# 07350100647/nvbio-gpl

Hardware: AMD Instinct MI355X
Metric: aligned reads/sec (150 bp single-end, 3 Gbp ref); GCUPS of the banded extend pass in `extend` (higher is better)
Workload: dtype u32 (FM-index coordinates) / i16x2 (band-31 DP, two alignments per 32-bit lane: 16-bit integer scores, held in binary16 lanes where every score is an integer of magnitude <= 2040 -- exact -- and in int16 lanes otherwise; bound-checked on the host)

## Files before the change

### include/nvbio_amd.h

```cpp
#ifndef NVBIO_AMD_H
#define NVBIO_AMD_H

#include <stdint.h>

#ifdef __cplusplus
extern "C" {
#endif

#define NVBIO_AMD_VERSION 100

typedef enum
{
    NVBIO_OK              = 0,
    NVBIO_ERR_INVALID     = 1,
    NVBIO_ERR_HIP         = 2,
    NVBIO_ERR_NOMEM       = 3,
    NVBIO_ERR_UNSUPPORTED = 4,
    NVBIO_ERR_NO_DEVICE   = 5
} nvbio_status;

int         nvbio_amd_version(void);
const char* nvbio_amd_last_error(void);
nvbio_status nvbio_amd_device_count(int* count);
nvbio_status nvbio_amd_device_arch(int device, char* name, uint32_t name_len);
nvbio_status nvbio_amd_stream_synchronize(int device, void* stream);
nvbio_status nvbio_amd_release_scratch(void);
nvbio_status nvbio_amd_set_scratch_check(int enable, uint32_t fill_byte);
nvbio_status nvbio_amd_scratch_check_report(char* buf, uint64_t buf_len);

typedef struct { uint32_t x, y; } nvbio_uint2;


typedef struct
{
    uint32_t        length;
    uint32_t        primary;
    uint32_t        L2[5];
    const uint32_t* bwt_occ_dev;
    uint64_t        bwt_occ_words;
    const uint32_t* ssa_dev;
    uint64_t        ssa_words;
    uint32_t        sa_int;
} nvbio_fm_index_view;

typedef struct nvbio_fm_index_s* nvbio_fm_index_t;

nvbio_status nvbio_fm_index_create(const nvbio_fm_index_view* view, int device, uint32_t kmer_len,
                                   void* stream, nvbio_fm_index_t* out);

typedef struct
{
    uint32_t kmer_len;
    uint32_t sa_int;
    uint32_t max_lcp;
    uint32_t verify;
    uint32_t table_flags;
    uint32_t bucket_symbols;
} nvbio_fm_build_options;

enum
{
    NVBIO_FM_TABLE_NO_DIRECT  = 1,
    NVBIO_FM_TABLE_NO_CONTEXT = 2,
    NVBIO_FM_TABLE_NO_GROUPS  = 4,
    NVBIO_FM_TABLE_CANONICAL_WIDE = 16,
    NVBIO_FM_TABLE_NO_TEXT_PLANES = 32,
    NVBIO_FM_TABLE_CANONICAL  = 8
};

nvbio_status nvbio_fm_index_build(const uint32_t* text2_dev, uint32_t length, int device,
                                  const nvbio_fm_build_options* options ,
                                  void* stream, nvbio_fm_index_t* out);

nvbio_status nvbio_fm_index_load(const char* bwt_path, const char* sa_path, int device, uint32_t kmer_len,
                                 void* stream, nvbio_fm_index_t* out);
nvbio_status nvbio_fm_index_save(nvbio_fm_index_t index, const char* bwt_path, const char* sa_path, void* stream);

nvbio_status nvbio_fm_index_destroy(nvbio_fm_index_t index);
nvbio_status nvbio_fm_index_get_view(nvbio_fm_index_t index, nvbio_fm_index_view* view);
nvbio_status nvbio_fm_index_export(nvbio_fm_index_t index, uint32_t* bwt_occ_out_dev, uint32_t* ssa_out_dev, void* stream);
nvbio_status nvbio_fm_index_device_bytes(nvbio_fm_index_t index, uint64_t* bytes);

nvbio_status nvbio_text_planes_bytes(uint32_t length, uint64_t* bytes);
nvbio_status nvbio_text_planes_build(int device, const uint32_t* text2_dev, uint32_t length, void* planes_dev, void* stream);
nvbio_status nvbio_fm_index_text_planes(nvbio_fm_index_t index, const void** planes_dev, uint32_t* length);

typedef struct
{
    const void*     symbols_dev;
    uint32_t        symbol_bits;
    const uint32_t* offsets_dev;
    uint32_t        offsets_are_ranges;
    uint32_t        fixed_len;
    uint32_t        stride;
    uint32_t        n;
    uint32_t        seeds_per_string;
    uint32_t        seed_interval;
    const uint32_t* seed_intervals_dev;
} nvbio_string_set;

enum
{
    NVBIO_FM_SCAN_FORWARD = 1,
    NVBIO_FM_COMPLEMENT   = 2,
    NVBIO_FM_NO_KMER_TABLE = 4,
    NVBIO_FM_NO_VERIFY     = 8,
    NVBIO_FM_COUNT_SECTORS = 16,
    NVBIO_FM_NO_PIPELINE   = 32
};

nvbio_status nvbio_fm_match(nvbio_fm_index_t index, const nvbio_string_set* queries, uint32_t flags,
                            nvbio_uint2* ranges_dev, uint32_t* blocks_dev, void* stream);

nvbio_status nvbio_fm_rank(nvbio_fm_index_t index, const uint32_t* rows_dev, const uint8_t* syms_dev, uint32_t n,
                           uint32_t* out_dev, void* stream);
nvbio_status nvbio_fm_rank4(nvbio_fm_index_t index, const uint32_t* rows_dev, uint32_t n,
                            uint32_t* out_dev, void* stream);

typedef struct
{
    const void* text_dev;
    uint32_t    word_bits;
    const void* occ_dev;
    uint32_t    index_bits;
    uint32_t    K;
    uint64_t    length;
} nvbio_rank_dictionary;
nvbio_status nvbio_rank_dictionary_occ_entries(const nvbio_rank_dictionary* dict, uint64_t* entries);
nvbio_status nvbio_rank_dictionary_build(int device, const nvbio_rank_dictionary* dict, void* occ_out_dev, uint64_t counts[4], void* stream);
nvbio_status nvbio_rank_dictionary_rank(int device, const nvbio_rank_dictionary* dict, const void* idx_dev, const uint8_t* syms_dev, uint32_t n,
                                        void* out_dev, void* stream);
nvbio_status nvbio_rank_dictionary_rank4(int device, const nvbio_rank_dictionary* dict, const void* idx_dev, uint32_t n, void* out_dev, void* stream);

nvbio_status nvbio_fm_basic_inv_psi(nvbio_fm_index_t index, const uint32_t* rows_dev, uint32_t n,
                                    uint32_t* out_dev, void* stream);

nvbio_status nvbio_fm_locate(nvbio_fm_index_t index, const uint32_t* rows_dev, uint32_t n,
                             uint32_t* pos_dev, void* stream);
nvbio_status nvbio_fm_match_direct(nvbio_fm_index_t index, const nvbio_string_set* queries, uint32_t flags,
                                   nvbio_uint2* ranges_dev, uint8_t* direct_dev, void* stream);
nvbio_status nvbio_fm_index_supports_direct(nvbio_fm_index_t index, int* yes);
nvbio_status nvbio_fm_filter_locate_direct(nvbio_fm_index_t index, const nvbio_uint2* ranges_dev, const uint64_t* slots_dev,
                                           const uint8_t* direct_dev, uint32_t n_queries, uint64_t begin, uint64_t end,
                                           nvbio_uint2* hits_dev, void* stream);

nvbio_status nvbio_fm_filter_locate_diagonals(nvbio_fm_index_t index, const nvbio_uint2* ranges_dev, const uint64_t* slots_dev,
                                              const uint8_t* direct_dev, uint32_t n_queries, uint64_t begin, uint64_t end,
                                              uint32_t seeds_per_read, uint32_t seed_interval, uint32_t seed_len, uint32_t read_len,
                                              uint32_t strand, const uint32_t* query_ids_dev, uint64_t* keys_dev, void* stream);

enum { NVBIO_BACKTRACK_REFERENCE_QUIRKS = 1 };
nvbio_status nvbio_fm_hamming_backtrack(nvbio_fm_index_t index, const nvbio_string_set* queries, uint32_t seed_len, uint32_t mismatches, uint32_t flags,
                                        uint32_t* counts_dev, uint32_t* n_ranges_dev, nvbio_uint2* ranges_dev, uint32_t max_ranges, void* stream);

nvbio_status nvbio_fm_match_seed_diagonals_temp_bytes(const nvbio_string_set* seeds, uint64_t* bytes);
nvbio_status nvbio_fm_match_seed_diagonals(nvbio_fm_index_t index, const nvbio_string_set* seeds, uint32_t flags, uint32_t read_len,
                                           uint32_t strand, uint64_t* keys_dev, nvbio_uint2* residual_ranges_dev, uint32_t* residual_ids_dev,
                                           uint32_t* counts_dev, void* temp_dev, uint64_t temp_bytes, void* stream);

#define NVBIO_FM_INLINE_HITS(h) (((uint32_t)(h) & 15u) << 8)
#define NVBIO_FM_DEFER_HEAVY 64u
nvbio_status nvbio_fm_match_seed_diagonals_both_temp_bytes(const nvbio_string_set* seeds, uint64_t* bytes);
nvbio_status nvbio_fm_match_seed_diagonals_both_keys_capacity(const nvbio_string_set* seeds, uint64_t* n_keys);
nvbio_status nvbio_fm_match_seed_diagonals_both(nvbio_fm_index_t index, const nvbio_string_set* seeds, uint32_t flags, uint32_t read_len,
                                                uint64_t* keys_dev, nvbio_uint2* residual_ranges_dev, uint32_t* residual_ids_dev,
                                                uint32_t residual_capacity, uint32_t* counts_dev, void* temp_dev, uint64_t temp_bytes,
                                                void* stream);
nvbio_status nvbio_fm_seed_tiles(const nvbio_string_set* seeds, uint32_t* reads_per_tile, uint32_t* n_tiles);
nvbio_status nvbio_fm_match_seed_diagonals_both_tiled(nvbio_fm_index_t index, const nvbio_string_set* seeds, uint32_t flags, uint32_t read_len,
                                                      uint64_t* keys_dev, nvbio_uint2* residual_ranges_dev, uint32_t* residual_ids_dev,
                                                      uint32_t residual_capacity, uint32_t* counts_dev, uint32_t* tile_offsets_dev,
                                                      void* temp_dev, uint64_t temp_bytes, void* stream);
int nvbio_fm_index_is_canonical(nvbio_fm_index_t index);

nvbio_status nvbio_fm_locate_init(nvbio_fm_index_t index, const uint32_t* rows_dev, uint32_t n,
                                  nvbio_uint2* jt_dev, void* stream);
nvbio_status nvbio_fm_locate_lookup(nvbio_fm_index_t index, const nvbio_uint2* jt_dev, uint32_t n,
                                    uint32_t* pos_dev, void* stream);

nvbio_status nvbio_fm_filter_rank(nvbio_fm_index_t index, const nvbio_string_set* queries, uint32_t flags,
                                  nvbio_uint2* ranges_dev, uint64_t* slots_dev, uint64_t* n_hits, void* stream);
nvbio_status nvbio_fm_filter_scan(nvbio_fm_index_t index, const nvbio_uint2* ranges_dev, uint32_t n_queries,
                                  uint64_t* slots_dev, uint64_t* n_hits, void* stream);
nvbio_status nvbio_fm_filter_locate(nvbio_fm_index_t index, const nvbio_uint2* ranges_dev, const uint64_t* slots_dev,
                                    uint32_t n_queries, uint64_t begin, uint64_t end,
                                    nvbio_uint2* hits_dev, void* stream);


typedef struct { uint32_t x, y, string_id, span; } nvbio_mem_range;
typedef struct { uint32_t pos, string_id, span_begin, span_end; } nvbio_mem_hit;
typedef struct { uint32_t min_intv, max_intv, min_span, split_len, split_width; } nvbio_mem_params;

nvbio_status nvbio_mem_filter_temp_bytes(const nvbio_string_set* reads, const nvbio_mem_params* params, uint64_t* bytes, void* stream);
nvbio_status nvbio_mem_filter_rank(nvbio_fm_index_t f_index, nvbio_fm_index_t r_index, const nvbio_string_set* reads,
                                   const nvbio_mem_params* params, nvbio_mem_range* ranges_dev, uint32_t max_ranges,
                                   uint32_t* first_range_dev, uint64_t* slots_dev, void* temp_dev, uint64_t temp_bytes,
                                   uint32_t* n_ranges, uint64_t* n_mems, uint64_t* records, void* stream);
nvbio_status nvbio_mem_filter_locate(nvbio_fm_index_t f_index, const nvbio_mem_range* ranges_dev, const uint64_t* slots_dev,
                                     uint32_t n_ranges, uint64_t begin, uint64_t end, nvbio_mem_hit* hits_dev, void* stream);

typedef struct nvbio_qgram_index_s* nvbio_qgram_index_t;

typedef struct
{
    uint32_t        q, symbol_size, qlut;
    uint32_t        is_set;
    uint32_t        n_qgrams, n_unique;
    uint64_t        lut_size;
    int             device;
    const uint64_t* qgrams_dev;
    const uint32_t* slots_dev;
    const void*     index_dev;
    const uint32_t* lut_dev;
} nvbio_qgram_index_view;

nvbio_status nvbio_qgram_index_build(int device, const void* text_dev, uint32_t text_bits, uint32_t length, uint32_t q, uint32_t symbol_size,
                                     uint32_t qlut, nvbio_qgram_index_t* out, void* stream);
nvbio_status nvbio_qgram_set_index_build(int device, const nvbio_string_set* set, uint32_t q, uint32_t symbol_size, uint32_t seed_interval,
                                         uint32_t qlut, nvbio_qgram_index_t* out, void* stream);
nvbio_status nvbio_qgram_index_destroy(nvbio_qgram_index_t index);
nvbio_status nvbio_qgram_index_get_view(nvbio_qgram_index_t index, nvbio_qgram_index_view* view);
nvbio_status nvbio_qgram_index_device_bytes(nvbio_qgram_index_t index, uint64_t* bytes);
nvbio_status nvbio_qgram_index_export(nvbio_qgram_index_t index, uint64_t* qgrams_out_dev, uint32_t* slots_out_dev, void* index_out_dev,
                                      uint32_t* lut_out_dev, void* stream);

nvbio_status nvbio_generate_qgrams_temp_bytes(uint32_t n, int sort, uint64_t* bytes);
nvbio_status nvbio_generate_qgrams(int device, uint32_t q, uint32_t symbol_size, const void* text_dev, uint32_t text_bits, uint32_t text_len,
                                   uint32_t first_pos, uint32_t n, uint64_t* qgrams_dev, uint32_t* indices_dev, int sort,
                                   void* temp_dev, uint64_t temp_bytes, void* stream);
nvbio_status nvbio_qgram_ranges(nvbio_qgram_index_t index, const uint64_t* qgrams_dev, uint32_t n, nvbio_uint2* ranges_dev, void* stream);

nvbio_status nvbio_qgram_filter_temp_bytes(uint32_t n_queries, uint64_t* bytes);
nvbio_status nvbio_qgram_filter_rank(nvbio_qgram_index_t index, const uint64_t* qgrams_dev, uint32_t n, nvbio_uint2* ranges_dev, uint64_t* slots_dev,
                                     void* temp_dev, uint64_t temp_bytes, uint64_t* n_hits, void* stream);
nvbio_status nvbio_qgram_filter_locate(nvbio_qgram_index_t index, const nvbio_uint2* ranges_dev, const uint64_t* slots_dev, const uint32_t* indices_dev,
                                       uint32_t n, uint64_t begin, uint64_t end, void* hits_dev, void* stream);
nvbio_status nvbio_qgram_filter_merge_temp_bytes(int is_set, uint32_t n_hits, uint64_t* bytes);
nvbio_status nvbio_qgram_filter_merge(int device, int is_set, uint32_t interval, const void* hits_dev, uint32_t n_hits, void* merged_dev,
                                      uint32_t* counts_dev, uint32_t* n_merged, void* temp_dev, uint64_t temp_bytes, void* stream);

typedef struct
{
    uint32_t           q, symbol_size;
    uint32_t           is_set;
    uint32_t           n_qgrams, n_unique;
    uint64_t           n_words;
    int                device;
    const nvbio_uint2* table_dev;
    const uint32_t*    ss_dev;
    const void*        p_dev;
} nvbio_qgroup_index_view;

nvbio_status nvbio_qgroup_index_build(int device, const void* text_dev, uint32_t text_bits, uint32_t length, uint32_t q, uint32_t symbol_size,
                                      nvbio_qgram_index_t* out, void* stream);
nvbio_status nvbio_qgroup_set_index_build(int device, const nvbio_string_set* set, uint32_t q, uint32_t symbol_size, uint32_t seed_interval,
                                          nvbio_qgram_index_t* out, void* stream);
nvbio_status nvbio_qgroup_index_get_view(nvbio_qgram_index_t index, nvbio_qgroup_index_view* view);
nvbio_status nvbio_qgroup_index_export(nvbio_qgram_index_t index, uint32_t* I_out_dev, uint32_t* S_out_dev, uint32_t* SS_out_dev, void* P_out_dev,
                                       void* stream);

enum { NVBIO_SUFSORT_NO_EMPTY_SUFFIXES = 1 };

typedef struct
{
    uint32_t n_suffixes;
    uint32_t rounds;
    uint32_t sorted_per_round[16];
    uint32_t symbols_per_word;
    uint64_t peak_bytes;
} nvbio_sufsort_stats;

nvbio_status nvbio_set_suffix_count(int device, const nvbio_string_set* set, uint32_t flags, uint32_t* n_suffixes, void* stream);
nvbio_status nvbio_set_suffix_sort(int device, const nvbio_string_set* set, uint32_t flags, nvbio_uint2* suffixes_dev, uint32_t* global_dev,
                                   uint64_t capacity, uint32_t* n_suffixes, nvbio_sufsort_stats* stats, void* stream);
nvbio_status nvbio_set_suffix_sort_flat(int device, const nvbio_string_set* set, uint32_t flags, uint32_t* suffix_array_dev, uint32_t* string_ids_dev,
                                        uint32_t* cum_lengths_dev, uint64_t capacity, uint32_t* n_suffixes, nvbio_sufsort_stats* stats, void* stream);
nvbio_status nvbio_set_bwt(int device, const nvbio_string_set* set, uint32_t flags, uint8_t* bwt_dev, nvbio_uint2* suffixes_dev,
                           uint64_t capacity, uint32_t* n_suffixes, nvbio_sufsort_stats* stats, void* stream);

nvbio_status nvbio_suffix_sort(const uint32_t* text2_dev, uint32_t length, int device, uint32_t* sa_dev, void* stream);
nvbio_status nvbio_bwt(const uint32_t* text2_dev, uint32_t length, int device, uint32_t* bwt_words_dev, uint32_t* primary, void* stream);


nvbio_status nvbio_hits_to_diagonals(int device, const nvbio_uint2* hits_dev, uint64_t n_hits, uint32_t seeds_per_read,
                                     uint32_t seed_interval, uint32_t seed_len, uint32_t read_len, uint32_t strand,
                                     uint64_t* keys_dev, void* stream);

nvbio_status nvbio_sort_unique_keys_temp_bytes(uint64_t n, uint64_t* bytes);
nvbio_status nvbio_sort_unique_keys(int device, uint64_t* keys_dev, uint64_t n, uint32_t* n_out_dev, void* temp_dev, uint64_t temp_bytes, void* stream);

nvbio_status nvbio_diagonals_to_windows(int device, const uint64_t* keys_dev, uint64_t n, uint32_t band, uint32_t read_len,
                                        uint32_t genome_len, uint32_t* read_id_dev, uint8_t* flags_dev,
                                        uint32_t* win_begin_dev, uint32_t* win_end_dev, void* stream);

nvbio_status nvbio_diagonals_to_windows_ragged(int device, const uint64_t* keys_dev, uint64_t n, uint32_t band, const uint32_t* read_offsets_dev,
                                               uint32_t genome_len, uint32_t* read_id_dev, uint8_t* flags_dev,
                                               uint32_t* win_begin_dev, uint32_t* win_end_dev, void* stream);
nvbio_status nvbio_fm_filter_locate_diagonals_ragged(nvbio_fm_index_t index, const nvbio_uint2* ranges_dev, const uint64_t* slots_dev,
                                                     const uint8_t* direct_dev, uint32_t n_queries, uint64_t begin, uint64_t end,
                                                     uint32_t seeds_per_read, uint32_t seed_len, const uint32_t* read_offsets_dev,
                                                     const uint32_t* seed_intervals_dev, uint32_t strand, const uint32_t* query_ids_dev,
                                                     uint64_t* keys_dev, void* stream);
nvbio_status nvbio_traceback_best_batch_ragged(int device, const uint64_t* best_dev, const int64_t* best_wb_dev, uint32_t n_reads,
                                               const uint32_t* read_offsets_dev, uint32_t band, uint32_t genome_len, const int32_t* min_scores_dev,
                                               uint8_t* flags_dev, uint32_t* win_begin_dev, uint32_t* win_end_dev, int32_t* scores_dev,
                                               nvbio_uint2* sinks_dev, void* stream);
nvbio_status nvbio_second_candidate_reduce_ragged(int device, const uint64_t* keys_dev, const int32_t* scores_dev, const nvbio_uint2* sinks_dev,
                                                  const uint32_t* win_begin_dev, uint64_t n, const uint64_t* best_dev,
                                                  const uint32_t* read_offsets_dev, const int32_t* min_scores_dev, uint64_t* second_dev, void* stream);
nvbio_status nvbio_mapq_ragged(int device, const uint64_t* best_dev, const uint64_t* second_dev, uint32_t n_reads, int32_t version, int32_t match,
                               const uint32_t* read_offsets_dev, const int32_t* min_scores_dev, int32_t* second_scores_dev, uint8_t* mapq_dev,
                               void* stream);

nvbio_status nvbio_fm_residual_diagonals(nvbio_fm_index_t index, const nvbio_uint2* ranges_dev, const uint32_t* ids_dev, uint32_t n, uint32_t cap,
// ... 380 lines not shown
```

### nvbio-gpl_amd/__init__.py

```python
import ctypes
import os

import numpy as np

_HERE = os.path.dirname(os.path.abspath(__file__))
LIB_PATH = os.path.join(_HERE, "lib", "libnvbio_amd.so")
HEADER_PATH = os.path.join(os.path.dirname(_HERE), "include", "nvbio_amd.h")

GLOBAL, LOCAL, SEMI_GLOBAL = 0, 1, 2
SCORE_MIN = -(1 << 30)
FM_SCAN_FORWARD, FM_COMPLEMENT, FM_NO_KMER_TABLE, FM_NO_VERIFY, FM_COUNT_SECTORS, FM_NO_PIPELINE, FM_DEFER_HEAVY = 1, 2, 4, 8, 16, 32, 64
FM_TABLE_NO_DIRECT, FM_TABLE_NO_CONTEXT, FM_TABLE_NO_GROUPS, FM_TABLE_CANONICAL, FM_TABLE_CANONICAL_WIDE = 1, 2, 4, 8, 16
FM_TABLE_NO_TEXT_PLANES = 32
READ_REVERSE, READ_COMPLEMENT = 1, 2
TRACEBACK_SINKS_GIVEN = 1
ALN_NO_UNGAPPED_SCORE, ALN_NO_THIRD_CHANCE, ALN_NO_PACKED_DP, ALN_FORCE_PACKED_DP, ALN_NO_UNGAPPED_TRACEBACK, ALN_PK_THREE_WAVES = 1, 2, 4, 8, 16, 32
ALN_NO_NARROW_TRACEBACK, ALN_NO_SECOND_CHANCE, ALN_PK_STRIPE8, ALN_NO_NARROW_SCORE, ALN_NO_BAND_ROUTE = 64, 128, 256, 512, 1024
ALN_NO_QUALITY_SHORTCUT, ALN_RAGGED_READS, ALN_NO_LENGTH_SORT, ALN_NO_F16_DP, ALN_NO_COOPERATIVE_DP, ALN_NO_GAP_CHANCE = 2048, 4096, 8192, 16384, 32768, 65536
ALN_SPLIT_CHANCES, ALN_NO_PAIRED_GAP_CHANCE = 131072, 262144
ALN_NO_NARROW_DP = 524288
ALN_NO_TEXT_PLANES = 1048576
ROUTE_SETTLED, ROUTE_FULL_BAND, ROUTE_CLASS_A, ROUTE_CLASS_B, ROUTE_REDONE = 0, 1, 2, 3, 8
DEFAULT_ALGO_FLAGS = 0
BACKTRACK_REFERENCE_QUIRKS = 1

_STATUS = {0: "OK", 1: "INVALID", 2: "HIP", 3: "NOMEM", 4: "UNSUPPORTED", 5: "NO_DEVICE"}


class NvbioError(RuntimeError):
    def __init__(self, status, msg):
        super().__init__("nvbio_amd: %s: %s" % (_STATUS.get(status, status), msg))
        self.status = status


class _View(ctypes.Structure):
    _fields_ = [("length", ctypes.c_uint32), ("primary", ctypes.c_uint32), ("L2", ctypes.c_uint32 * 5),
                ("bwt_occ_dev", ctypes.c_void_p), ("bwt_occ_words", ctypes.c_uint64),
                ("ssa_dev", ctypes.c_void_p), ("ssa_words", ctypes.c_uint64), ("sa_int", ctypes.c_uint32)]


class _BuildOptions(ctypes.Structure):
    _fields_ = [("kmer_len", ctypes.c_uint32), ("sa_int", ctypes.c_uint32), ("max_lcp", ctypes.c_uint32),
                ("verify", ctypes.c_uint32), ("table_flags", ctypes.c_uint32), ("bucket_symbols", ctypes.c_uint32)]


class _StringSet(ctypes.Structure):
    _fields_ = [("symbols_dev", ctypes.c_void_p), ("symbol_bits", ctypes.c_uint32),
                ("offsets_dev", ctypes.c_void_p), ("offsets_are_ranges", ctypes.c_uint32),
                ("fixed_len", ctypes.c_uint32), ("stride", ctypes.c_uint32), ("n", ctypes.c_uint32),
                ("seeds_per_string", ctypes.c_uint32), ("seed_interval", ctypes.c_uint32),
                ("seed_intervals_dev", ctypes.c_void_p)]


class _Scheme(ctypes.Structure):
    _fields_ = [("match", ctypes.c_int32), ("mm_min", ctypes.c_int32), ("mm_max", ctypes.c_int32),
                ("pat_gap_open", ctypes.c_int32), ("pat_gap_ext", ctypes.c_int32),
                ("txt_gap_open", ctypes.c_int32), ("txt_gap_ext", ctypes.c_int32)]


class _SWScheme(ctypes.Structure):
    _fields_ = [("match", ctypes.c_int32), ("mismatch", ctypes.c_int32), ("deletion", ctypes.c_int32),
                ("insertion", ctypes.c_int32)]


class _Batch(ctypes.Structure):
    _fields_ = [("reads_dev", ctypes.c_void_p), ("read_bits", ctypes.c_uint32),
                ("read_offsets_dev", ctypes.c_void_p), ("quals_dev", ctypes.c_void_p),
                ("read_id_dev", ctypes.c_void_p), ("flags_dev", ctypes.c_void_p),
                ("text_dev", ctypes.c_void_p), ("text_bits", ctypes.c_uint32),
                ("win_begin_dev", ctypes.c_void_p), ("win_end_dev", ctypes.c_void_p), ("n", ctypes.c_uint32),
                ("max_read_len", ctypes.c_uint32), ("algo_flags", ctypes.c_uint32),
                ("text_planes_dev", ctypes.c_void_p)]


class _HitQueues(ctypes.Structure):
    _fields_ = [("idx_queue_dev", ctypes.c_void_p), ("hit_read_id_dev", ctypes.c_void_p), ("hit_seed_dev", ctypes.c_void_p),
                ("hit_loc_dev", ctypes.c_void_p), ("hit_score_dev", ctypes.c_void_p), ("hit_sink_dev", ctypes.c_void_p),
                ("n", ctypes.c_uint32)]


class _SeedHitsParams(ctypes.Structure):
    _fields_ = [(n, ctypes.c_uint32) for n in ("seeds_per_read", "first_offset", "seed_interval", "seed_len", "read_len", "max_hits",
                                                "rep_seeds", "max_effort", "min_ext", "max_ext")]


class _RaggedSeedLayout(ctypes.Structure):
    _fields_ = [("read_offsets_dev", ctypes.c_void_p), ("seed_intervals_dev", ctypes.c_void_p)] + \
               [(n, ctypes.c_uint32) for n in ("seeds_per_read", "seeding_pass", "max_reseed", "seed_len", "min_read_len")]


class _RankDict(ctypes.Structure):
    _fields_ = [("text_dev", ctypes.c_void_p), ("word_bits", ctypes.c_uint32), ("occ_dev", ctypes.c_void_p), ("index_bits", ctypes.c_uint32),
                ("K", ctypes.c_uint32), ("length", ctypes.c_uint64)]


_lib = None


def lib():
    global _lib
    if _lib is None:
        if not os.path.exists(LIB_PATH):
            raise NvbioError(5, "%s is missing: build it with __graft_entry__.build() "
                                "(there is no CPU fallback)" % LIB_PATH)
        import torch
        L = ctypes.CDLL(LIB_PATH)
        L.nvbio_amd_last_error.restype = ctypes.c_char_p
        L.nvbio_amd_version.restype = ctypes.c_int
        _lib = L
    return _lib


def release_scratch():
    _check(lib().nvbio_amd_release_scratch())


def set_scratch_check(enable, fill_byte=0):
    _check(lib().nvbio_amd_set_scratch_check(ctypes.c_int(1 if enable else 0), ctypes.c_uint32(fill_byte)))


def scratch_check_report():
    buf = ctypes.create_string_buffer(1 << 16)
    _check(lib().nvbio_amd_scratch_check_report(buf, ctypes.c_uint64(len(buf))))
    out = {}
    for line in buf.value.decode().splitlines():
        tag, checked, damaged, sub, off = line.split()
        out[tag] = (int(checked), int(damaged), None if sub == "-" else int(sub), None if off == "-" else int(off))
    return out


def _check(status):
    if status != 0:
        raise NvbioError(status, lib().nvbio_amd_last_error().decode())


def _torch():
    import torch
    return torch


_SCRATCH = {}


def _scratch(device, nbytes, cap=8 << 30):
    torch = _torch()
    nbytes = int(min(max(nbytes, 1 << 20), cap))
    key = str(device)
    t = _SCRATCH.get(key)
    if t is None or t.numel() < nbytes:
        _SCRATCH[key] = None
        t = _SCRATCH[key] = torch.empty(nbytes, dtype=torch.uint8, device=device)
    return t


def _ptr(t):
    return None if t is None else ctypes.c_void_p(t.data_ptr())


def _stream_ptr(device):
    torch = _torch()
    return ctypes.c_void_p(torch.cuda.current_stream(device).cuda_stream)


def device_count():
    n = ctypes.c_int(0)
    lib().nvbio_amd_device_count(ctypes.byref(n))
    return n.value


def _dev_tensor(a, dtype, device):
    torch = _torch()
    if a is None:
        return None
    if isinstance(a, torch.Tensor):
        t = a
        if t.dtype != dtype:
            t = t.view(dtype) if t.element_size() == torch.empty(0, dtype=dtype).element_size() else t.to(dtype)
        return t.to(device).contiguous()
    a = np.ascontiguousarray(a)
    np_of = {torch.int32: np.int32, torch.uint8: np.uint8, torch.int64: np.int64}[dtype]
    if a.dtype.itemsize == np.dtype(np_of).itemsize:
        a = a.view(np_of)
    else:
        a = a.astype(np_of)
    return torch.from_numpy(a).to(device)


class PackedStringSet:

    def __init__(self, symbols, bits, n, offsets=None, ranges=False, fixed_len=0, stride=None, device="cuda:0",
                 seeds_per_string=0, seed_interval=0, seed_intervals=None):
        torch = _torch()
        self.bits, self.n = int(bits), int(n)
        self.symbols = _dev_tensor(symbols, torch.uint8 if bits == 8 else torch.int32, device)
        self.offsets = _dev_tensor(offsets, torch.int32, device)
        self.ranges, self.fixed_len = bool(ranges), int(fixed_len)
        self.stride = int(fixed_len if stride is None else stride)
        self.device = device
        self.seeds_per_string, self.seed_interval = int(seeds_per_string), int(seed_interval)
        self.seed_intervals = _dev_tensor(seed_intervals, torch.int32, device)

    def c_struct(self):
        return _StringSet(_ptr(self.symbols), self.bits, _ptr(self.offsets), 1 if self.ranges else 0,
                          self.fixed_len, self.stride, self.n, self.seeds_per_string, self.seed_interval, _ptr(self.seed_intervals))


class FMIndex:

    def __init__(self, handle, device, keep=()):
        self._h, self.device, self._keep = handle, device, keep
        self._text_src = None
        self._text_planes = None

    @staticmethod
    def _dev_index(device):
        torch = _torch()
        d = torch.device(device)
        return d.index if d.index is not None else 0

    @classmethod
    def from_arrays(cls, length, primary, L2, bwt_occ, ssa, kmer_len=0, sa_int=16, device="cuda:0"):
        torch = _torch()
        b = _dev_tensor(bwt_occ, torch.int32, device)
        s = _dev_tensor(ssa, torch.int32, device) if ssa is not None else None
        v = _View()
        v.length, v.primary = int(length), int(primary)
        for i in range(5):
            v.L2[i] = int(L2[i])
        v.bwt_occ_dev, v.bwt_occ_words = b.data_ptr(), b.numel()
        v.ssa_dev, v.ssa_words = (s.data_ptr(), s.numel()) if s is not None else (None, 0)
        v.sa_int = sa_int
        h = ctypes.c_void_p()
        _check(lib().nvbio_fm_index_create(ctypes.byref(v), cls._dev_index(device), ctypes.c_uint32(kmer_len),
                                           _stream_ptr(device), ctypes.byref(h)))
        return cls(h, device, keep=(b, s))

    @classmethod
    def build(cls, text2, length, kmer_len=0, max_lcp=0, sa_int=16, verify=False, device="cuda:0", table_flags=0,
              bucket_symbols=None):
        torch = _torch()
        t = _dev_tensor(text2, torch.int32, device)
        h = ctypes.c_void_p()
        opts = _BuildOptions(kmer_len, sa_int, max_lcp, 1 if verify else 0, int(table_flags),
                             0 if bucket_symbols is None else 1 + int(bucket_symbols))
        _check(lib().nvbio_fm_index_build(_ptr(t), ctypes.c_uint32(length), cls._dev_index(device),
                                          ctypes.byref(opts), _stream_ptr(device), ctypes.byref(h)))
        fmi = cls(h, device, keep=(t,))
        fmi._text_src = (t.data_ptr(), int(length))
        fmi._text_planes = fmi.text_planes()
        return fmi

    @classmethod
    def load(cls, bwt_path, sa_path=None, kmer_len=0, device="cuda:0"):
        h = ctypes.c_void_p()
        _check(lib().nvbio_fm_index_load(bwt_path.encode(), sa_path.encode() if sa_path else None,
                                         cls._dev_index(device), ctypes.c_uint32(kmer_len), _stream_ptr(device),
                                         ctypes.byref(h)))
        return cls(h, device)

    def save(self, bwt_path, sa_path=None):
        _check(lib().nvbio_fm_index_save(self._h, bwt_path.encode(), sa_path.encode() if sa_path else None,
                                         _stream_ptr(self.device)))

    def close(self):
        if self._h is not None:
            _torch().cuda.synchronize(self.device)
            _check(lib().nvbio_fm_index_destroy(self._h))
            self._h = None
            self._seed_bufs = None

    def __del__(self):
        try:
            self.close()
        except Exception:
            pass

    def view(self):
        v = _View()
        _check(lib().nvbio_fm_index_get_view(self._h, ctypes.byref(v)))
        return v

    @property
    def length(self):
        return self.view().length

    @property
    def primary(self):
        return self.view().primary

    def arrays(self):
        torch = _torch()
        v = self.view()
        b = torch.empty(int(v.bwt_occ_words), dtype=torch.int32, device=self.device)
        s = torch.empty(int(v.ssa_words), dtype=torch.int32, device=self.device)
        _check(lib().nvbio_fm_index_export(self._h, _ptr(b), _ptr(s), _stream_ptr(self.device)))
        return b, s

    def device_bytes(self):
        b = ctypes.c_uint64()
        _check(lib().nvbio_fm_index_device_bytes(self._h, ctypes.byref(b)))
        return b.value

    def text_planes(self):
        p, n = ctypes.c_void_p(), ctypes.c_uint32()
        _check(lib().nvbio_fm_index_text_planes(self._h, ctypes.byref(p), ctypes.byref(n)))
        return (p.value, n.value) if p.value else None

    def text_planes_of(self, text2, length):
        tp = self._text_planes if self._h is not None else None
        same = tp is not None and self._text_src == (text2.data_ptr(), int(length)) and tp[1] == int(length)
        return tp[0] if same else None

    def match(self, queries, flags=0, want_blocks=False):
        torch = _torch()
        ranges = torch.empty((queries.n, 2), dtype=torch.int32, device=self.device)
        blocks = torch.empty(queries.n, dtype=torch.int32, device=self.device) if want_blocks else None
        qs = queries.c_struct()
        _check(lib().nvbio_fm_match(self._h, ctypes.byref(qs), ctypes.c_uint32(flags), _ptr(ranges), _ptr(blocks),
                                    _stream_ptr(self.device)))
        return (ranges, blocks) if want_blocks else ranges

    def supports_direct(self):
        yes = ctypes.c_int(0)
        _check(lib().nvbio_fm_index_supports_direct(self._h, ctypes.byref(yes)))
        return bool(yes.value)

    def match_direct(self, queries, flags=0):
        torch = _torch()
        ranges = torch.empty((queries.n, 2), dtype=torch.int32, device=self.device)
        direct = torch.empty(queries.n, dtype=torch.uint8, device=self.device)
        qs = queries.c_struct()
        _check(lib().nvbio_fm_match_direct(self._h, ctypes.byref(qs), ctypes.c_uint32(flags), _ptr(ranges), _ptr(direct),
                                           _stream_ptr(self.device)))
        return ranges, direct

    def hamming_backtrack(self, queries, seed_len, mismatches, quirks=False, max_ranges=0):
        torch = _torch()
        counts = torch.empty(queries.n, dtype=torch.int32, device=self.device)
        nr = torch.empty(queries.n, dtype=torch.int32, device=self.device)
        rg = torch.zeros((queries.n, max_ranges, 2), dtype=torch.int32, device=self.device) if max_ranges else None
        qs = queries.c_struct()
        _check(lib().nvbio_fm_hamming_backtrack(self._h, ctypes.byref(qs), ctypes.c_uint32(seed_len), ctypes.c_uint32(mismatches),
                                                ctypes.c_uint32(BACKTRACK_REFERENCE_QUIRKS if quirks else 0), _ptr(counts), _ptr(nr), _ptr(rg),
                                                ctypes.c_uint32(max_ranges), _stream_ptr(self.device)))
        return counts, nr, rg

    def match_seed_diagonals(self, seeds, flags, read_len, strand, buffers=None, grid_blocks=0):
        torch = _torch()
        n = seeds.n
        if buffers is None:
            buffers = {}
        qs = seeds.c_struct()
        if buffers.get("n") != n or buffers.get("spr") != seeds.seeds_per_string:
            buffers["n"], buffers["spr"] = n, seeds.seeds_per_string
            buffers["keys"] = torch.empty(n, dtype=torch.int64, device=self.device)
            buffers["ranges"] = torch.empty((n, 2), dtype=torch.int32, device=self.device)
            buffers["ids"] = torch.empty(n, dtype=torch.int32, device=self.device)
            buffers["counts"] = torch.empty(4, dtype=torch.int32, device=self.device)
            nb = ctypes.c_uint64(0)
            _check(lib().nvbio_fm_match_seed_diagonals_temp_bytes(ctypes.byref(qs), ctypes.byref(nb)))
            buffers["temp"] = torch.empty(nb.value, dtype=torch.uint8, device=self.device)
        assert grid_blocks % 64 == 0 and grid_blocks < (1 << 22)
        _check(lib().nvbio_fm_match_seed_diagonals(self._h, ctypes.byref(qs), ctypes.c_uint32(flags | ((grid_blocks // 64) << 16)),
                                                   ctypes.c_uint32(read_len), ctypes.c_uint32(strand), _ptr(buffers["keys"]),
                                                   _ptr(buffers["ranges"]), _ptr(buffers["ids"]), _ptr(buffers["counts"]),
                                                   _ptr(buffers["temp"]), ctypes.c_uint64(buffers["temp"].numel()),
                                                   _stream_ptr(self.device)))
        return buffers

    @property
    def canonical_kmer(self):
        fn = lib().nvbio_fm_index_is_canonical
        fn.restype = ctypes.c_int
        return int(fn(self._h))

    @property
    def canonical(self):
        return self.canonical_kmer != 0

    def match_seed_diagonals_both(self, seeds, read_len, buffers=None, flags=0, grid_blocks=0, inline_hits=0, defer_heavy=False):
        torch = _torch()
        n = seeds.n
        if buffers is None:
            buffers = {}
        qs = seeds.c_struct()
        if buffers.get("n") != n or buffers.get("spr") != seeds.seeds_per_string:
            buffers["n"], buffers["spr"] = n, seeds.seeds_per_string
            cap = ctypes.c_uint64(0)
            _check(lib().nvbio_fm_match_seed_diagonals_both_keys_capacity(ctypes.byref(qs), ctypes.byref(cap)))
            buffers["keys"] = torch.empty(max(int(cap.value), 1), dtype=torch.int64, device=self.device)
            buffers["ranges"] = torch.empty((2 * n, 2), dtype=torch.int32, device=self.device)
            buffers["ids"] = torch.empty(2 * n, dtype=torch.int32, device=self.device)
            buffers["counts"] = torch.empty(6, dtype=torch.int32, device=self.device)
            nb = ctypes.c_uint64(0)
            _check(lib().nvbio_fm_match_seed_diagonals_both_temp_bytes(ctypes.byref(qs), ctypes.byref(nb)))
            buffers["temp"] = torch.empty(nb.value, dtype=torch.uint8, device=self.device)
            rpt, nt = ctypes.c_uint32(0), ctypes.c_uint32(0)
            _check(lib().nvbio_fm_seed_tiles(ctypes.byref(qs), ctypes.byref(rpt), ctypes.byref(nt)))
            buffers["reads_per_tile"], buffers["n_tiles"] = int(rpt.value), int(nt.value)
            buffers["tile_offsets"] = torch.zeros(int(nt.value) + 1, dtype=torch.int32, device=self.device)
        assert grid_blocks % 64 == 0 and grid_blocks < (1 << 22)
        _check(lib().nvbio_fm_match_seed_diagonals_both_tiled(
            self._h, ctypes.byref(qs), ctypes.c_uint32(flags | (FM_DEFER_HEAVY if defer_heavy else 0) | ((int(inline_hits) & 15) << 8) | ((grid_blocks // 64) << 16)),
            ctypes.c_uint32(read_len),
            _ptr(buffers["keys"]), _ptr(buffers["ranges"]), _ptr(buffers["ids"]), ctypes.c_uint32(n), _ptr(buffers["counts"]),
            _ptr(buffers["tile_offsets"]), _ptr(buffers["temp"]), ctypes.c_uint64(buffers["temp"].numel()), _stream_ptr(self.device)))
        return buffers

    def residual_diagonals(self, ranges, ids, cap, seeds_per_read, seed_interval, seed_len, read_len, read_offsets=None, seed_intervals=None):
        torch = _torch()
        n = int(ids.numel())
        keys = torch.empty(max(n * int(cap), 1), dtype=torch.int64, device=self.device)
        n_keys = torch.zeros(1, dtype=torch.int32, device=self.device)
        _check(lib().nvbio_fm_residual_diagonals(
            self._h, _ptr(ranges), _ptr(ids), ctypes.c_uint32(n), ctypes.c_uint32(int(cap)), ctypes.c_uint32(seeds_per_read),
            ctypes.c_uint32(seed_interval), ctypes.c_uint32(seed_len), ctypes.c_uint32(read_len), _ptr(read_offsets), _ptr(seed_intervals),
            _ptr(keys), _ptr(n_keys), _stream_ptr(self.device)))
        return keys, n_keys

    def rank(self, rows, syms):
        torch = _torch()
        rows = _dev_tensor(rows, torch.int32, self.device)
        syms = _dev_tensor(syms, torch.uint8, self.device)
        out = torch.empty(rows.numel(), dtype=torch.int32, device=self.device)
        _check(lib().nvbio_fm_rank(self._h, _ptr(rows), _ptr(syms), ctypes.c_uint32(rows.numel()), _ptr(out),
                                   _stream_ptr(self.device)))
        return out

    def rank4(self, rows):
        torch = _torch()
        rows = _dev_tensor(rows, torch.int32, self.device)
        out = torch.empty((rows.numel(), 4), dtype=torch.int32, device=self.device)
        _check(lib().nvbio_fm_rank4(self._h, _ptr(rows), ctypes.c_uint32(rows.numel()), _ptr(out),
                                    _stream_ptr(self.device)))
        return out

    def basic_inv_psi(self, rows):
        torch = _torch()
        rows = _dev_tensor(rows, torch.int32, self.device)
        out = torch.empty(rows.numel(), dtype=torch.int32, device=self.device)
        _check(lib().nvbio_fm_basic_inv_psi(self._h, _ptr(rows), ctypes.c_uint32(rows.numel()), _ptr(out),
                                            _stream_ptr(self.device)))
        return out

    def locate(self, rows):
        torch = _torch()
        rows = _dev_tensor(rows, torch.int32, self.device)
        pos = torch.empty(rows.numel(), dtype=torch.int32, device=self.device)
        _check(lib().nvbio_fm_locate(self._h, _ptr(rows), ctypes.c_uint32(rows.numel()), _ptr(pos),
                                     _stream_ptr(self.device)))
        return pos

    def locate_ssa_iterator(self, rows):
        torch = _torch()
        rows = _dev_tensor(rows, torch.int32, self.device)
        jt = torch.empty((rows.numel(), 2), dtype=torch.int32, device=self.device)
        _check(lib().nvbio_fm_locate_init(self._h, _ptr(rows), ctypes.c_uint32(rows.numel()), _ptr(jt),
                                          _stream_ptr(self.device)))
        return jt

    def lookup_ssa_iterator(self, jt):
        torch = _torch()
        pos = torch.empty(jt.shape[0], dtype=torch.int32, device=self.device)
        _check(lib().nvbio_fm_locate_lookup(self._h, _ptr(jt), ctypes.c_uint32(jt.shape[0]), _ptr(pos),
                                            _stream_ptr(self.device)))
        return pos


class FMIndexFilter:

    def __init__(self):
        self._index = None
        self._ranges = self._slots = self._direct = None
        self._n_hits = 0
        self._n_queries = 0

    def rank(self, index, string_set, flags=0):
        torch = _torch()
        self._index, self._n_queries, self._direct = index, string_set.n, None
        self._ranges = torch.empty((string_set.n, 2), dtype=torch.int32, device=index.device)
        self._slots = torch.empty(string_set.n, dtype=torch.int64, device=index.device)
        total = ctypes.c_uint64(0)
        qs = string_set.c_struct()
        _check(lib().nvbio_fm_filter_rank(index._h, ctypes.byref(qs), ctypes.c_uint32(flags), _ptr(self._ranges),
                                          _ptr(self._slots), ctypes.byref(total), _stream_ptr(index.device)))
        self._n_hits = total.value
        return self._n_hits

    def rank_ranges(self, index, ranges, direct=None):
        torch = _torch()
        self._index, self._n_queries, self._ranges, self._direct = index, ranges.shape[0], ranges, direct
        self._slots = torch.empty(ranges.shape[0], dtype=torch.int64, device=index.device)
        total = ctypes.c_uint64(0)
        _check(lib().nvbio_fm_filter_scan(index._h, _ptr(ranges), ctypes.c_uint32(ranges.shape[0]), _ptr(self._slots),
                                          ctypes.byref(total), _stream_ptr(index.device)))
        self._n_hits = total.value
        return self._n_hits

    def locate(self, begin, end, hits=None):
        torch = _torch()
        if hits is None:
            hits = torch.empty((end - begin, 2), dtype=torch.int32, device=self._index.device)
        if self._direct is not None:
            _check(lib().nvbio_fm_filter_locate_direct(self._index._h, _ptr(self._ranges), _ptr(self._slots), _ptr(self._direct),
                                                       ctypes.c_uint32(self._n_queries), ctypes.c_uint64(begin),
                                                       ctypes.c_uint64(end), _ptr(hits), _stream_ptr(self._index.device)))
            return hits
        _check(lib().nvbio_fm_filter_locate(self._index._h, _ptr(self._ranges), _ptr(self._slots),
                                            ctypes.c_uint32(self._n_queries), ctypes.c_uint64(begin),
                                            ctypes.c_uint64(end), _ptr(hits), _stream_ptr(self._index.device)))
        return hits

    def locate_diagonals(self, begin, end, seeds_per_read, seed_interval, seed_len, read_len, strand, query_ids=None, read_offsets=None,
                         seed_intervals=None):
        torch = _torch()
        keys = torch.empty(end - begin, dtype=torch.int64, device=self._index.device)
        if read_offsets is not None:
            _check(lib().nvbio_fm_filter_locate_diagonals_ragged(
                self._index._h, _ptr(self._ranges), _ptr(self._slots), _ptr(self._direct), ctypes.c_uint32(self._n_queries),
                ctypes.c_uint64(begin), ctypes.c_uint64(end), ctypes.c_uint32(seeds_per_read), ctypes.c_uint32(seed_len), _ptr(read_offsets),
                _ptr(seed_intervals), ctypes.c_uint32(strand), _ptr(query_ids), _ptr(keys), _stream_ptr(self._index.device)))
            return keys
        _check(lib().nvbio_fm_filter_locate_diagonals(
            self._index._h, _ptr(self._ranges), _ptr(self._slots), _ptr(self._direct), ctypes.c_uint32(self._n_queries),
            ctypes.c_uint64(begin), ctypes.c_uint64(end), ctypes.c_uint32(seeds_per_read), ctypes.c_uint32(seed_interval),
            ctypes.c_uint32(seed_len), ctypes.c_uint32(read_len), ctypes.c_uint32(strand), _ptr(query_ids), _ptr(keys),
            _stream_ptr(self._index.device)))
        return keys

    def n_hits(self):
        return self._n_hits

    def ranges(self):
        return self._ranges

    def slots(self):
        return self._slots


class _MemParams(ctypes.Structure):
    _fields_ = [("min_intv", ctypes.c_uint32), ("max_intv", ctypes.c_uint32), ("min_span", ctypes.c_uint32),
                ("split_len", ctypes.c_uint32), ("split_width", ctypes.c_uint32)]


MEM_GROUP_FLAG = 1 << 31
MEM_UNLIMITED = 0xFFFFFFFF
# ... 333 lines not shown

class QGramFilter:

    def __init__(self):
        self._index = None
        self._ranges = self._slots = self._indices = self._temp = None
        self._merged = self._counts = None
        self._n_queries = self._n_hits = 0

    def _grow_temp(self, nbytes, dev):
        torch = _torch()
        if self._temp is None or self._temp.numel() < nbytes or self._temp.device != torch.device(dev):
            self._temp = None
            self._temp = torch.empty(max(int(nbytes), 1), dtype=torch.uint8, device=dev)

    def rank(self, index, qgrams, indices):
        torch = _torch()
        dev = index.device
        g = _dev_tensor(qgrams, torch.int64, dev)
        ix = _dev_tensor(indices, torch.int32, dev)
        n = g.numel()
        self._index, self._n_queries, self._indices = index, n, ix
        if self._ranges is None or self._ranges.shape[0] < n or self._ranges.device != torch.device(dev):
            self._ranges = torch.empty((max(n, 1), 2), dtype=torch.int32, device=dev)
            self._slots = torch.empty(max(n, 1), dtype=torch.int64, device=dev)
        tb = ctypes.c_uint64(0)
        _check(lib().nvbio_qgram_filter_temp_bytes(ctypes.c_uint32(n), ctypes.byref(tb)))
        self._grow_temp(tb.value, dev)
        nh = ctypes.c_uint64(0)
        _check(lib().nvbio_qgram_filter_rank(index._h, _ptr(g), ctypes.c_uint32(n), _ptr(self._ranges), _ptr(self._slots), _ptr(self._temp),
                                             ctypes.c_uint64(self._temp.numel()), ctypes.byref(nh), _stream_ptr(dev)))
        self._n_hits = nh.value
        return self._n_hits

    def n_hits(self):
        return self._n_hits

    def ranges(self):
        return self._ranges[:self._n_queries]

    def slots(self):
        return self._slots[:self._n_queries]

    def locate(self, begin, end, hits=None):
        torch = _torch()
        cols = 4 if self._index.IS_SET else 2
        if hits is None:
            hits = torch.empty((max(end - begin, 0), cols), dtype=torch.int32, device=self._index.device)
        if end > begin:
            _check(lib().nvbio_qgram_filter_locate(self._index._h, _ptr(self._ranges), _ptr(self._slots), _ptr(self._indices),
                                                   ctypes.c_uint32(self._n_queries), ctypes.c_uint64(begin), ctypes.c_uint64(end), _ptr(hits),
                                                   _stream_ptr(self._index.device)))
        return hits

    def merge(self, interval, hits, is_set=None):
        torch = _torch()
        if is_set is None:
            is_set = hits.dim() == 2 and hits.shape[1] == 4
        dev = hits.device
        n = hits.shape[0]
        tb = ctypes.c_uint64(0)
        _check(lib().nvbio_qgram_filter_merge_temp_bytes(ctypes.c_int(1 if is_set else 0), ctypes.c_uint32(n), ctypes.byref(tb)))
        self._grow_temp(tb.value, dev)
        if self._merged is None or self._merged.shape[0] < max(n, 1) or self._merged.device != dev:
            self._merged = torch.empty((max(n, 1), 2), dtype=torch.int32, device=dev)
            self._counts = torch.empty(max(n, 1), dtype=torch.int32, device=dev)
        nm = ctypes.c_uint32(0)
        hits = hits.contiguous()
        _check(lib().nvbio_qgram_filter_merge(FMIndex._dev_index(dev), ctypes.c_int(1 if is_set else 0), ctypes.c_uint32(interval), _ptr(hits),
                                              ctypes.c_uint32(n), _ptr(self._merged), _ptr(self._counts), ctypes.byref(nm), _ptr(self._temp),
                                              ctypes.c_uint64(self._temp.numel()), _stream_ptr(dev)))
        m = nm.value
        merged = self._merged.view(-1)[:2 * m].view(m, 2) if is_set else self._merged.view(-1)[:m]
        return merged.clone(), self._counts[:m].clone()


class GotohScheme:

    def __init__(self, match, mm_min, mm_max, pat_gap_open, pat_gap_ext, txt_gap_open, txt_gap_ext):
        self.c = _Scheme(match, mm_min, mm_max, pat_gap_open, pat_gap_ext, txt_gap_open, txt_gap_ext)


def SimpleGotohScheme(match, mismatch, gap_open, gap_ext):
    return GotohScheme(match, -mismatch, -mismatch, gap_open, gap_ext, gap_open, gap_ext)


def EditDistanceScheme():
    return GotohScheme(0, 1, 1, -1, -1, -1, -1)


class SimpleSmithWatermanScheme:

    def __init__(self, match, mismatch, deletion, insertion):
        self.c = _SWScheme(match, mismatch, deletion, insertion)


class SmithWatermanAligner:

    def __init__(self, type, scheme):
        self.type, self.sw = type, scheme
        c = scheme.c
        self.scheme = (GotohScheme(c.match, -c.mismatch, -c.mismatch, c.deletion, c.deletion, c.deletion, c.deletion)
                       if c.deletion == c.insertion else None)


def make_smith_waterman_aligner(type, scheme):
    return SmithWatermanAligner(type, scheme)


def make_edit_distance_aligner(type):
    return SmithWatermanAligner(type, SimpleSmithWatermanScheme(0, -1, -1, -1))


class GotohAligner:

    def __init__(self, type, scheme):
        self.type, self.scheme = type, scheme


def make_gotoh_aligner(type, scheme):
    return GotohAligner(type, scheme)


class AlignmentBatch:

    def __init__(self, reads, read_bits, read_offsets, text, text_bits, win_begin, win_end, quals=None, read_id=None,
                 flags=None, device="cuda:0", max_read_len=0, algo_flags=None, text_planes=None):
        torch = _torch()
        self.device = device
        self.text_planes = text_planes
        self.algo_flags = DEFAULT_ALGO_FLAGS if algo_flags is None else int(algo_flags)
        self.read_bits, self.text_bits = int(read_bits), int(text_bits)
        self.reads = _dev_tensor(reads, torch.uint8 if read_bits == 8 else torch.int32, device)
        self.read_offsets = _dev_tensor(read_offsets, torch.int32, device)
        self.text = _dev_tensor(text, torch.uint8 if text_bits == 8 else torch.int32, device)
        self.win_begin = _dev_tensor(win_begin, torch.int32, device)
        self.win_end = _dev_tensor(win_end, torch.int32, device)
        self.quals = _dev_tensor(quals, torch.uint8, device)
        self.read_id = _dev_tensor(read_id, torch.int32, device)
        self.flags = _dev_tensor(flags, torch.uint8, device)
        self.n = int(self.win_begin.numel())
        self.max_read_len = int(max_read_len)

    def size(self):
        return self.n

    def c_struct(self):
        return _Batch(_ptr(self.reads), self.read_bits, _ptr(self.read_offsets), _ptr(self.quals), _ptr(self.read_id),
                      _ptr(self.flags), _ptr(self.text), self.text_bits, _ptr(self.win_begin), _ptr(self.win_end),
                      self.n, self.max_read_len, self.algo_flags,
                      ctypes.c_void_p(self.text_planes.data_ptr() if hasattr(self.text_planes, "data_ptr") else self.text_planes))


def text_planes_bytes(length):
    b = ctypes.c_uint64()
    _check(lib().nvbio_text_planes_bytes(ctypes.c_uint32(length), ctypes.byref(b)))
    return b.value


def build_text_planes(text2, length, device="cuda:0", out=None):
    torch = _torch()
    t = _dev_tensor(text2, torch.int32, device)
    if out is None:
        out = torch.empty(text_planes_bytes(length), dtype=torch.uint8, device=device)
    _check(lib().nvbio_text_planes_build(FMIndex._dev_index(device), _ptr(t), ctypes.c_uint32(length), _ptr(out), _stream_ptr(device)))
    return out


DEVICE_THREAD_SCHEDULER = "DeviceThreadScheduler"
DEVICE_STAGED_THREAD_SCHEDULER = "DeviceStagedThreadScheduler"


class BatchedBandedAlignmentScore:

    def __init__(self, band_len, aligner, scheduler=DEVICE_THREAD_SCHEDULER):
        self.band_len, self.aligner, self.scheduler = int(band_len), aligner, scheduler
        if scheduler not in (DEVICE_THREAD_SCHEDULER, DEVICE_STAGED_THREAD_SCHEDULER):
            raise NvbioError(1, "unknown scheduler %r" % (scheduler,))

    def min_temp_storage(self, max_pattern_len, max_text_len, stream_size):
        return 0

    max_temp_storage = min_temp_storage

    def enact(self, batch, scores=None, sinks=None, min_scores=None):
        torch = _torch()
        if scores is None:
            scores = torch.empty(batch.n, dtype=torch.int32, device=batch.device)
        if sinks is None:
            sinks = torch.empty((batch.n, 2), dtype=torch.int32, device=batch.device)
        bs = batch.c_struct()
        sw = getattr(self.aligner, "sw", None)
        if self.scheduler == DEVICE_STAGED_THREAD_SCHEDULER:
            if sw is not None:
                raise NvbioError(4, "the staged scheduler is instantiated for Gotoh aligners")
            per_job = min_scores is not None and not isinstance(min_scores, int)
            if per_job and (min_scores.dtype != torch.int32 or min_scores.numel() != batch.n):
                raise NvbioError(1, "min_scores: int32 per job")
            _check(lib().nvbio_banded_gotoh_score_staged(
                FMIndex._dev_index(batch.device), ctypes.c_uint32(self.band_len), ctypes.c_int(self.aligner.type),
                ctypes.byref(self.aligner.scheme.c), ctypes.byref(bs), _ptr(min_scores) if per_job else None,
                ctypes.c_int32(SCORE_MIN if min_scores is None else (0 if per_job else int(min_scores))),
                _ptr(scores), _ptr(sinks), _stream_ptr(batch.device)))
            return scores, sinks
        fn = lib().nvbio_banded_sw_score if sw is not None else lib().nvbio_banded_gotoh_score
        _check(fn(FMIndex._dev_index(batch.device), ctypes.c_uint32(self.band_len), ctypes.c_int(self.aligner.type),
                  ctypes.byref(sw.c if sw is not None else self.aligner.scheme.c),
                  ctypes.byref(bs), _ptr(scores), _ptr(sinks), _stream_ptr(batch.device)))
        return scores, sinks


def batch_banded_alignment_score(band_len, aligner, batch):
    return BatchedBandedAlignmentScore(band_len, aligner).enact(batch)


def banded_gotoh_score_routes(band_len, aligner, batch):
    torch = _torch()
    scores = torch.empty(batch.n, dtype=torch.int32, device=batch.device)
    sinks = torch.empty((batch.n, 2), dtype=torch.int32, device=batch.device)
    routes = torch.empty(batch.n, dtype=torch.uint8, device=batch.device)
    bs = batch.c_struct()
    _check(lib().nvbio_banded_gotoh_score_routes(FMIndex._dev_index(batch.device), ctypes.c_uint32(int(band_len)), ctypes.c_int(aligner.type),
                                                 ctypes.byref(aligner.scheme.c), ctypes.byref(bs), _ptr(scores), _ptr(sinks), _ptr(routes),
                                                 _stream_ptr(batch.device)))
    return scores, sinks, routes


TB_ROUTE_SETTLED, TB_ROUTE_FULL_BAND, TB_ROUTE_BAND15, TB_ROUTE_BAND7 = 0, 1, 2, 3


def banded_gotoh_traceback_routes(band_len, aligner, batch, cigar_stride=64, temp=None, scores=None, sinks=None):
    torch = _torch()
    n, dev = batch.n, batch.device
    given = scores is not None and sinks is not None
    if not given:
        scores = torch.empty(n, dtype=torch.int32, device=dev)
        sinks = torch.empty((n, 2), dtype=torch.int32, device=dev)
    sources = torch.empty((n, 2), dtype=torch.int32, device=dev)
    cigars = torch.zeros((n, cigar_stride), dtype=torch.int16, device=dev)
    lens = torch.empty(n, dtype=torch.int32, device=dev)
    routes = torch.empty(n, dtype=torch.uint8, device=dev)
    band_off = torch.empty(n, dtype=torch.uint8, device=dev)
    bs = batch.c_struct()
    _check(lib().nvbio_banded_gotoh_traceback_routes(
        FMIndex._dev_index(dev), ctypes.c_uint32(int(band_len)), ctypes.c_int(aligner.type), ctypes.byref(aligner.scheme.c), ctypes.byref(bs),
        _ptr(scores), _ptr(sources), _ptr(sinks), _ptr(cigars), ctypes.c_uint32(cigar_stride), _ptr(lens),
        ctypes.c_uint32(TRACEBACK_SINKS_GIVEN if given else 0), _ptr(temp),
        ctypes.c_uint64(0 if temp is None else temp.numel() * temp.element_size()), _ptr(routes), _ptr(band_off), _stream_ptr(dev)))
    return scores, sources, sinks, cigars, lens, routes, band_off


GAP_PAIR_MAX_SHIFT = 5
NO_PARTNER = 0xFFFFFFFF


def banded_gap_pairs(batch):
    torch = _torch()
    partner = torch.empty(batch.n, dtype=torch.int32, device=batch.device)
    bs = batch.c_struct()
    _check(lib().nvbio_banded_gap_pairs(FMIndex._dev_index(batch.device), ctypes.byref(bs), _ptr(partner), _stream_ptr(batch.device)))
    return partner


class BatchedBandedAlignmentTraceback:

    def __init__(self, band_len, aligner):
        self.band_len, self.aligner = int(band_len), aligner

    def min_temp_storage(self, batch):
        out = ctypes.c_uint64(0)
        bs = batch.c_struct()
        _check(lib().nvbio_banded_gotoh_traceback_temp_bytes(ctypes.byref(bs), ctypes.c_uint32(self.band_len), ctypes.byref(out)))
        return int(out.value)

    def enact(self, batch, cigar_stride=64, temp=None, scores=None, sinks=None):
        torch = _torch()
        n, dev = batch.n, batch.device
        given = scores is not None and sinks is not None
        if not given:
            scores = torch.empty(n, dtype=torch.int32, device=dev)
            sinks = torch.empty((n, 2), dtype=torch.int32, device=dev)
        sources = torch.empty((n, 2), dtype=torch.int32, device=dev)
        cigars = torch.zeros((n, cigar_stride), dtype=torch.int16, device=dev)
        lens = torch.empty(n, dtype=torch.int32, device=dev)
        bs = batch.c_struct()
        sw = getattr(self.aligner, "sw", None)
        fn = lib().nvbio_banded_sw_traceback if sw is not None else lib().nvbio_banded_gotoh_traceback
        _check(fn(
            FMIndex._dev_index(dev), ctypes.c_uint32(self.band_len), ctypes.c_int(self.aligner.type),
            ctypes.byref(sw.c if sw is not None else self.aligner.scheme.c), ctypes.byref(bs), _ptr(scores), _ptr(sources), _ptr(sinks), _ptr(cigars),
            ctypes.c_uint32(cigar_stride), _ptr(lens), ctypes.c_uint32(TRACEBACK_SINKS_GIVEN if given else 0), _ptr(temp),
            ctypes.c_uint64(0 if temp is None else temp.numel() * temp.element_size()), _stream_ptr(dev)))
        return scores, sources, sinks, cigars, lens


class BatchedAlignmentTraceback:

    def __init__(self, aligner):
        self.aligner = aligner

    def min_temp_storage(self, batch, max_pattern_len, max_text_len):
        out = ctypes.c_uint64(0)
        bs = batch.c_struct()
        _check(lib().nvbio_full_gotoh_traceback_temp_bytes(ctypes.byref(bs), ctypes.c_uint32(max_pattern_len),
                                                           ctypes.c_uint32(max_text_len), ctypes.byref(out)))
        return int(out.value)
# ... 655 lines not shown
```

### nvbio-gpl_amd/csrc/bitplanes.h

```cpp
#pragma once
#include "common.h"

namespace nvbio_amd {

constexpr uint32_t PLANE_MAX_READ = 161u;

template <int RBITS> struct ReadWords { static constexpr int N = (161 + 15) * RBITS / 32 + 2; uint32_t w[N]; };

template <int RBITS>
__device__ __forceinline__ void load_read_words(const void* reads, const uint32_t first, const uint32_t M, ReadWords<RBITS>& out)
{
    constexpr uint32_t RPW = 32u / RBITS;
    const uint32_t* __restrict__ rwords = (const uint32_t*)reads;
    const uint32_t rw0 = (first & ~(RPW - 1u)) / RPW, rw_last = (first + M - 1u) / RPW;
    #pragma unroll
    for (int j = 0; j < ReadWords<RBITS>::N; ++j) { const uint32_t widx = rw0 + (uint32_t)j; out.w[j] = rwords[widx < rw_last ? widx : rw_last]; }
}

template <typename W>
__device__ __forceinline__ void load_text_words13(const void* text, const uint32_t tb, const uint32_t T, W& out)
{
    const uint32_t* __restrict__ twords = (const uint32_t*)text;
    const uint32_t tw0 = (tb & ~15u) >> 4, tw_last = (tb + T - 1u) >> 4;
    #pragma unroll
    for (int j = 0; j < 13; ++j) { const uint32_t widx = tw0 + (uint32_t)j; out.w[j] = twords[widx < tw_last ? widx : tw_last]; }
}

template <typename W>
__device__ __forceinline__ void load_text_words14(const void* text, const uint32_t tb, const uint32_t T, W& out)
{
    const uint32_t* __restrict__ twords = (const uint32_t*)text;
    const uint32_t tw0 = (tb & ~15u) >> 4, tw_last = (tb + T - 1u) >> 4;
    #pragma unroll
    for (int j = 0; j < 14; ++j) { const uint32_t widx = tw0 + (uint32_t)j; out.w[j] = twords[widx < tw_last ? widx : tw_last]; }
}

__device__ __forceinline__ void shr192(uint64_t (&v)[3], const uint32_t sh)
{
    const uint32_t ws = sh >> 6, bs = sh & 63u;
    uint64_t x[5] = { v[0], v[1], v[2], 0ull, 0ull };
    uint64_t y[4];
    #pragma unroll
    for (int k = 0; k < 4; ++k) y[k] = ws == 0u ? x[k] : (ws == 1u ? x[k + 1 < 5 ? k + 1 : 4] : (ws == 2u ? (k + 2 < 5 ? x[k + 2] : 0ull) : 0ull));
    #pragma unroll
    for (int k = 0; k < 3; ++k) v[k] = bs ? ((y[k] >> bs) | (y[k + 1] << (64u - bs))) : y[k];
}
__device__ __forceinline__ void mirror192(uint64_t (&v)[3])
{
    const uint64_t a = __brevll( v[2] ), c = __brevll( v[0] );
    v[1] = __brevll( v[1] ); v[0] = a; v[2] = c;
}

__device__ __forceinline__ uint32_t squeeze2(uint32_t x)
{
    x &= 0x55555555u;
    x = (x | (x >> 1)) & 0x33333333u; x = (x | (x >> 2)) & 0x0F0F0F0Fu; x = (x | (x >> 4)) & 0x00FF00FFu; x = (x | (x >> 8)) & 0xFFFFu;
    return x;
}
__device__ __forceinline__ uint32_t squeeze4(uint32_t x)
{
    x &= 0x11111111u;
    x = (x | (x >> 3)) & 0x03030303u; x = (x | (x >> 6)) & 0x000F000Fu; x = (x | (x >> 12)) & 0xFFu;
    return x;
}

template <int RBITS>
__device__ __forceinline__ void read_planes192(const ReadWords<RBITS>& rw, const uint32_t first, const uint32_t M, const bool rev, const bool comp,
                                               uint64_t (&rlo)[3], uint64_t (&rhi)[3], uint64_t (&rn)[3])
{
    constexpr uint32_t RPW = 32u / RBITS;
    const uint32_t roff = first & (RPW - 1u);
    #pragma unroll
    for (int k = 0; k < 3; ++k) { rlo[k] = 0; rhi[k] = 0; rn[k] = 0; }
    #pragma unroll
    for (int j = 0; j < ReadWords<RBITS>::N; ++j)
    {
        if (!__any( (uint32_t)j * RPW < roff + M )) continue;
        const uint32_t w = __brev( rw.w[j] );
        uint32_t lo, hi, nn;
        if (RBITS == 4)
        {
            lo = squeeze4( w >> 3 ); hi = squeeze4( w >> 2 ); nn = squeeze4( (w >> 1) | w );
        }
        else { lo = squeeze2( w >> 1 ); hi = squeeze2( w ); nn = 0; }
        const int bitpos = j * (int)RPW;
        if (bitpos < 192)
        {
            rlo[bitpos >> 6] |= (uint64_t)lo << (bitpos & 63);
            rhi[bitpos >> 6] |= (uint64_t)hi << (bitpos & 63);
            rn [bitpos >> 6] |= (uint64_t)nn << (bitpos & 63);
        }
    }
    if (rev)
    {
        mirror192( rlo ); mirror192( rhi ); mirror192( rn );
        const uint32_t sh = 192u - roff - M;
        shr192( rlo, sh ); shr192( rhi, sh ); shr192( rn, sh );
    }
    else { shr192( rlo, roff ); shr192( rhi, roff ); shr192( rn, roff ); }
    if (comp)
    {
        #pragma unroll
        for (int k = 0; k < 3; ++k) { rlo[k] ^= ~rn[k]; rhi[k] ^= ~rn[k]; }
    }
}

template <typename W>
__device__ __forceinline__ void text_planes208(const W& tw, const uint32_t tb, uint64_t (&tlo)[4], uint64_t (&thi)[4])
{
    #pragma unroll
    for (int k = 0; k < 4; ++k) { tlo[k] = 0; thi[k] = 0; }
    #pragma unroll
    for (int j = 0; j < 13; ++j)
    {
        const uint32_t w = __brev( tw.w[j] );
        const uint32_t lo = squeeze2( w >> 1 ), hi = squeeze2( w );
        const int bitpos = j * 16;
        tlo[bitpos >> 6] |= (uint64_t)lo << (bitpos & 63);
        thi[bitpos >> 6] |= (uint64_t)hi << (bitpos & 63);
    }
    const uint32_t toff = tb & 15u;
    if (toff)
    {
        #pragma unroll
        for (int k = 0; k < 3; ++k)
        {
            tlo[k] = (tlo[k] >> toff) | (tlo[k + 1] << (64u - toff));
            thi[k] = (thi[k] >> toff) | (thi[k + 1] << (64u - toff));
        }
        tlo[3] >>= toff; thi[3] >>= toff;
    }
}

constexpr uint32_t TEXT_PLANE_LINE_BYTES = 128u;
inline __host__ __device__ uint64_t text_plane_lines(const uint32_t n) { return (((uint64_t)n + 255u) >> 8) + 1u; }

template <int UNITS> struct TextUnits { uint32_t w[4 * UNITS]; };

template <int UNITS, int FROM = 0, int TO = UNITS>
__device__ __forceinline__ void load_text_units(const void* planes, const uint32_t tb, TextUnits<UNITS>& out)
{
    static_assert( UNITS == 4 || UNITS == 5, "4 units hold 192 symbols at any shift, 5 units hold 197" );
    static_assert( 3 + UNITS - 1 <= 7, "the last unit of a window lies in the line its first unit lies in" );
    typedef uint32_t unit_t __attribute__((ext_vector_type(4)));
    const unit_t* __restrict__ p = (const unit_t*)planes + ((size_t)(tb >> 8) * 8u + ((tb & 255u) >> 6));
    #pragma unroll
    for (int j = FROM; j < TO; ++j) { const unit_t v = p[j]; out.w[4*j] = v.x; out.w[4*j+1] = v.y; out.w[4*j+2] = v.z; out.w[4*j+3] = v.w; }
}

template <int UNITS>
__device__ __forceinline__ void text_planes_units(const TextUnits<UNITS>& tu, const uint32_t tb, uint64_t (&tlo)[4], uint64_t (&thi)[4])
{
    const uint32_t s = tb & 63u;
    const uint32_t up = s >= 32u ? 0xFFFFFFFFu : 0u;
    auto lo = [&](const int i) { return i < 2 * UNITS ? tu.w[4 * (i >> 1) + (i & 1)] : 0u; };
    auto hi = [&](const int i) { return i < 2 * UNITS ? tu.w[4 * (i >> 1) + 2 + (i & 1)] : 0u; };
    uint32_t a[9], c[9];
    #pragma unroll
    for (int i = 0; i < 9; ++i) { a[i] = (lo( i + 1 ) & up) | (lo( i ) & ~up); c[i] = (hi( i + 1 ) & up) | (hi( i ) & ~up); }
    #pragma unroll
    for (int k = 0; k < 4; ++k)
    {
        tlo[k] = (uint64_t)__builtin_amdgcn_alignbit( a[2*k+1], a[2*k], s ) | ((uint64_t)__builtin_amdgcn_alignbit( a[2*k+2], a[2*k+1], s ) << 32);
        thi[k] = (uint64_t)__builtin_amdgcn_alignbit( c[2*k+1], c[2*k], s ) | ((uint64_t)__builtin_amdgcn_alignbit( c[2*k+2], c[2*k+1], s ) << 32);
    }
}

template <typename W>
__device__ __forceinline__ void text_planes224(const W& tw, const uint32_t tb, uint64_t (&tlo)[4], uint64_t (&thi)[4])
{
    #pragma unroll
    for (int k = 0; k < 4; ++k) { tlo[k] = 0; thi[k] = 0; }
    #pragma unroll
    for (int j = 0; j < 14; ++j)
    {
        const uint32_t w = __brev( tw.w[j] );
        const uint32_t lo = squeeze2( w >> 1 ), hi = squeeze2( w );
        const int bitpos = j * 16;
        tlo[bitpos >> 6] |= (uint64_t)lo << (bitpos & 63);
        thi[bitpos >> 6] |= (uint64_t)hi << (bitpos & 63);
    }
    const uint32_t toff = tb & 15u;
    if (toff)
    {
        #pragma unroll
        for (int k = 0; k < 3; ++k)
        {
            tlo[k] = (tlo[k] >> toff) | (tlo[k + 1] << (64u - toff));
            thi[k] = (thi[k] >> toff) | (thi[k + 1] << (64u - toff));
        }
        tlo[3] >>= toff; thi[3] >>= toff;
    }
}

}
```

### nvbio-gpl_amd/csrc/fm_canon_inl.h

```cpp
constexpr uint32_t CTAB_FLANK    = 7u;
constexpr uint32_t CTAB_ROWS_MAX = 8u;
constexpr uint32_t CTAB_INLINE   = 4u;

__device__ __forceinline__ uint64_t canon_revcomp(const uint64_t key, const uint32_t k)
{
    return reverse_symbols( key, k ) ^ ((1ull << (2u * k)) - 1ull);
}
__device__ __forceinline__ uint64_t canon_index(const uint64_t ckey, const uint32_t k)
{
    return ((ckey >> (k + 1u)) << k) | (ckey & ((1ull << k) - 1ull));
}
__device__ __forceinline__ uint64_t canon_key(const uint64_t idx, const uint32_t k)
{
    return ((idx >> k) << (k + 1u)) | (idx & ((1ull << k) - 1ull));
}
__device__ __forceinline__ uint32_t text_symbol(const uint32_t* __restrict__ text, const uint32_t i)
{
    return (text[i >> 4] >> (30u - 2u * (i & 15u))) & 3u;
}

__device__ __forceinline__ uint2 canon_range(const DevIndex& f, const uint64_t key)
{
    const uint2 r = f.ktab[key >> 2];
    uint32_t x = r.x, y = r.y, nb = 0;
// ... 6 lines not shown
{
    if (m == 1u || (wide && m == 2u)) return 1u;
    return m >= 2u && m <= 4u ? 2u : (m >= 5u && m <= CTAB_ROWS_MAX ? 3u : 0u);
}

__device__ __forceinline__ uint2 canon_row(const uint32_t* __restrict__ text, const uint32_t length, const uint32_t k, const uint32_t p, const uint32_t o)
{
    uint32_t before = 0, after = 0;
    #pragma unroll
    for (uint32_t t = 0; t < CTAB_FLANK; ++t)
    {
        const bool has_l = p >= t + 1u, has_r = (uint64_t)p + k + t < length;
        const uint32_t l = has_l ? text_symbol( text, p - 1u - t ) : 0u;
        const uint32_t g = has_r ? text_symbol( text, p + k + t ) : 0u;
        const uint32_t b = o ? (has_r ? 3u - g : 0u) : l;
        const uint32_t a = o ? (has_l ? 3u - l : 0u) : g;
        before |= b << (2u * (CTAB_FLANK - 1u - t));
        after  |= a << (2u * (CTAB_FLANK - 1u - t));
    }
    return make_uint2( p, DTAB_MARK | (o << 28) | (before << 14) | after );
}

__global__ void __launch_bounds__(256)
fm_ctab_count_kernel(const DevIndex f, const uint32_t k, const uint32_t wide, uint2* __restrict__ tab, const uint64_t n, const uint32_t n_tiles,
                     uint32_t* __restrict__ cnt_small, uint32_t* __restrict__ cnt_large)
{
    const uint32_t stride = wide ? 2u : 1u;
    __shared__ uint32_t s_a[4], s_b[4];
    for (uint32_t tile = blockIdx.x; tile < n_tiles; tile += gridDim.x)
    {
        const uint64_t e0 = (uint64_t)tile * DT_TILE + threadIdx.x * 4u;
        uint32_t a = 0, b = 0;
        #pragma unroll
        for (uint32_t j = 0; j < 4u; ++j)
            if (e0 + j < n)
            {
                const uint64_t key = canon_key( e0 + j, k );
                const uint2 r1 = canon_range( f, key ), r2 = canon_range( f, canon_revcomp( key, k ) );
                tab[(e0 + j) * stride] = r2;
                const uint32_t c = canon_class( range_rows( r1 ) + range_rows( r2 ), wide != 0u );
                a += (c == 2u); b += (c == 3u);
            }
        a = wave_inclusive_sum( a ); b = wave_inclusive_sum( b );
        if ((threadIdx.x & 63u) == 63u) { s_a[threadIdx.x >> 6] = a; s_b[threadIdx.x >> 6] = b; }
        __syncthreads();
        if (threadIdx.x == 0) { cnt_small[tile] = s_a[0] + s_a[1] + s_a[2] + s_a[3]; cnt_large[tile] = s_b[0] + s_b[1] + s_b[2] + s_b[3]; }
        __syncthreads();
    }
}

__global__ void __launch_bounds__(256)
fm_ctab_fill_kernel(const DevIndex f, const uint32_t k, const uint32_t wide, uint2* __restrict__ tab, const uint64_t n, const uint32_t n_tiles,
                    const uint32_t* __restrict__ off_small, const uint32_t* __restrict__ off_large, const uint32_t tot_large, uint2* __restrict__ side)
{
    __shared__ uint32_t s_a[4], s_b[4];
    const uint32_t stride = wide ? 2u : 1u;
    auto position = [&](const uint32_t row) -> uint32_t { const uint32_t sv = f.ssa[row]; return sv == 0xFFFFFFFFu ? f.length : sv; };
    for (uint32_t tile = blockIdx.x; tile < n_tiles; tile += gridDim.x)
    {
        const uint64_t e0 = (uint64_t)tile * DT_TILE + threadIdx.x * 4u;
        uint2 r1[4], r2[4]; uint32_t c[4];
        uint32_t a = 0, b = 0;
        #pragma unroll
        for (uint32_t j = 0; j < 4u; ++j)
        {
            c[j] = 0u; r1[j] = r2[j] = make_uint2( 1u, 0u );
            if (e0 + j < n)
            {
                r1[j] = canon_range( f, canon_key( e0 + j, k ) ); r2[j] = tab[(e0 + j) * stride];
                c[j] = canon_class( range_rows( r1[j] ) + range_rows( r2[j] ), wide != 0u );
                a += (c[j] == 2u); b += (c[j] == 3u);
            }
        }
        const uint32_t ia = wave_inclusive_sum( a ), ib = wave_inclusive_sum( b );
        if ((threadIdx.x & 63u) == 63u) { s_a[threadIdx.x >> 6] = ia; s_b[threadIdx.x >> 6] = ib; }
        __syncthreads();
        uint32_t ga = ia - a, gb = ib - b;
        for (uint32_t w = 0; w < (threadIdx.x >> 6); ++w) { ga += s_a[w]; gb += s_b[w]; }
        ga += off_small[tile]; gb += off_large[tile];
        __syncthreads();
        #pragma unroll
        for (uint32_t j = 0; j < 4u; ++j)
        {
            if (e0 + j >= n) continue;
            const uint32_t n1 = range_rows( r1[j] ), n2 = range_rows( r2[j] ), m = n1 + n2;
            uint2* ent = tab + (e0 + j) * stride;
            if (wide) ent[1] = make_uint2( 0u, 0u );
            auto occurrence = [&](const uint32_t s) -> uint2 {
                return s < n1 ? canon_row( f.text, f.length, k, position( r1[j].x + s ), 0u )
                              : canon_row( f.text, f.length, k, position( r2[j].x + (s - n1) ), 1u );
            };
            if (c[j] == 1u)
            {
                ent[0] = occurrence( 0u );
                if (m == 2u) ent[1] = occurrence( 1u );
            }
            else if (c[j] >= 2u)
            {
                const uint32_t slots = c[j] == 2u ? 4u : 8u;
                const uint32_t idx4  = c[j] == 2u ? 2u * tot_large + ga++ : 2u * gb++;
                uint2* g = side + 4ull * idx4;
                for (uint32_t s = 0; s < slots; ++s) g[s] = s < m ? occurrence( s ) : make_uint2( 0u, DTAB_MARK );
                ent[0] = make_uint2( DTAB_MARK | idx4, DTAB_MARK | m );
            }
            else ent[0] = m ? make_uint2( 0u, 1u ) : make_uint2( 1u, 0u );
        }
    }
}

static nvbio_status build_canonical_table(FMIndexImpl* idx, const uint32_t k, const bool wide, hipStream_t stream)
{
    const uint32_t length = idx->view.length;
    if ((uint64_t)length + 2u > DTAB_MARK) { set_error( "canonical table: the text is too long for the position marker" ); return NVBIO_ERR_UNSUPPORTED; }
    const uint64_t entries = 1ull << (2u * k - 1u);
    const uint32_t n_tiles = (uint32_t)((entries + DT_TILE - 1u) / DT_TILE);
    const dim3 grid( n_tiles < 256u * 64u ? n_tiles : 256u * 64u ), block( 256 );
    uint2* tab = nullptr; uint32_t* cnt = nullptr; void* temp = nullptr; uint2* side = nullptr;
    size_t temp_bytes = 0;
    const uint64_t tab_bytes = entries * sizeof(uint2) * (wide ? 2u : 1u);
    if (hipMalloc( (void**)&tab, tab_bytes ) != hipSuccess) { (void)hipGetLastError(); set_error( "canonical table: out of device memory" ); return NVBIO_ERR_NOMEM; }
    if (hipMalloc( (void**)&cnt, 4ull * n_tiles * sizeof(uint32_t) ) != hipSuccess) { (void)hipGetLastError(); (void)hipFree( tab ); set_error( "canonical table: out of device memory" ); return NVBIO_ERR_NOMEM; }
    uint32_t *cs = cnt, *cl = cnt + n_tiles, *os = cnt + 2ull * n_tiles, *ol = cnt + 3ull * n_tiles;
    const DevIndex f = idx->dev();
    nvbio_status st = NVB_LAUNCH( fm_ctab_count_kernel, grid, block, stream, f, k, wide ? 1u : 0u, tab, entries, n_tiles, cs, cl );
    if (st != NVBIO_OK) { (void)hipFree( cnt ); (void)hipFree( tab ); return st; }
    hipError_t e = hipcub::DeviceScan::ExclusiveSum( nullptr, temp_bytes, cs, os, (int)n_tiles, stream );
    if (e == hipSuccess) e = hipMalloc( &temp, temp_bytes ? temp_bytes : 16 );
    if (e == hipSuccess) e = hipcub::DeviceScan::ExclusiveSum( temp, temp_bytes, cs, os, (int)n_tiles, stream );
    if (e == hipSuccess) e = hipcub::DeviceScan::ExclusiveSum( temp, temp_bytes, cl, ol, (int)n_tiles, stream );
    uint32_t last[4] = { 0, 0, 0, 0 };
    if (e == hipSuccess) e = hipMemcpyAsync( &last[0], cs + n_tiles - 1u, 4, hipMemcpyDeviceToHost, stream );
    if (e == hipSuccess) e = hipMemcpyAsync( &last[1], os + n_tiles - 1u, 4, hipMemcpyDeviceToHost, stream );
    if (e == hipSuccess) e = hipMemcpyAsync( &last[2], cl + n_tiles - 1u, 4, hipMemcpyDeviceToHost, stream );
    if (e == hipSuccess) e = hipMemcpyAsync( &last[3], ol + n_tiles - 1u, 4, hipMemcpyDeviceToHost, stream );
    if (e == hipSuccess) e = hipStreamSynchronize( stream );
    if (e != hipSuccess) { (void)hipGetLastError(); set_error( "canonical table: counting pass failed: %s", hipGetErrorString( e ) ); st = NVBIO_ERR_HIP; }
    const uint32_t tot_small = last[0] + last[1], tot_large = last[2] + last[3];
    const uint64_t units = 2ull * tot_large + tot_small;
    if (st == NVBIO_OK && units >= (1ull << 30)) { set_error( "canonical table: too many groups" ); st = NVBIO_ERR_UNSUPPORTED; }
    if (st == NVBIO_OK && hipMalloc( (void**)&side, (units ? units : 1u) * 32ull ) != hipSuccess) { (void)hipGetLastError(); set_error( "canonical table: out of device memory" ); st = NVBIO_ERR_NOMEM; }
    if (st == NVBIO_OK)
    {
        st = NVB_LAUNCH( fm_ctab_fill_kernel, grid, block, stream, f, k, wide ? 1u : 0u, tab, entries, n_tiles, (const uint32_t*)os, (const uint32_t*)ol, tot_large, side );
        if (st == NVBIO_OK && hipStreamSynchronize( stream ) != hipSuccess) { set_error( "canonical table: fill pass failed" ); st = NVBIO_ERR_HIP; }
    }
    (void)hipFree( cnt );
    if (temp) (void)hipFree( temp );
    if (st != NVBIO_OK) { (void)hipFree( tab ); if (side) (void)hipFree( side ); return st; }
    idx->ctab = tab; idx->cside = side; idx->ckmer = k; idx->cwide = wide ? 1u : 0u;
    idx->owned_bytes += tab_bytes + (units ? units : 1u) * 32ull;
    return NVBIO_OK;
}

template <int BITS, bool COUNT, bool WIDE, bool DEFER>
__global__ void __launch_bounds__(256)
fm_seed_both_kernel(const DevIndex f, const StringSetDev q, const SeedTiles tl, const uint32_t read_len, const uint32_t inline_max,
                    uint64_t* __restrict__ tile_keys, uint32_t* __restrict__ tile_counts, uint2* __restrict__ res_ranges,
                    uint32_t* __restrict__ res_ids, const uint32_t res_cap, unsigned int* __restrict__ counts, unsigned long long* __restrict__ sectors_out,
                    uint32_t* __restrict__ tile_defer, uint32_t* __restrict__ defer_counts)
{
    const uint32_t lane = threadIdx.x & 63u;
    const uint32_t n_waves = gridDim.x * 4u;
    const uint32_t k = f.ckmer, len = q.fixed_len, r = len - k;
    const uint32_t lr = lane / q.spr, j = lane - lr * q.spr;
    const bool lane_ok = lr < tl.rpt;
    const bool ragged = q.intervals != nullptr;
    const uint32_t rmask = (1u << (2u * r)) - 1u;
    const uint32_t fshift = 2u * (CTAB_FLANK - r);
    DevIndex fplain = f; fplain.dtab = nullptr; fplain.dkmer = 0;

    auto seed_geom = [&](const uint32_t rid, uint32_t& begin, uint32_t& p_fw, uint32_t& rlen) -> bool {
        const uint32_t base = q.offsets ? q.offsets[rid] : rid * q.stride;
        p_fw  = j * (ragged ? q.intervals[rid] : q.interval);
        rlen  = ragged ? q.offsets[rid + 1] - base : read_len;
        begin = base + p_fw;
        return !ragged || p_fw + len <= rlen;
    };
    auto entry_of = [&](const uint64_t V, uint32_t& qo) -> uint4 {
        const uint64_t key = V >> (2u * r);
        qo = (uint32_t)(key >> k) & 1u;
        const uint64_t idx = canon_index( qo ? canon_revcomp( key, k ) : key, k );
        if (WIDE)
        {
            typedef unsigned int u4v __attribute__((ext_vector_type(4)));
            const u4v v = __builtin_nontemporal_load( (const u4v*)f.ctab + idx );
            return make_uint4( v.x, v.y, v.z, v.w );
        }
        const uint2 e = load_table_entry( f.ctab, idx, true );
        return make_uint4( e.x, e.y, 0u, 0u );
    };

    uint32_t tile = blockIdx.x * 4u + (threadIdx.x >> 6);
    if (tile >= tl.n_tiles) return;
    SeedWords W = { 0, 0, 0, 0, 0 }; uint32_t w_begin = 0, w_pfw = 0, w_rlen = 0; bool w_valid = false;
    uint64_t V = 0; uint4 e = make_uint4( 1u, 0u, 0u, 0u ); bool e_valid = false; uint32_t qo = 0, c_pfw = 0, c_rlen = 0; bool c_seed = false;
    {
        const uint32_t rid = tile * tl.rpt + lr;
        if (lane_ok && rid < tl.reads)
        {
            uint32_t b0;
            c_seed = seed_geom( rid, b0, c_pfw, c_rlen );
            if (c_seed)
            {
                const SeedWords W0 = load_seed_words<BITS>( q.symbols, b0, len );
                e_valid = seed_bits_from_words<BITS>( W0, b0, len, false, false, V );
                if (e_valid) e = entry_of( V, qo );
            }
        }
        const uint32_t t1 = tile + n_waves, rid1 = t1 * tl.rpt + lr;
        if (t1 < tl.n_tiles && lane_ok && rid1 < tl.reads)
        {
            w_valid = seed_geom( rid1, w_begin, w_pfw, w_rlen );
            if (w_valid) W = load_seed_words<BITS>( q.symbols, w_begin, len );
        }
    }
    for (; tile < tl.n_tiles; tile += n_waves)
    {
        const uint32_t rid = tile * tl.rpt + lr;
        const bool valid = lane_ok && rid < tl.reads && c_seed;
        const bool is_one   = e_valid && e.y >= DTAB_MARK && e.x < DTAB_MARK;
        const bool is_group = e_valid && e.y >= DTAB_MARK && e.x >= DTAB_MARK;
        const bool is_heavy = e_valid && e.y < DTAB_MARK && e.x <= e.y;
        uint4 q0 = make_uint4( 0, 0, 0, 0 ), q1 = q0, q2 = q0, q3 = q0;
        const uint32_t m = e.y - DTAB_MARK;
        if (is_group)
        {
            const uint4* g4 = (const uint4*)(f.cside + 4ull * (e.x - DTAB_MARK));
            q0 = g4[0]; q1 = g4[1];
            if (m > 4u) { q2 = g4[2]; q3 = g4[3]; }
        }
        uint64_t Vn = 0; uint4 en = make_uint4( 1u, 0u, 0u, 0u ); bool en_valid = false; uint32_t qon = 0;
        const uint32_t n_pfw = w_pfw, n_rlen = w_rlen; const bool n_seed = w_valid;
        if (w_valid)
        {
            en_valid = seed_bits_from_words<BITS>( W, w_begin, len, false, false, Vn );
            if (en_valid) en = entry_of( Vn, qon );
        }
        {
            const uint32_t t2 = tile + 2u * n_waves, rid2 = t2 * tl.rpt + lr;
            w_valid = t2 < tl.n_tiles && lane_ok && rid2 < tl.reads;
            if (w_valid) w_valid = seed_geom( rid2, w_begin, w_pfw, w_rlen );
            if (w_valid) W = load_seed_words<BITS>( q.symbols, w_begin, len );
        }
        const uint32_t rest = (uint32_t)V & rmask;
        const uint32_t want = qo ? (~rest & rmask) : rest;
        uint32_t hits[2] = { 0, 0 }, pos[2][CTAB_INLINE] = { { 0, 0, 0, 0 }, { 0, 0, 0, 0 } };
        auto row = [&](const uint32_t P, const uint32_t C) {
            const uint32_t pay = C - DTAB_MARK;
            const uint32_t o = (pay >> 28) & 1u;
            const uint32_t flank = qo ? (pay & 0x3FFFu) : ((pay >> 14) & 0x3FFFu);
            if ((flank >> fshift) != want) return;
            const bool rev = (o ^ qo) != 0u;
            if (rev ? ((uint64_t)P + len > f.length) : (P < r)) return;
            const uint32_t v = rev ? P : P - r;
            #pragma unroll
            for (int s = 0; s < 2; ++s)
                if ((s == 1) == rev)
                {
                    #pragma unroll
                    for (uint32_t t = 0; t < CTAB_INLINE; ++t) pos[s][t] = (hits[s] == t) ? v : pos[s][t];
                    ++hits[s];
                }
        };
        if (is_one) { row( e.x, e.y ); if (WIDE && e.w >= DTAB_MARK) row( e.z, e.w ); }
        else if (is_group)
        {
#define NVB_CROW(jj, P, C) if ((jj) < m) row( (P), (C) );
            NVB_CROW( 0u, q0.x, q0.y ) NVB_CROW( 1u, q0.z, q0.w ) NVB_CROW( 2u, q1.x, q1.y ) NVB_CROW( 3u, q1.z, q1.w )
            NVB_CROW( 4u, q2.x, q2.y ) NVB_CROW( 5u, q2.z, q2.w ) NVB_CROW( 6u, q3.x, q3.y ) NVB_CROW( 7u, q3.z, q3.w )
#undef NVB_CROW
        }
        uint32_t sectors = e_valid ? (is_group ? 2u : 1u) : 0u;
        const uint32_t i = rid * q.spr + j;
        uint32_t tile_fill = 0;
        uint32_t defer_fill = 0;
        #pragma unroll
        for (int s = 0; s < 2; ++s)
        {
            uint32_t cnt = (valid && e_valid && !is_heavy && hits[s] <= inline_max) ? hits[s] : 0u;
            uint32_t rx = 1u, ry = 0u;
            bool searched = false, deferred = false;
            const uint32_t sflags = s ? (NVBIO_FM_SCAN_FORWARD | NVBIO_FM_COMPLEMENT) : 0u;
            auto plain_search = [&]() -> bool {
                uint32_t nblk, sec = 0; bool single = false;
                match_one<BITS,false,true,true>( fplain, q, sflags, f.ktab != nullptr, false, i, rx, ry, nblk, single, &sec );
                sectors += sec; searched = true;
                return single;
            };
            if (valid && e_valid && (is_heavy || hits[s] > inline_max))
            {
                cnt = 0u;
                if (DEFER) deferred = true;
                else if (plain_search()) { pos[s][0] = rx; cnt = 1u; }
                else if (rx <= ry && ry - rx < inline_max)
                {
                    cnt = ry - rx + 1u;
                    #pragma unroll
                    for (uint32_t t = 0; t < CTAB_INLINE; ++t)
                        if (t < cnt) { const uint32_t sv = f.ssa[rx + t]; pos[s][t] = (sv == 0xFFFFFFFFu) ? f.length : sv; }
                    sectors += cnt;
                }
            }
            uint32_t total = (uint32_t)__popcll( __ballot( cnt == 1u ) );
            #pragma unroll
            for (uint32_t t = 0; t < CTAB_INLINE; ++t) total += (uint32_t)__popcll( __ballot( cnt >= 2u && t < cnt ) );
            if (total > 64u && cnt >= 2u)
            {
                if (DEFER) { deferred = true; rx = 1u; ry = 0u; }
                else if (!searched) (void)plain_search();
                cnt = 0u;
            }
            uint64_t* slots = tile_keys + (uint64_t)tile * 128u + tile_fill;
            uint32_t n_out = 0; uint64_t last = ~0ull;
            const uint32_t x1 = cnt == 1u ? pos[s][0] : (cnt == 0u ? rx : 1u), y1 = cnt == 1u ? pos[s][0] : (cnt == 0u ? ry : 0u);
            emit_seed_results( c_pfw, len, c_rlen, (uint32_t)s, lane, valid, cnt == 1u, x1, y1, rid, i, slots, n_out, last,
                               res_ranges + (s ? res_cap : 0u), res_ids + (s ? res_cap : 0u), counts + s );
            if (__ballot( cnt >= 2u ))
            {
                uint32_t pq = c_pfw;
                if (s) pq = c_rlen - pq - len;
                #pragma unroll
                for (uint32_t t = 0; t < CTAB_INLINE; ++t)
                {
                    const bool on = cnt >= 2u && t < cnt;
                    const uint64_t mk = __ballot( on );
                    if (on) slots[n_out + (uint32_t)__popcll( mk & ((1ull << lane) - 1ull) )] =
                                ((uint64_t)rid << 34) | ((uint64_t)s << 33) | ((uint64_t)pos[s][t] + 1024u - pq);
                    n_out += (uint32_t)__popcll( mk );
                }
            }
            tile_fill += n_out;
            if (DEFER)
            {
                const uint64_t md = __ballot( deferred );
                if (md)
                {
                    if (deferred) tile_defer[(uint64_t)tile * 128u + defer_fill + (uint32_t)__popcll( md & ((1ull << lane) - 1ull) )] = i | ((uint32_t)s << 31);
                    defer_fill += (uint32_t)__popcll( md );
                }
            }
        }
        if (lane == 0) { tile_counts[tile] = tile_fill; if (DEFER) defer_counts[tile] = defer_fill; }
        if (COUNT)
        {
            uint32_t tot = valid ? sectors : 0u;
            #pragma unroll
            for (int d = 32; d > 0; d >>= 1) tot += (uint32_t)__shfl_xor( (int)tot, d );
            if (lane == 0 && tot) atomicAdd( sectors_out, (unsigned long long)tot );
        }
        V = Vn; e = en; e_valid = en_valid; qo = qon; c_pfw = n_pfw; c_rlen = n_rlen; c_seed = n_seed;
    }
}

constexpr uint32_t HEAVY_PER_LANE = 4u;
template <int BITS>
__global__ void __launch_bounds__(256)
fm_seed_heavy_kernel(const DevIndex f, const StringSetDev q, const uint32_t read_len, const uint32_t* __restrict__ list, const uint32_t* __restrict__ n_list,
                     uint64_t* __restrict__ keys_out, uint2* __restrict__ res_ranges, uint32_t* __restrict__ res_ids, const uint32_t res_cap,
                     unsigned int* __restrict__ counts)
{
    __shared__ uint32_t s_cnt[4][3], s_base[3];
    const uint32_t n = *n_list;
    const uint32_t lane = threadIdx.x & 63u, wave = threadIdx.x >> 6;
    const uint32_t len = q.fixed_len;
    const bool ragged = q.intervals != nullptr;
    DevIndex fplain = f; fplain.dtab = nullptr; fplain.dkmer = 0;
    const uint32_t chunk = 256u * HEAVY_PER_LANE;
    for (uint32_t c0 = blockIdx.x * chunk; c0 < n; c0 += gridDim.x * chunk)
    {
        uint32_t kind[HEAVY_PER_LANE], vx[HEAVY_PER_LANE], vy[HEAVY_PER_LANE], ent[HEAVY_PER_LANE];
        uint32_t nk = 0, nr0 = 0, nr1 = 0;
        #pragma unroll
        for (uint32_t u = 0; u < HEAVY_PER_LANE; ++u)
        {
            const uint32_t t = c0 + u * 256u + threadIdx.x;
            kind[u] = 0u; vx[u] = 1u; vy[u] = 0u; ent[u] = 0u;
            if (t < n)
            {
                ent[u] = list[t];
                const uint32_t i = ent[u] & 0x7FFFFFFFu, s = ent[u] >> 31;
                uint32_t rx, ry, nblk; bool single;
                match_one<BITS,false,true,true>( fplain, q, s ? (NVBIO_FM_SCAN_FORWARD | NVBIO_FM_COMPLEMENT) : 0u, f.ktab != nullptr, false, i, rx, ry, nblk, single );
                if (!single && rx == ry) { const uint32_t sv = f.ssa[rx]; rx = ry = (sv == 0xFFFFFFFFu) ? f.length : sv; single = true; }
                if (single)        { kind[u] = 1u; vx[u] = rx; ++nk; }
                else if (rx < ry)  { kind[u] = 2u + s; vx[u] = rx; vy[u] = ry; if (s) ++nr1; else ++nr0; }
            }
        }
        uint32_t pk = nk, p0 = nr0, p1 = nr1;
        #pragma unroll
        for (int d = 1; d < 64; d <<= 1)
        {
            const uint32_t a = (uint32_t)__shfl_up( (int)pk, d ), b = (uint32_t)__shfl_up( (int)p0, d ), c = (uint32_t)__shfl_up( (int)p1, d );
            if (lane >= (uint32_t)d) { pk += a; p0 += b; p1 += c; }
        }
        if (lane == 63u) { s_cnt[wave][0] = pk; s_cnt[wave][1] = p0; s_cnt[wave][2] = p1; }
        __syncthreads();
        if (threadIdx.x < 3u)
        {
            const uint32_t tot = s_cnt[0][threadIdx.x] + s_cnt[1][threadIdx.x] + s_cnt[2][threadIdx.x] + s_cnt[3][threadIdx.x];
            s_base[threadIdx.x] = tot ? atomicAdd( &counts[threadIdx.x], tot ) : 0u;
        }
        __syncthreads();
        uint32_t ok = s_base[0] + (pk - nk), o0 = s_base[1] + (p0 - nr0), o1 = s_base[2] + (p1 - nr1);
        for (uint32_t w = 0; w < wave; ++w) { ok += s_cnt[w][0]; o0 += s_cnt[w][1]; o1 += s_cnt[w][2]; }
        #pragma unroll
        for (uint32_t u = 0; u < HEAVY_PER_LANE; ++u)
        {
            const uint32_t i = ent[u] & 0x7FFFFFFFu, s = ent[u] >> 31;
            if (kind[u] == 1u)
            {
                const uint32_t rid = i / q.spr, j = i - rid * q.spr;
                uint32_t pq = j * (ragged ? q.intervals[rid] : q.interval);
                const uint32_t rlen = ragged ? q.offsets[rid + 1] - q.offsets[rid] : read_len;
                if (s) pq = rlen - pq - len;
                keys_out[ok++] = ((uint64_t)rid << 34) | ((uint64_t)s << 33) | ((uint64_t)vx[u] + 1024u - pq);
            }
            else if (kind[u] == 2u) { res_ranges[o0] = make_uint2( vx[u], vy[u] ); res_ids[o0] = i; ++o0; }
            else if (kind[u] == 3u) { res_ranges[res_cap + o1] = make_uint2( vx[u], vy[u] ); res_ids[res_cap + o1] = i; ++o1; }
        }
        __syncthreads();
    }
}

__global__ void __launch_bounds__(256)
fm_seed_defer_compact_kernel(const uint32_t* __restrict__ tile_defer, const uint32_t* __restrict__ defer_counts, const uint32_t* __restrict__ defer_offsets,
                             const uint32_t n_tiles, uint32_t* __restrict__ list, uint32_t* __restrict__ n_out)
{
    for (uint32_t tile = blockIdx.x * blockDim.x + threadIdx.x; tile < n_tiles; tile += gridDim.x * blockDim.x)
    {
        const uint32_t n = defer_counts[tile], off = defer_offsets[tile];
        const uint32_t* src = tile_defer + (uint64_t)tile * 128u;
        for (uint32_t k = 0; k < n; ++k) list[off + k] = src[k];
        if (tile == n_tiles - 1u) n_out[0] = off + n;
    }
}
```

### nvbio-gpl_amd/csrc/fm_index.hip

```cpp
#include "fm_device.h"
#include "fm_seed_device.h"
#include "seed_hits_device.h"
#include <hipcub/hipcub.hpp>
#include <new>
#include <stdlib.h>

namespace nvbio_amd {

struct FMIndexImpl
{
    int                  device;
    nvbio_fm_index_view  view;
    uint2*               ktab;
    uint32_t             kmer;
    uint2*               dtab;
    uint32_t             dkmer;
    uint2*               side;
    uint32_t             dmark, dctx;
    uint2*               ctab;
    uint2*               cside;
    uint32_t             ckmer;
    uint32_t             cwide;
    uint32_t             table_flags;
    bool                 owns_arrays;
    uint64_t             owned_bytes;
    uint32_t*            isa;
    uint32_t*            text;
    void*                planes;

    DevIndex dev() const
    {
        DevIndex d;
        d.length = view.length; d.primary = view.primary;
        d.L2_0 = view.L2[0]; d.L2_1 = view.L2[1]; d.L2_2 = view.L2[2]; d.L2_3 = view.L2[3]; d.L2_4 = view.L2[4];
        d.rec  = (const uint4*)view.bwt_occ_dev;
        d.ssa  = view.ssa_dev;
        d.sa_log = 0; while ((1u << d.sa_log) < (view.sa_int ? view.sa_int : 16u)) ++d.sa_log;
        d.ktab = ktab; d.kmer = kmer; d.dtab = dtab; d.dkmer = dkmer;
        d.side = side; d.dmark = dmark; d.dctx = dctx;
        d.isa = isa; d.text = text;
        d.ctab = ctab; d.cside = cside; d.ckmer = ckmer;
        return d;
    }
};

struct StringSetDev
{
    const void*     symbols;
    const uint32_t* offsets;
    uint32_t        ranges;
    uint32_t        fixed_len;
    uint32_t        stride;
    uint32_t        n;
    uint32_t        spr;
    uint32_t        interval;
    const uint32_t* intervals;
};

__device__ __forceinline__ bool string_bounds(const StringSetDev& q, const uint32_t i, uint32_t& begin, uint32_t& len)
{
    if (q.spr)
    {
        const uint32_t r = i / q.spr, j = i - r * q.spr;
        const uint32_t base = q.offsets ? q.offsets[r] : r * q.stride;
        begin = base + j * (q.intervals ? q.intervals[r] : q.interval);
        len   = q.fixed_len;
        if (q.intervals && begin + len > q.offsets[r + 1]) return false;
    }
    else if (q.offsets)
    {
        begin = q.offsets[i];
        len   = q.ranges ? q.offsets[i + 1] - begin : q.fixed_len;
    }
    else { begin = i * q.stride; len = q.fixed_len; }
    return true;
}

#ifndef NVB_NT_TABLE
#define NVB_NT_TABLE 1
#endif
constexpr bool NT_TABLE = NVB_NT_TABLE != 0;

struct SearchState
{
    uint32_t x, y, s;
    bool     have_pos;
    uint32_t tpos;
    bool     have_ctx;
    uint32_t ctx;
    bool     is_pos;
    uint32_t sectors;
};

__device__ __forceinline__ uint2 load_table_entry(const uint2* __restrict__ tab, const uint64_t key, const bool nt)
{
    if (nt && NT_TABLE)
    {
        const unsigned long long v = __builtin_nontemporal_load( (const unsigned long long*)tab + key );
        return make_uint2( (uint32_t)v, (uint32_t)(v >> 32) );
    }
    return tab[key];
}

template <class Sym>
__device__ __forceinline__ void direct_entry(const DevIndex& f, const uint2 e, Sym& sym, const uint32_t len, SearchState& st)
{
    if (e.y < f.dmark) { st.x = e.x; st.y = e.y; return; }
    if (e.x < f.dmark)
    {
        st.have_pos = true; st.tpos = e.x; st.x = st.y = 0u;
        st.have_ctx = f.dctx != 0u; st.ctx = e.y - f.dmark;
        return;
    }
    const uint32_t m  = e.y - f.dmark;
    const uint4*   g4 = (const uint4*)(f.side + 4ull * (e.x - f.dmark));
    st.sectors += 1u;
    const uint4 q0 = g4[0], q1 = g4[1];
    uint4 q2 = make_uint4( 0, 0, 0, 0 ), q3 = q2;
    if (m > 3u) { q2 = g4[2]; q3 = g4[3]; }
    const uint32_t r = len - st.s;
    st.x = q0.x; st.y = q0.y;
    if (r > f.dctx) return;
    uint32_t rest = 0; bool clean = true;
    for (uint32_t t = 0; t < r; ++t) { const uint32_t c = sym( st.s + t ); clean = clean && c < 4u; rest = (rest << 2) | (c & 3u); }
    if (!clean) { st.x = 1u; st.y = 0u; return; }
    uint32_t hits = 0, pos = 0;
#define NVB_SIDE_ROW(j, P, C) if ((j) <= m && context_matches( (P), (C) - f.dmark, rest, r )) { ++hits; pos = (P); }
    NVB_SIDE_ROW( 1u, q0.z, q0.w ) NVB_SIDE_ROW( 2u, q1.x, q1.y ) NVB_SIDE_ROW( 3u, q1.z, q1.w )
    NVB_SIDE_ROW( 4u, q2.x, q2.y ) NVB_SIDE_ROW( 5u, q2.z, q2.w ) NVB_SIDE_ROW( 6u, q3.x, q3.y ) NVB_SIDE_ROW( 7u, q3.z, q3.w )
#undef NVB_SIDE_ROW
    if (hits == 0u)      { st.x = 1u; st.y = 0u; }
    else if (hits == 1u) { st.x = st.y = pos - r; st.is_pos = true; st.s = len; }
}

template <bool COUNT, bool DIRECT, class Sym>
__device__ __forceinline__ void search_tail(const DevIndex& f, Sym& sym, const uint32_t len, const bool verify, SearchState& st, uint32_t& nblk)
{
    uint32_t x = st.x, y = st.y, s = st.s;
    if (st.is_pos) return;
    for (; s < len && x <= y && !st.have_pos; ++s)
    {
        if (DIRECT && x == y) break;
        if (verify && x == y && len - s >= 2u)
        {
            const uint32_t sv = f.ssa[x];
            const uint32_t p  = (sv == 0xFFFFFFFFu) ? f.length : sv;
            const uint32_t r  = len - s;
            const uint32_t full = (p >= r) ? f.isa[p - r] : 0u;
            SymbolReader<2> tr( f.text );
            uint32_t t = 0;
            while (t < r && t < p)
            {
                const uint32_t c = sym( s + t );
                if (c > 3u || c != tr.get( p - 1u - t )) break;
                ++t;
            }
            if (t == r)  { x = y = full; s = len; }
            else if (t)  { x = y = f.isa[p - t]; s += t; }
            if (s >= len) break;
        }
        const uint32_t c = sym( s );
        if (c > 3u) { x = 1u; y = 0u; break; }
        search_step<COUNT>( f, x, y, c, nblk, &st.sectors );
    }
    if (DIRECT && ((s < len && x == y) || st.have_pos))
    {
        uint32_t p = st.tpos;
        if (!st.have_pos)
        {
            const uint32_t sv = NT_TABLE ? __builtin_nontemporal_load( f.ssa + x ) : f.ssa[x];
            p = (sv == 0xFFFFFFFFu) ? f.length : sv;
            st.sectors += 1u;
        }
        const uint32_t r  = len - s;
        bool ok = (p >= r);
        if (ok && r > 0u)
        {
            const uint32_t w0 = (p - r) >> 4;
            if (st.have_pos && st.have_ctx && r <= f.dctx)
            {
                uint32_t rest = 0;
// ... 762 lines not shown
            {
                const uint32_t p = position( r[k].x );
                tab[e0 + k] = make_uint2( p, DTAB_MARK | left_context( text, p ) );
            }
            else if (c[k] >= 2u)
            {
                const uint32_t rows  = r[k].y - r[k].x + 1u;
                const uint32_t slots = c[k] == 2u ? 4u : 8u;
                const uint32_t idx4  = c[k] == 2u ? 2u * tot_large + ga++ : 2u * gb++;
                uint2* g = side + 4ull * idx4;
                g[0] = r[k];
                for (uint32_t j = 1; j < slots; ++j)
                {
                    uint2 v = make_uint2( 0u, DTAB_MARK );
                    if (j <= rows) { const uint32_t p = position( r[k].x + j - 1u ); v = make_uint2( p, DTAB_MARK | left_context( text, p ) ); }
                    g[j] = v;
                }
                tab[e0 + k] = make_uint2( DTAB_MARK | idx4, DTAB_MARK | rows );
            }
        }
    }
}

static nvbio_status build_direct_table(FMIndexImpl* idx, uint2* tab, const uint64_t entries, hipStream_t stream)
{
    const uint32_t length = idx->view.length;
    idx->side = nullptr; idx->dmark = 0xFFFFFFFFu; idx->dctx = 0;
    if ((uint64_t)length + 2u > DTAB_MARK || (idx->table_flags & NVBIO_FM_TABLE_NO_CONTEXT))
    {
        return NVB_LAUNCH( fm_dtab_kernel, dim3( grid_for( entries ) ), dim3(256), stream, tab, idx->view.ssa_dev, length, entries );
    }
    const uint32_t n_tiles = (uint32_t)((entries + DT_TILE - 1u) / DT_TILE);
    const dim3 grid( n_tiles < 256u * 64u ? n_tiles : 256u * 64u ), block( 256 );
    BuildBuffers bufs;
    uint32_t* cnt = nullptr; uint2* side = nullptr;
    size_t temp_bytes = 0;
    uint32_t tot_small = 0, tot_large = 0;
    const bool want_groups = !(idx->table_flags & NVBIO_FM_TABLE_NO_GROUPS);
    nvbio_status st = NVBIO_OK;
    if (want_groups)
    {
        cnt = bufs.alloc<uint32_t>( 4ull * n_tiles );
        if (!cnt) { set_error( "direct table: out of device memory" ); return NVBIO_ERR_NOMEM; }
        uint32_t *cs = cnt, *cl = cnt + n_tiles, *os = cnt + 2ull * n_tiles, *ol = cnt + 3ull * n_tiles;
        NVB_CHECK( NVB_LAUNCH( fm_dtab_count_kernel, grid, block, stream, (const uint2*)tab, entries, n_tiles, cs, cl ) );
        hipError_t e = hipcub::DeviceScan::ExclusiveSum( nullptr, temp_bytes, cs, os, (int)n_tiles, stream );
        void* temp = nullptr;
        if (e == hipSuccess && !(temp = bufs.alloc<uint8_t>( temp_bytes ))) e = hipErrorOutOfMemory;
        if (e == hipSuccess) e = hipcub::DeviceScan::ExclusiveSum( temp, temp_bytes, cs, os, (int)n_tiles, stream );
        if (e == hipSuccess) e = hipcub::DeviceScan::ExclusiveSum( temp, temp_bytes, cl, ol, (int)n_tiles, stream );
        uint32_t last[4] = { 0, 0, 0, 0 };
        if (e == hipSuccess) e = hipMemcpyAsync( &last[0], cs + n_tiles - 1u, 4, hipMemcpyDeviceToHost, stream );
        if (e == hipSuccess) e = hipMemcpyAsync( &last[1], os + n_tiles - 1u, 4, hipMemcpyDeviceToHost, stream );
        if (e == hipSuccess) e = hipMemcpyAsync( &last[2], cl + n_tiles - 1u, 4, hipMemcpyDeviceToHost, stream );
        if (e == hipSuccess) e = hipMemcpyAsync( &last[3], ol + n_tiles - 1u, 4, hipMemcpyDeviceToHost, stream );
        if (e == hipSuccess) e = hipStreamSynchronize( stream );
        if (e != hipSuccess) { (void)hipGetLastError(); set_error( "direct table: counting pass failed: %s", hipGetErrorString( e ) ); st = NVBIO_ERR_HIP; }
        tot_small = last[0] + last[1]; tot_large = last[2] + last[3];
        const uint64_t units = 2ull * tot_large + tot_small;
        if (st == NVBIO_OK && units > 0 && units < (1ull << 30))
            side = bufs.alloc<uint2>( units * 4u );
    }
    if (st == NVBIO_OK)
    {
        NVB_CHECK( NVB_LAUNCH( fm_dtab_fill_kernel, grid, block, stream, tab, entries, n_tiles, cnt ? cnt + 2ull * n_tiles : nullptr,
                               cnt ? cnt + 3ull * n_tiles : nullptr, tot_large, idx->view.ssa_dev, (const uint32_t*)idx->text, length, side ) );
        if (hipStreamSynchronize( stream ) != hipSuccess) { set_error( "direct table: fill pass failed" ); st = NVBIO_ERR_HIP; }
    }
    if (st != NVBIO_OK) return st;
    bufs.forget( side );
    idx->side = side; idx->dmark = DTAB_MARK; idx->dctx = DTAB_CTX;
    if (side) idx->owned_bytes += (2ull * tot_large + tot_small) * 32ull;
    return NVBIO_OK;
}

#include "fm_canon_inl.h"

static nvbio_status build_canonical_tables(FMIndexImpl* idx, uint32_t k, hipStream_t stream)
{
    const uint32_t kk = k - 1u;
    const uint64_t entries = 1ull << (2 * kk);
    BuildBuffers bufs;
    uint2* a = bufs.alloc<uint2>( entries );
    uint2* b = a ? bufs.alloc<uint2>( entries / 4 ) : nullptr;
    if (!b) { set_error( "k-mer table: out of device memory" ); return NVBIO_ERR_NOMEM; }
    uint2* cur = (kk % 2 == 0) ? a : b;
    uint2* oth = (kk % 2 == 0) ? b : a;
    DevIndex f = idx->dev(); f.ktab = nullptr; f.kmer = 0; f.dtab = nullptr; f.dkmer = 0;
    NVB_CHECK( NVB_LAUNCH( fm_ktab_root_kernel, dim3(1), dim3(1), stream, cur, idx->view.length ) );
    for (uint32_t j = 1; j <= kk; ++j)
    {
        const uint64_t n_next = 1ull << (2 * j);
        NVB_CHECK( NVB_LAUNCH( fm_ktab_level_kernel, dim3( grid_for( n_next ) ), dim3(256), stream, f, (const uint2*)cur, oth, n_next ) );
        uint2* t = cur; cur = oth; oth = t;
    }
    const bool ok = hipStreamSynchronize( stream ) == hipSuccess;
    bufs.release( b );
    if (!ok) { set_error( "k-mer table build failed" ); return NVBIO_ERR_HIP; }
    idx->ktab = a; idx->kmer = kk;
    idx->owned_bytes += entries * sizeof(uint2);
    const nvbio_status st = build_canonical_table( idx, k, (idx->table_flags & NVBIO_FM_TABLE_CANONICAL_WIDE) != 0, stream );
    if (st != NVBIO_OK) { idx->ktab = nullptr; idx->kmer = 0; return st; }
    bufs.forget( a );
    return NVBIO_OK;
}

static nvbio_status build_kmer_table(FMIndexImpl* idx, uint32_t k, hipStream_t stream)
{
    idx->ktab = nullptr; idx->kmer = 0; idx->dtab = nullptr; idx->dkmer = 0; idx->side = nullptr; idx->dmark = 0xFFFFFFFFu; idx->dctx = 0;
    idx->ctab = nullptr; idx->cside = nullptr; idx->ckmer = 0; idx->cwide = 0;
    if (k == 0) return NVBIO_OK;
    const bool direct = idx->text && idx->view.ssa_dev && idx->view.sa_int == 1 && k >= 2 && !(idx->table_flags & NVBIO_FM_TABLE_NO_DIRECT);
    if (idx->table_flags & (NVBIO_FM_TABLE_CANONICAL | NVBIO_FM_TABLE_CANONICAL_WIDE))
    {
        if (!direct || (k & 1u) == 0u || k < 3u)
        {
            set_error( "NVBIO_FM_TABLE_CANONICAL needs the full suffix array, the text (sa_int = 1) and an odd kmer_len >= 3" );
            return NVBIO_ERR_UNSUPPORTED;
        }
        return build_canonical_tables( idx, k, stream );
    }
    const uint64_t entries = 1ull << (2 * k);
    BuildBuffers bufs;
    uint2* a = bufs.alloc<uint2>( entries );
    uint2* b = a ? bufs.alloc<uint2>( entries / 4 ) : nullptr;
    if (!b) { set_error( "k-mer table: out of device memory" ); return NVBIO_ERR_NOMEM; }
    uint2* cur = (k % 2 == 0) ? a : b;
    uint2* oth = (k % 2 == 0) ? b : a;
    DevIndex f = idx->dev(); f.ktab = nullptr; f.kmer = 0; f.dtab = nullptr; f.dkmer = 0;
    NVB_CHECK( NVB_LAUNCH( fm_ktab_root_kernel, dim3(1), dim3(1), stream, cur, idx->view.length ) );
    for (uint32_t j = 1; j <= k; ++j)
    {
        const uint64_t n_next = 1ull << (2 * j);
        NVB_CHECK( NVB_LAUNCH( fm_ktab_level_kernel, dim3( grid_for( n_next ) ), dim3(256), stream, f, (const uint2*)cur, oth, n_next ) );
        uint2* t = cur; cur = oth; oth = t;
    }
    if (direct) NVB_CHECK( build_direct_table( idx, a, entries, stream ) );
    if (hipStreamSynchronize( stream ) != hipSuccess) { set_error( "k-mer table build failed" ); return NVBIO_ERR_HIP; }
    bufs.forget( a );
    if (direct)
    {
        bufs.forget( b );
        idx->ktab = b; idx->kmer = k - 1u; idx->dtab = a; idx->dkmer = k;
        idx->owned_bytes += (entries + entries / 4) * sizeof(uint2);
    }
    else
    {
        idx->ktab = a; idx->kmer = k;
        idx->owned_bytes += entries * sizeof(uint2);
    }
    return NVBIO_OK;
}

nvbio_status fm_index_adopt(const nvbio_fm_index_view* view, int device, uint32_t kmer_len, bool owns, hipStream_t stream, nvbio_fm_index_t* out,
                            uint32_t* isa, uint32_t* text, uint32_t table_flags)
{
    FMIndexImpl* idx = new (std::nothrow) FMIndexImpl;
    if (!idx) { set_error( "out of host memory" ); return NVBIO_ERR_NOMEM; }
    idx->device = device; idx->view = *view; idx->ktab = nullptr; idx->kmer = 0; idx->dtab = nullptr; idx->dkmer = 0; idx->isa = nullptr; idx->text = nullptr;
    idx->side = nullptr; idx->dmark = 0xFFFFFFFFu; idx->dctx = 0; idx->table_flags = table_flags;
    idx->ctab = nullptr; idx->cside = nullptr; idx->ckmer = 0; idx->cwide = 0;
    if (idx->view.sa_int == 0) idx->view.sa_int = 16;
    idx->owns_arrays = owns; idx->owned_bytes = owns ? (view->bwt_occ_words + view->ssa_words) * 4ull : 0ull;
    idx->isa = isa; idx->text = text;
    if (isa)  idx->owned_bytes += ((uint64_t)view->length + 1u) * 4ull;
    if (text) idx->owned_bytes += (((uint64_t)view->length + 15u) / 16u) * 4ull;
    idx->planes = nullptr;
    nvbio_status st = build_kmer_table( idx, kmer_len, stream );
    const bool tables = st == NVBIO_OK;
    if (st == NVBIO_OK && text && !(table_flags & NVBIO_FM_TABLE_NO_TEXT_PLANES))
    {
        uint64_t bytes = 0;
        (void)nvbio_text_planes_bytes( view->length, &bytes );
        if (hipMalloc( &idx->planes, bytes ) != hipSuccess) { idx->planes = nullptr; set_error( "out of device memory (text planes, %llu bytes)", (unsigned long long)bytes ); st = NVBIO_ERR_NOMEM; }
        else st = nvbio_text_planes_build( device, text, view->length, idx->planes, stream );
        if (st == NVBIO_OK && hipStreamSynchronize( stream ) != hipSuccess) { set_error( "text planes build failed" ); st = NVBIO_ERR_HIP; }
        if (st == NVBIO_OK) idx->owned_bytes += bytes;
    }
    if (st != NVBIO_OK)
    {
        if (idx->planes) (void)hipFree( idx->planes );
        if (tables)
        {
            if (idx->ktab)  (void)hipFree( idx->ktab );
            if (idx->dtab)  (void)hipFree( idx->dtab );
            if (idx->side)  (void)hipFree( idx->side );
            if (idx->ctab)  (void)hipFree( idx->ctab );
            if (idx->cside) (void)hipFree( idx->cside );
        }
        if (owns) { (void)hipFree( (void*)view->bwt_occ_dev ); (void)hipFree( (void*)view->ssa_dev ); }
        if (isa)  (void)hipFree( isa );
        if (text) (void)hipFree( text );
        delete idx;
        return st;
    }
    *out = (nvbio_fm_index_t)idx;
    return NVBIO_OK;
}

}

using namespace nvbio_amd;

nvbio_status nvbio_amd::fm_handle_dev(nvbio_fm_index_t index, DevIndex* d, int* device)
{
    NVB_REQUIRE( index != nullptr, "index is NULL" );
    const FMIndexImpl* idx = (const FMIndexImpl*)index;
    *d = idx->dev(); *device = idx->device;
    return NVBIO_OK;
}

extern "C" {

nvbio_status nvbio_fm_index_create(const nvbio_fm_index_view* view, int device, uint32_t kmer_len, void* stream, nvbio_fm_index_t* out)
{
    NVB_REQUIRE( view && out, "view/out is NULL" );
    NVB_REQUIRE( view->bwt_occ_dev != nullptr, "bwt_occ_dev is NULL" );
    NVB_REQUIRE( ((uintptr_t)view->bwt_occ_dev & 31u) == 0, "bwt_occ_dev must be 32-byte aligned" );
    NVB_REQUIRE( kmer_len <= 17, "kmer_len must be <= 17" );
    NVB_REQUIRE( view->L2[4] == view->length, "L2[4] must equal length" );
    const uint32_t K = view->sa_int ? view->sa_int : 16u;
    NVB_REQUIRE( K <= 64 && (K & (K - 1u)) == 0, "sa_int must be a power of two in [1,64]" );
    NVB_REQUIRE( view->primary <= view->length, "primary out of range" );
    const uint64_t need = 2ull * ((((uint64_t)view->length + 15u) / 16u + 3u) & ~3ull);
    NVB_REQUIRE( view->bwt_occ_words >= need, "bwt_occ_words too small for length" );
    NVB_REQUIRE( view->ssa_dev == nullptr || view->ssa_words >= (uint64_t)view->length / K + 1u, "ssa_words too small for length" );
    DeviceGuard g( device ); if (!g.ok) return NVBIO_ERR_NO_DEVICE;
    return fm_index_adopt( view, device, kmer_len, false, (hipStream_t)stream, out, nullptr, nullptr, 0u );
}

nvbio_status nvbio_fm_index_destroy(nvbio_fm_index_t index)
{
    if (!index) return NVBIO_OK;
    FMIndexImpl* idx = (FMIndexImpl*)index;
    DeviceGuard g( idx->device ); if (!g.ok) return NVBIO_ERR_NO_DEVICE;
    if (idx->ktab) (void)hipFree( idx->ktab );
    if (idx->dtab) (void)hipFree( idx->dtab );
    if (idx->side) (void)hipFree( idx->side );
    if (idx->ctab)  (void)hipFree( idx->ctab );
    if (idx->cside) (void)hipFree( idx->cside );
    if (idx->isa)  (void)hipFree( idx->isa );
    if (idx->text) (void)hipFree( idx->text );
    if (idx->planes) (void)hipFree( idx->planes );
    if (idx->owns_arrays) { (void)hipFree( (void*)idx->view.bwt_occ_dev ); (void)hipFree( (void*)idx->view.ssa_dev ); }
    delete idx;
    return NVBIO_OK;
}

nvbio_status nvbio_fm_index_get_view(nvbio_fm_index_t index, nvbio_fm_index_view* view)
{
    NVB_REQUIRE( index && view, "index/view is NULL" );
    *view = ((FMIndexImpl*)index)->view;
    return NVBIO_OK;
}

nvbio_status nvbio_fm_index_export(nvbio_fm_index_t index, uint32_t* bwt_occ_out_dev, uint32_t* ssa_out_dev, void* stream)
{
    NVB_REQUIRE( index != nullptr, "index is NULL" );
    FMIndexImpl* idx = (FMIndexImpl*)index;
    DeviceGuard g( idx->device ); if (!g.ok) return NVBIO_ERR_NO_DEVICE;
    if (bwt_occ_out_dev)
        NVB_HIP( hipMemcpyAsync( bwt_occ_out_dev, idx->view.bwt_occ_dev, idx->view.bwt_occ_words * 4ull, hipMemcpyDeviceToDevice, (hipStream_t)stream ) );
    if (ssa_out_dev && idx->view.ssa_dev)
        NVB_HIP( hipMemcpyAsync( ssa_out_dev, idx->view.ssa_dev, idx->view.ssa_words * 4ull, hipMemcpyDeviceToDevice, (hipStream_t)stream ) );
    return NVBIO_OK;
}

nvbio_status nvbio_fm_index_device_bytes(nvbio_fm_index_t index, uint64_t* bytes)
{
    NVB_REQUIRE( index && bytes, "index/bytes is NULL" );
    *bytes = ((FMIndexImpl*)index)->owned_bytes;
    return NVBIO_OK;
}

nvbio_status nvbio_fm_index_text_planes(nvbio_fm_index_t index, const void** planes_dev, uint32_t* length)
{
    NVB_REQUIRE( index && planes_dev && length, "index/planes_dev/length is NULL" );
    const FMIndexImpl* idx = (const FMIndexImpl*)index;
    *planes_dev = idx->planes;
    *length     = idx->planes ? idx->view.length : 0u;
    return NVBIO_OK;
}

nvbio_status nvbio_fm_match(nvbio_fm_index_t index, const nvbio_string_set* queries, uint32_t flags,
                            nvbio_uint2* ranges_dev, uint32_t* blocks_dev, void* stream)
{
    NVB_REQUIRE( index != nullptr, "index is NULL" );
    FMIndexImpl* idx = (FMIndexImpl*)index;
    StringSetDev q; NVB_CHECK( make_set( queries, &q ) );
    if (q.n == 0) return NVBIO_OK;
    NVB_REQUIRE( ranges_dev != nullptr, "ranges_dev is NULL" );
    NVB_REQUIRE( blocks_dev == nullptr || (flags & NVBIO_FM_NO_KMER_TABLE), "blocks_dev requires NVBIO_FM_NO_KMER_TABLE" );
    DeviceGuard g( idx->device ); if (!g.ok) return NVBIO_ERR_NO_DEVICE;
    const DevIndex f = idx->dev();
    const dim3 grid( grid_for( q.n ) ), block( 256 );
    hipStream_t s = (hipStream_t)stream;
    const bool use_table = (f.ktab != nullptr) && !(flags & NVBIO_FM_NO_KMER_TABLE);
    return with_value( SymbolBits(), queries->symbol_bits, [&](auto BITS)
    {
        if (blocks_dev) return NVB_LAUNCH( (fm_match_kernel<BITS,true,false>),  grid, block, s, f, q, flags, (uint2*)ranges_dev, blocks_dev, nullptr );
        if (use_table)  return NVB_LAUNCH( (fm_match_kernel<BITS,false,true>),  grid, block, s, f, q, flags, (uint2*)ranges_dev, blocks_dev, nullptr );
        return                 NVB_LAUNCH( (fm_match_kernel<BITS,false,false>), grid, block, s, f, q, flags, (uint2*)ranges_dev, blocks_dev, nullptr );
    }, bad_symbol_bits );
}

nvbio_status nvbio_fm_rank(nvbio_fm_index_t index, const uint32_t* rows_dev, const uint8_t* syms_dev, uint32_t n, uint32_t* out_dev, void* stream)
{
    NVB_REQUIRE( index != nullptr, "index is NULL" );
    if (n == 0) return NVBIO_OK;
    NVB_REQUIRE( rows_dev && syms_dev && out_dev, "NULL device pointer" );
    FMIndexImpl* idx = (FMIndexImpl*)index;
    DeviceGuard g( idx->device ); if (!g.ok) return NVBIO_ERR_NO_DEVICE;
    return NVB_LAUNCH( fm_rank_kernel, dim3( grid_for( n ) ), dim3(256), (hipStream_t)stream, idx->dev(), rows_dev, syms_dev, n, out_dev );
}

nvbio_status nvbio_fm_rank4(nvbio_fm_index_t index, const uint32_t* rows_dev, uint32_t n, uint32_t* out_dev, void* stream)
{
    NVB_REQUIRE( index != nullptr, "index is NULL" );
    if (n == 0) return NVBIO_OK;
    NVB_REQUIRE( rows_dev && out_dev, "NULL device pointer" );
    NVB_REQUIRE( ((uintptr_t)out_dev & 15u) == 0, "out_dev must be 16-byte aligned" );
    FMIndexImpl* idx = (FMIndexImpl*)index;
    DeviceGuard g( idx->device ); if (!g.ok) return NVBIO_ERR_NO_DEVICE;
    return NVB_LAUNCH( fm_rank4_kernel, dim3( grid_for( n ) ), dim3(256), (hipStream_t)stream, idx->dev(), rows_dev, n, (uint4*)out_dev );
}

static nvbio_status locate_common(nvbio_fm_index_t index, const uint32_t* rows_dev, uint32_t n, uint32_t* pos_dev, nvbio_uint2* jt_dev, void* stream)
{
    NVB_REQUIRE( index != nullptr, "index is NULL" );
    if (n == 0) return NVBIO_OK;
    NVB_REQUIRE( rows_dev && (pos_dev || jt_dev), "NULL device pointer" );
    FMIndexImpl* idx = (FMIndexImpl*)index;
    NVB_REQUIRE( jt_dev || idx->view.ssa_dev, "index has no sampled suffix array" );
    DeviceGuard g( idx->device ); if (!g.ok) return NVBIO_ERR_NO_DEVICE;
    if (pos_dev) NVB_CHECK( NVB_LAUNCH( fm_locate_kernel<0>, dim3( grid_for( n ) ), dim3(256), (hipStream_t)stream, idx->dev(), rows_dev, n, pos_dev, (uint2*)nullptr ) );
    else         NVB_CHECK( NVB_LAUNCH( fm_locate_kernel<1>, dim3( grid_for( n ) ), dim3(256), (hipStream_t)stream, idx->dev(), rows_dev, n, (uint32_t*)nullptr, (uint2*)jt_dev ) );
    return NVBIO_OK;
}

nvbio_status nvbio_fm_basic_inv_psi(nvbio_fm_index_t index, const uint32_t* rows_dev, uint32_t n, uint32_t* out_dev, void* stream)
{
    NVB_REQUIRE( index != nullptr, "index is NULL" );
    if (n == 0) return NVBIO_OK;
    NVB_REQUIRE( rows_dev && out_dev, "NULL device pointer" );
    FMIndexImpl* idx = (FMIndexImpl*)index;
    DeviceGuard g( idx->device ); if (!g.ok) return NVBIO_ERR_NO_DEVICE;
    return NVB_LAUNCH( fm_inv_psi_kernel, dim3( grid_for( n ) ), dim3(256), (hipStream_t)stream, idx->dev(), rows_dev, n, out_dev );
}

nvbio_status nvbio_fm_locate(nvbio_fm_index_t index, const uint32_t* rows_dev, uint32_t n, uint32_t* pos_dev, void* stream)
{
    NVB_REQUIRE( pos_dev != nullptr || n == 0, "pos_dev is NULL" );
    return locate_common( index, rows_dev, n, pos_dev, nullptr, stream );
}
nvbio_status nvbio_fm_locate_init(nvbio_fm_index_t index, const uint32_t* rows_dev, uint32_t n, nvbio_uint2* jt_dev, void* stream)
{
    NVB_REQUIRE( jt_dev != nullptr || n == 0, "jt_dev is NULL" );
    return locate_common( index, rows_dev, n, nullptr, jt_dev, stream );
}
nvbio_status nvbio_fm_locate_lookup(nvbio_fm_index_t index, const nvbio_uint2* jt_dev, uint32_t n, uint32_t* pos_dev, void* stream)
{
    NVB_REQUIRE( index != nullptr, "index is NULL" );
    if (n == 0) return NVBIO_OK;
    NVB_REQUIRE( jt_dev && pos_dev, "NULL device pointer" );
    FMIndexImpl* idx = (FMIndexImpl*)index;
    NVB_REQUIRE( idx->view.ssa_dev, "index has no sampled suffix array" );
    DeviceGuard g( idx->device ); if (!g.ok) return NVBIO_ERR_NO_DEVICE;
    return NVB_LAUNCH( fm_lookup_kernel, dim3( grid_for( n ) ), dim3(256), (hipStream_t)stream, idx->dev(), (const uint2*)jt_dev, n, pos_dev );
}

nvbio_status nvbio_fm_filter_scan(nvbio_fm_index_t index, const nvbio_uint2* ranges_dev, uint32_t n_queries,
                                  uint64_t* slots_dev, uint64_t* n_hits, void* stream)
{
    NVB_REQUIRE( index && n_hits, "NULL argument" );
    *n_hits = 0;
    if (n_queries == 0) return NVBIO_OK;
    NVB_REQUIRE( ranges_dev && slots_dev, "NULL device pointer" );
    FMIndexImpl* idx = (FMIndexImpl*)index;
    DeviceGuard g( idx->device ); if (!g.ok) return NVBIO_ERR_NO_DEVICE;
    hipStream_t s = (hipStream_t)stream;

    hipcub::TransformInputIterator<uint64_t, RangeSize, const uint2*> sizes( (const uint2*)ranges_dev, RangeSize() );
    size_t temp_bytes = 0;
    NVB_HIP( hipcub::DeviceScan::InclusiveSum( nullptr, temp_bytes, sizes, slots_dev, (int)n_queries, s ) );
    ScratchBlock temp;
    NVB_CHECK( temp.alloc( "fm_filter_scan", temp_bytes, s, "filter_scan: out of device memory" ) );
    const hipError_t e = hipcub::DeviceScan::InclusiveSum( temp.get(), temp_bytes, sizes, slots_dev, (int)n_queries, s );
    if (e != hipSuccess) { set_error( "filter_scan: scan failed: %s", hipGetErrorString( e ) ); return NVBIO_ERR_HIP; }
    NVB_HIP( hipMemcpyAsync( n_hits, slots_dev + (n_queries - 1), sizeof(uint64_t), hipMemcpyDeviceToHost, s ) );
    NVB_HIP( hipStreamSynchronize( s ) );
    return NVBIO_OK;
}

nvbio_status nvbio_fm_filter_rank(nvbio_fm_index_t index, const nvbio_string_set* queries, uint32_t flags,
                                  nvbio_uint2* ranges_dev, uint64_t* slots_dev, uint64_t* n_hits, void* stream)
{
    NVB_REQUIRE( index && queries && n_hits, "NULL argument" );
    *n_hits = 0;
    if (queries->n == 0) return NVBIO_OK;
    NVB_REQUIRE( ranges_dev && slots_dev, "NULL device pointer" );
    NVB_CHECK( nvbio_fm_match( index, queries, flags, ranges_dev, nullptr, stream ) );
    return nvbio_fm_filter_scan( index, ranges_dev, queries->n, slots_dev, n_hits, stream );
}

nvbio_status nvbio_fm_filter_locate(nvbio_fm_index_t index, const nvbio_uint2* ranges_dev, const uint64_t* slots_dev,
                                    uint32_t n_queries, uint64_t begin, uint64_t end, nvbio_uint2* hits_dev, void* stream)
{
    NVB_REQUIRE( index != nullptr, "index is NULL" );
    if (end <= begin) return NVBIO_OK;
    NVB_REQUIRE( ranges_dev && slots_dev && hits_dev, "NULL device pointer" );
    FMIndexImpl* idx = (FMIndexImpl*)index;
    NVB_REQUIRE( idx->view.ssa_dev, "index has no sampled suffix array" );
    DeviceGuard g( idx->device ); if (!g.ok) return NVBIO_ERR_NO_DEVICE;
    return NVB_LAUNCH( fm_filter_locate_kernel<false>, dim3( expand_grid( begin, end ) ), dim3(256), (hipStream_t)stream,
                       idx->dev(), (const uint2*)ranges_dev, slots_dev, n_queries, begin, end, (uint2*)hits_dev, (const uint8_t*)nullptr, DiagSpec{}, (uint64_t*)nullptr );
}

nvbio_status nvbio_fm_index_supports_direct(nvbio_fm_index_t index, int* yes)
{
    NVB_REQUIRE( index && yes, "index/yes is NULL" );
    FMIndexImpl* idx = (FMIndexImpl*)index;
    *yes = (idx->text && idx->view.ssa_dev && idx->view.sa_int == 1) ? 1 : 0;
    return NVBIO_OK;
}

nvbio_status nvbio_fm_match_direct(nvbio_fm_index_t index, const nvbio_string_set* queries, uint32_t flags,
                                   nvbio_uint2* ranges_dev, uint8_t* direct_dev, void* stream)
{
    NVB_REQUIRE( index != nullptr, "index is NULL" );
    FMIndexImpl* idx = (FMIndexImpl*)index;
    StringSetDev q; NVB_CHECK( make_set( queries, &q ) );
    if (q.n == 0) return NVBIO_OK;
    NVB_REQUIRE( ranges_dev && direct_dev, "NULL device pointer" );
    if (!(idx->text && idx->view.ssa_dev && idx->view.sa_int == 1))
// ... 55 lines not shown
        tile_offsets = c.take<uint32_t>( tl.n_tiles + 1u );
        scan_temp    = c.take<uint8_t>( scan_bytes );
        if (both)
        {
            tile_defer    = c.take<uint32_t>( (uint64_t)tl.n_tiles * 128u );
            defer_counts  = c.take<uint32_t>( tl.n_tiles + 1u );
            defer_offsets = c.take<uint32_t>( tl.n_tiles + 1u );
            defer_list    = c.take<uint32_t>( (uint64_t)tl.n_tiles * 128u );
            defer_n       = c.take<uint32_t>( 1 );
        }
    }
};

static nvbio_status seed_scratch_layout(const nvbio_string_set* seeds, bool both, SeedScratch* L)
{
    NVB_REQUIRE( seeds != nullptr, "seeds is NULL" );
    const uint32_t spr = seeds->seeds_per_string;
    NVB_REQUIRE( spr > 0, "the string set must enumerate seeds (seeds_per_string > 0)" );
    NVB_REQUIRE( seeds->n % spr == 0, "n must be a multiple of seeds_per_string" );
    NVB_REQUIRE( !both || spr <= 64u, "the two-strand seed pass takes at most 64 seeds per read" );
    L->both       = both;
    L->tl.reads   = seeds->n / spr;
    L->tl.rpt     = spr <= 64u ? 64u / spr : 1u;
    L->tl.n_tiles = (L->tl.reads + L->tl.rpt - 1u) / L->tl.rpt;
    L->slots      = both ? 128u : 64u * ((spr + 63u) / 64u);
    L->scan_bytes = 0;
    if (L->tl.n_tiles)
        NVB_HIP( hipcub::DeviceScan::ExclusiveSum( nullptr, L->scan_bytes, (const uint32_t*)nullptr, (uint32_t*)nullptr, (int)L->tl.n_tiles, (hipStream_t)0 ) );
    return NVBIO_OK;
}

nvbio_status nvbio_fm_match_seed_diagonals_temp_bytes(const nvbio_string_set* seeds, uint64_t* bytes)
{
    NVB_REQUIRE( bytes != nullptr, "bytes is NULL" );
    SeedScratch L; NVB_CHECK( seed_scratch_layout( seeds, false, &L ) );
    ScratchLayout c( nullptr, scratch_check_enabled() ); L.carve( c ); *bytes = c.bytes();
    return NVBIO_OK;
}

nvbio_status nvbio_fm_match_seed_diagonals(nvbio_fm_index_t index, const nvbio_string_set* seeds, uint32_t flags, uint32_t read_len,
                                           uint32_t strand, uint64_t* keys_dev, nvbio_uint2* residual_ranges_dev, uint32_t* residual_ids_dev,
                                           uint32_t* counts_dev, void* temp_dev, uint64_t temp_bytes, void* stream)
{
    NVB_REQUIRE( index != nullptr, "index is NULL" );
    FMIndexImpl* idx = (FMIndexImpl*)index;
    StringSetDev q; NVB_CHECK( make_set( seeds, &q ) );
    NVB_REQUIRE( counts_dev != nullptr, "counts_dev is NULL" );
    NVB_REQUIRE( q.spr > 0, "the string set must enumerate seeds (seeds_per_string > 0)" );
    NVB_REQUIRE( q.intervals == nullptr, "ragged seed sets (seed_intervals_dev) go through nvbio_fm_match_seed_diagonals_both" );
    NVB_REQUIRE( (uint64_t)(q.spr - 1u) * q.interval + q.fixed_len <= read_len, "seeds do not fit the read" );
    NVB_REQUIRE( q.fixed_len > 0, "empty seeds" );
    if (!(idx->text && idx->view.ssa_dev && idx->view.sa_int == 1))
    {
        set_error( "nvbio_fm_match_seed_diagonals needs the full suffix array and the text: build the index with sa_int = 1" );
        return NVBIO_ERR_UNSUPPORTED;
    }
    DeviceGuard g( idx->device ); if (!g.ok) return NVBIO_ERR_NO_DEVICE;
    hipStream_t s = (hipStream_t)stream;
    const bool count = (flags & NVBIO_FM_COUNT_SECTORS) != 0;
    NVB_REQUIRE( !count || ((uintptr_t)counts_dev & 7u) == 0, "counts_dev must be 8-byte aligned with NVBIO_FM_COUNT_SECTORS" );
    NVB_HIP( hipMemsetAsync( counts_dev, 0, (count ? 4 : 2) * sizeof(uint32_t), s ) );
    if (q.n == 0) return NVBIO_OK;
    NVB_REQUIRE( keys_dev && residual_ranges_dev && residual_ids_dev, "NULL device pointer" );
    SeedScratch L; NVB_CHECK( seed_scratch_layout( seeds, false, &L ) );
    ScratchBlock temp;
    NVB_CHECK( temp.alloc_layout( "fm_seed_pass", s, "seed pass: out of device memory for %llu bytes of scratch", [&](ScratchLayout& c) { L.carve( c ); },
                                  temp_dev, temp_bytes, "nvbio_fm_match_seed_diagonals_temp_bytes" ) );
    uint64_t* tile_keys = L.tile_keys; uint32_t* tile_counts = L.tile_counts;
    const DevIndex f = idx->dev();
    unsigned blocks = (L.tl.n_tiles + 3u) / 4u;
    const unsigned cap = (flags >> 16) ? (flags >> 16) * 64u : 256u * 64u;
    if (blocks > cap) blocks = cap;
    const dim3 grid( blocks ), block( 256 );
    const bool pipe = !count && !(flags & NVBIO_FM_NO_PIPELINE) && seeds->symbol_bits != 8 && q.spr <= 64u && q.fixed_len <= 32u && f.dtab != nullptr &&
                      f.ktab != nullptr && !(flags & NVBIO_FM_NO_KMER_TABLE) && f.dctx != 0u && q.fixed_len >= f.dkmer && q.fixed_len - f.dkmer <= f.dctx;
    NVB_CHECK( with_value( SymbolBits(), seeds->symbol_bits, [&](auto BITS)
    {
        if (pipe)  return NVB_LAUNCH( (fm_seed_pipe_kernel<(BITS == 8 ? 4 : BITS)>), grid, block, s, f, q, L.tl, flags & 0xFFFFu, read_len, strand, tile_keys, tile_counts,
                                      (uint2*)residual_ranges_dev, residual_ids_dev, (unsigned int*)counts_dev );
        if (count) return NVB_LAUNCH( (fm_seed_tiles_kernel<BITS,true>), grid, block, s, f, q, L.tl, flags & 0xFFFFu, read_len, strand, tile_keys, tile_counts,
                                      (uint2*)residual_ranges_dev, residual_ids_dev, (unsigned int*)counts_dev, (unsigned long long*)(counts_dev + 2) );
        return            NVB_LAUNCH( (fm_seed_tiles_kernel<BITS,false>), grid, block, s, f, q, L.tl, flags & 0xFFFFu, read_len, strand, tile_keys, tile_counts,
                                      (uint2*)residual_ranges_dev, residual_ids_dev, (unsigned int*)counts_dev, (unsigned long long*)nullptr );
    }, bad_symbol_bits ) );
    size_t scan_bytes = L.scan_bytes;
    const hipError_t e = hipcub::DeviceScan::ExclusiveSum( L.scan_temp, scan_bytes, (const uint32_t*)tile_counts, L.tile_offsets, (int)L.tl.n_tiles, s );
    if (e != hipSuccess) { set_error( "seed pass failed: %s", hipGetErrorString( e ) ); return NVBIO_ERR_HIP; }
    return NVB_LAUNCH( fm_seed_compact_kernel, dim3( grid_for( 4ull * L.tl.n_tiles ) ), block, s, (const uint64_t*)tile_keys, (const uint32_t*)tile_counts,
                       (const uint32_t*)L.tile_offsets, L.tl.n_tiles, L.slots, keys_dev, (unsigned int*)counts_dev, (unsigned int*)nullptr, (uint32_t*)nullptr );
}

int nvbio_fm_index_is_canonical(nvbio_fm_index_t index)
{
    return index != nullptr && ((FMIndexImpl*)index)->ctab != nullptr ? (int)((FMIndexImpl*)index)->ckmer : 0;
}

nvbio_status nvbio_fm_match_seed_diagonals_both_temp_bytes(const nvbio_string_set* seeds, uint64_t* bytes)
{
    NVB_REQUIRE( bytes != nullptr, "bytes is NULL" );
    SeedScratch L; NVB_CHECK( seed_scratch_layout( seeds, true, &L ) );
    ScratchLayout c( nullptr, scratch_check_enabled() ); L.carve( c ); *bytes = c.bytes();
    return NVBIO_OK;
}

nvbio_status nvbio_fm_match_seed_diagonals_both_keys_capacity(const nvbio_string_set* seeds, uint64_t* n_keys)
{
    NVB_REQUIRE( n_keys != nullptr, "n_keys is NULL" );
    SeedScratch L; NVB_CHECK( seed_scratch_layout( seeds, true, &L ) );
    *n_keys = 256ull * L.tl.n_tiles;
    return NVBIO_OK;
}

nvbio_status nvbio_fm_seed_tiles(const nvbio_string_set* seeds, uint32_t* reads_per_tile, uint32_t* n_tiles)
{
    NVB_REQUIRE( reads_per_tile && n_tiles, "NULL output pointer" );
    SeedScratch L; NVB_CHECK( seed_scratch_layout( seeds, true, &L ) );
    *reads_per_tile = L.tl.rpt; *n_tiles = L.tl.n_tiles;
    return NVBIO_OK;
}

nvbio_status nvbio_fm_match_seed_diagonals_both(nvbio_fm_index_t index, const nvbio_string_set* seeds, uint32_t flags, uint32_t read_len,
                                                uint64_t* keys_dev, nvbio_uint2* residual_ranges_dev, uint32_t* residual_ids_dev,
                                                uint32_t residual_capacity, uint32_t* counts_dev, void* temp_dev, uint64_t temp_bytes,
                                                void* stream)
{
    return nvbio_fm_match_seed_diagonals_both_tiled( index, seeds, flags, read_len, keys_dev, residual_ranges_dev, residual_ids_dev, residual_capacity,
                                                     counts_dev, nullptr, temp_dev, temp_bytes, stream );
}

nvbio_status nvbio_fm_match_seed_diagonals_both_tiled(nvbio_fm_index_t index, const nvbio_string_set* seeds, uint32_t flags, uint32_t read_len,
                                                      uint64_t* keys_dev, nvbio_uint2* residual_ranges_dev, uint32_t* residual_ids_dev,
                                                      uint32_t residual_capacity, uint32_t* counts_dev, uint32_t* tile_offsets_dev,
                                                      void* temp_dev, uint64_t temp_bytes, void* stream)
{
    NVB_REQUIRE( index != nullptr, "index is NULL" );
    FMIndexImpl* idx = (FMIndexImpl*)index;
    StringSetDev q; NVB_CHECK( make_set( seeds, &q ) );
    NVB_REQUIRE( counts_dev != nullptr, "counts_dev is NULL" );
    if (idx->ctab == nullptr)
    {
        set_error( "nvbio_fm_match_seed_diagonals_both needs the canonical table: build the index with NVBIO_FM_TABLE_CANONICAL" );
        return NVBIO_ERR_UNSUPPORTED;
    }
    NVB_REQUIRE( q.spr > 0 && q.spr <= 64u, "the string set must enumerate 1..64 seeds per read (seeds_per_string)" );
    NVB_REQUIRE( seeds->symbol_bits == 2 || seeds->symbol_bits == 4, "packed seeds (2 or 4 bits per symbol)" );
    NVB_REQUIRE( q.fixed_len >= idx->ckmer && q.fixed_len - idx->ckmer <= CTAB_FLANK, "seed length outside [kmer_len, kmer_len + 7]" );
    NVB_REQUIRE( q.intervals != nullptr || (uint64_t)(q.spr - 1u) * q.interval + q.fixed_len <= read_len, "seeds do not fit the read" );
    NVB_REQUIRE( residual_capacity >= q.n, "residual_capacity must be at least the number of seeds" );
    NVB_REQUIRE( q.n < (1u << 31), "at most 2^31 - 1 seeds per call (bit 31 of a seed id carries the strand)" );
    DeviceGuard g( idx->device ); if (!g.ok) return NVBIO_ERR_NO_DEVICE;
    hipStream_t s = (hipStream_t)stream;
    const bool count = (flags & NVBIO_FM_COUNT_SECTORS) != 0;
    const bool defer = (flags & NVBIO_FM_DEFER_HEAVY) != 0 && !count;
    NVB_REQUIRE( !count || ((uintptr_t)counts_dev & 7u) == 0, "counts_dev must be 8-byte aligned with NVBIO_FM_COUNT_SECTORS" );
    NVB_HIP( hipMemsetAsync( counts_dev, 0, (count ? 6 : 4) * sizeof(uint32_t), s ) );
    if (q.n == 0) return NVBIO_OK;
    NVB_REQUIRE( keys_dev && residual_ranges_dev && residual_ids_dev, "NULL device pointer" );
    SeedScratch L; NVB_CHECK( seed_scratch_layout( seeds, true, &L ) );
    ScratchBlock temp;
    NVB_CHECK( temp.alloc_layout( "fm_seed_pass_both", s, "seed pass: out of device memory for %llu bytes of scratch", [&](ScratchLayout& c) { L.carve( c ); },
                                  temp_dev, temp_bytes, "nvbio_fm_match_seed_diagonals_both_temp_bytes" ) );
    uint64_t* tile_keys = L.tile_keys; uint32_t* tile_counts = L.tile_counts; uint32_t* tile_defer = L.tile_defer; uint32_t* defer_counts = L.defer_counts;
    uint32_t* tile_offsets = tile_offsets_dev ? tile_offsets_dev : L.tile_offsets;
    const DevIndex f = idx->dev();
    unsigned blocks = (L.tl.n_tiles + 3u) / 4u;
    const unsigned cap = (flags >> 16) ? (flags >> 16) * 64u : 256u * 64u;
    if (blocks > cap) blocks = cap;
    const dim3 grid( blocks ), block( 256 );
    uint32_t inline_max = (flags >> 8) & 15u;
    inline_max = inline_max < 1u ? 1u : (inline_max > CTAB_INLINE ? CTAB_INLINE : inline_max);
    NVB_CHECK( with_value( Values<2, 4>(), seeds->symbol_bits, [&](auto BITS)
    {
        const auto launch = [&](auto CNT, auto W, auto D)
        {
            return NVB_LAUNCH( (fm_seed_both_kernel<BITS,CNT,W,D>), grid, block, s, f, q, L.tl, read_len, inline_max, tile_keys, tile_counts,
                               (uint2*)residual_ranges_dev, residual_ids_dev, residual_capacity, (unsigned int*)counts_dev,
                               CNT ? (unsigned long long*)(counts_dev + 4) : (unsigned long long*)nullptr, tile_defer, defer_counts );
        };
        const auto wide = [&](auto W)
        {
            if (count) return launch( std::true_type(),  W, std::false_type() );
            if (defer) return launch( std::false_type(), W, std::true_type() );
            return            launch( std::false_type(), W, std::false_type() );
        };
        return idx->cwide ? wide( std::true_type() ) : wide( std::false_type() );
    }, bad_symbol_bits ) );
    size_t scan_bytes = L.scan_bytes;
    hipError_t e = hipcub::DeviceScan::ExclusiveSum( L.scan_temp, scan_bytes, (const uint32_t*)tile_counts, tile_offsets, (int)L.tl.n_tiles, s );
    if (e == hipSuccess)
        NVB_CHECK( NVB_LAUNCH( fm_seed_compact_kernel, dim3( grid_for( 4ull * L.tl.n_tiles ) ), block, s, (const uint64_t*)tile_keys, (const uint32_t*)tile_counts,
                               (const uint32_t*)tile_offsets, L.tl.n_tiles, 128u, keys_dev, (unsigned int*)counts_dev, (unsigned int*)counts_dev + 3,
                               tile_offsets_dev ? tile_offsets_dev + L.tl.n_tiles : (uint32_t*)nullptr ) );
    if (e == hipSuccess && defer)
    {
        scan_bytes = L.scan_bytes;
        e = hipcub::DeviceScan::ExclusiveSum( L.scan_temp, scan_bytes, (const uint32_t*)defer_counts, L.defer_offsets, (int)L.tl.n_tiles, s );
        if (e == hipSuccess)
        {
            NVB_CHECK( NVB_LAUNCH( fm_seed_defer_compact_kernel, dim3( grid_for( L.tl.n_tiles ) ), block, s, (const uint32_t*)tile_defer, (const uint32_t*)defer_counts,
                                   (const uint32_t*)L.defer_offsets, L.tl.n_tiles, L.defer_list, L.defer_n ) );
            const uint64_t max_chunks = (128ull * L.tl.n_tiles + 256u * HEAVY_PER_LANE - 1u) / (256u * HEAVY_PER_LANE);
            const dim3 hgrid( (unsigned)(max_chunks < 4096u ? (max_chunks ? max_chunks : 1u) : 4096u) );
            if (seeds->symbol_bits == 2)
                NVB_CHECK( NVB_LAUNCH( (fm_seed_heavy_kernel<2>), hgrid, block, s, f, q, read_len, (const uint32_t*)L.defer_list, (const uint32_t*)L.defer_n, keys_dev,
                                       (uint2*)residual_ranges_dev, residual_ids_dev, residual_capacity, (unsigned int*)counts_dev ) );
            else
                NVB_CHECK( NVB_LAUNCH( (fm_seed_heavy_kernel<4>), hgrid, block, s, f, q, read_len, (const uint32_t*)L.defer_list, (const uint32_t*)L.defer_n, keys_dev,
                                       (uint2*)residual_ranges_dev, residual_ids_dev, residual_capacity, (unsigned int*)counts_dev ) );
        }
    }
    if (e != hipSuccess) { set_error( "seed pass failed: %s", hipGetErrorString( e ) ); return NVBIO_ERR_HIP; }
    return NVBIO_OK;
}

nvbio_status nvbio_fm_filter_locate_direct(nvbio_fm_index_t index, const nvbio_uint2* ranges_dev, const uint64_t* slots_dev,
                                           const uint8_t* direct_dev, uint32_t n_queries, uint64_t begin, uint64_t end,
                                           nvbio_uint2* hits_dev, void* stream)
{
    NVB_REQUIRE( index != nullptr, "index is NULL" );
    if (end <= begin) return NVBIO_OK;
    NVB_REQUIRE( ranges_dev && slots_dev && hits_dev && direct_dev, "NULL device pointer" );
    FMIndexImpl* idx = (FMIndexImpl*)index;
    NVB_REQUIRE( idx->view.ssa_dev, "index has no sampled suffix array" );
    DeviceGuard g( idx->device ); if (!g.ok) return NVBIO_ERR_NO_DEVICE;
    return NVB_LAUNCH( fm_filter_locate_kernel<false>, dim3( expand_grid( begin, end ) ), dim3(256), (hipStream_t)stream,
                       idx->dev(), (const uint2*)ranges_dev, slots_dev, n_queries, begin, end, (uint2*)hits_dev, direct_dev, DiagSpec{}, (uint64_t*)nullptr );
}

static nvbio_status filter_locate_diagonals(nvbio_fm_index_t index, const nvbio_uint2* ranges_dev, const uint64_t* slots_dev,
                                            const uint8_t* direct_dev, uint32_t n_queries, uint64_t begin, uint64_t end,
                                            uint32_t seeds_per_read, uint32_t seed_interval, uint32_t seed_len, uint32_t read_len,
                                            uint32_t strand, const uint32_t* query_ids_dev, const uint32_t* read_offsets_dev,
                                            const uint32_t* seed_intervals_dev, uint64_t* keys_dev, void* stream)
{
    NVB_REQUIRE( index != nullptr, "index is NULL" );
    if (end <= begin) return NVBIO_OK;
    NVB_REQUIRE( ranges_dev && slots_dev && keys_dev, "NULL device pointer" );
    NVB_REQUIRE( seeds_per_read > 0, "seeds_per_read must be positive" );
    NVB_REQUIRE( (read_offsets_dev == nullptr) == (seed_intervals_dev == nullptr), "ragged reads need both read_offsets_dev and seed_intervals_dev" );
    NVB_REQUIRE( read_offsets_dev != nullptr || (uint64_t)(seeds_per_read - 1u) * seed_interval + seed_len <= read_len, "seeds do not fit the read" );
    FMIndexImpl* idx = (FMIndexImpl*)index;
    NVB_REQUIRE( idx->view.ssa_dev, "index has no sampled suffix array" );
    DeviceGuard g( idx->device ); if (!g.ok) return NVBIO_ERR_NO_DEVICE;
    const DiagSpec ds = { seeds_per_read, seed_interval, seed_len, read_len, strand, query_ids_dev, read_offsets_dev, seed_intervals_dev };
    return NVB_LAUNCH( fm_filter_locate_kernel<true>, dim3( expand_grid( begin, end ) ), dim3(256), (hipStream_t)stream,
                       idx->dev(), (const uint2*)ranges_dev, slots_dev, n_queries, begin, end, (uint2*)nullptr, direct_dev, ds, keys_dev );
}

nvbio_status nvbio_fm_filter_locate_diagonals(nvbio_fm_index_t index, const nvbio_uint2* ranges_dev, const uint64_t* slots_dev,
                                              const uint8_t* direct_dev, uint32_t n_queries, uint64_t begin, uint64_t end,
                                              uint32_t seeds_per_read, uint32_t seed_interval, uint32_t seed_len, uint32_t read_len,
                                              uint32_t strand, const uint32_t* query_ids_dev, uint64_t* keys_dev, void* stream)
{
    return filter_locate_diagonals( index, ranges_dev, slots_dev, direct_dev, n_queries, begin, end, seeds_per_read, seed_interval, seed_len, read_len,
                                    strand, query_ids_dev, nullptr, nullptr, keys_dev, stream );
}

nvbio_status nvbio_fm_filter_locate_diagonals_ragged(nvbio_fm_index_t index, const nvbio_uint2* ranges_dev, const uint64_t* slots_dev,
                                                     const uint8_t* direct_dev, uint32_t n_queries, uint64_t begin, uint64_t end,
                                                     uint32_t seeds_per_read, uint32_t seed_len, const uint32_t* read_offsets_dev,
                                                     const uint32_t* seed_intervals_dev, uint32_t strand, const uint32_t* query_ids_dev,
                                                     uint64_t* keys_dev, void* stream)
{
    NVB_REQUIRE( read_offsets_dev && seed_intervals_dev, "read_offsets_dev and seed_intervals_dev are required" );
    return filter_locate_diagonals( index, ranges_dev, slots_dev, direct_dev, n_queries, begin, end, seeds_per_read, 0u, seed_len, 0u,
                                    strand, query_ids_dev, read_offsets_dev, seed_intervals_dev, keys_dev, stream );
}



nvbio_status nvbio_fm_residual_diagonals(nvbio_fm_index_t index, const nvbio_uint2* ranges_dev, const uint32_t* ids_dev, uint32_t n, uint32_t cap,
                                         uint32_t seeds_per_read, uint32_t seed_interval, uint32_t seed_len, uint32_t read_len,
                                         const uint32_t* read_offsets_dev, const uint32_t* seed_intervals_dev,
                                         uint64_t* keys_dev, uint32_t* n_keys_dev, void* stream)
{
    NVB_REQUIRE( index != nullptr && n_keys_dev != nullptr, "NULL argument" );
    FMIndexImpl* idx = (FMIndexImpl*)index;
    DeviceGuard g( idx->device ); if (!g.ok) return NVBIO_ERR_NO_DEVICE;
    hipStream_t s = (hipStream_t)stream;
    NVB_HIP( hipMemsetAsync( n_keys_dev, 0, sizeof(uint32_t), s ) );
    if (n == 0) return NVBIO_OK;
    NVB_REQUIRE( ranges_dev && ids_dev && keys_dev, "NULL device pointer" );
    NVB_REQUIRE( cap >= 1u && cap <= 64u, "cap must be in 1..64" );
    NVB_REQUIRE( (uint64_t)n * cap < (1ull << 31), "n * cap must stay below 2^31" );
    NVB_REQUIRE( seeds_per_read > 0, "seeds_per_read must be positive" );
    NVB_REQUIRE( (read_offsets_dev == nullptr) == (seed_intervals_dev == nullptr), "ragged reads need both read_offsets_dev and seed_intervals_dev" );
    if (!(idx->view.ssa_dev && idx->view.sa_int == 1))
    {
        set_error( "nvbio_fm_residual_diagonals needs the full suffix array: build the index with sa_int = 1" );
        return NVBIO_ERR_UNSUPPORTED;
    }
    size_t sort_bytes = 0;
    NVB_HIP( hipcub::DeviceRadixSort::SortPairs( nullptr, sort_bytes, (const uint32_t*)nullptr, (uint32_t*)nullptr, (const uint64_t*)nullptr, (uint64_t*)nullptr, (int)n, 0, 32, s ) );
    uint32_t* ids_s; uint64_t* rng_s; void* tmp;
    ScratchBlock aux;
    NVB_CHECK( aux.alloc_layout( "fm_residual_diagonals", s, "residual diagonals: out of device memory", [&](ScratchLayout& c)
                                 { ids_s = c.take<uint32_t>( n ); rng_s = c.take<uint64_t>( n ); tmp = c.take<uint8_t>( sort_bytes ); } ) );
    const hipError_t e = hipcub::DeviceRadixSort::SortPairs( tmp, sort_bytes, ids_dev, ids_s, (const uint64_t*)ranges_dev, rng_s, (int)n, 0, 32, s );
    if (e != hipSuccess) { set_error( "residual diagonals failed: %s", hipGetErrorString( e ) ); return NVBIO_ERR_HIP; }
    const DiagSpec ds = { seeds_per_read, seed_interval, seed_len, read_len, 0u, nullptr, read_offsets_dev, seed_intervals_dev };
    return NVB_LAUNCH( residual_locate_kernel, dim3( grid_for( n ) ), dim3(256), s, idx->dev(), (const uint2*)rng_s, (const uint32_t*)ids_s, n, cap, ds,
                       keys_dev, (unsigned int*)n_keys_dev );
}

nvbio_status nvbio_seed_hits_map_approx(nvbio_fm_index_t index, nvbio_fm_index_t reverse_index, const void* reads_dev, uint32_t read_bits,
                                        const uint32_t* read_queue_dev, uint32_t n_reads, const nvbio_seed_hits_params* p, nvbio_uint2* deques_dev,
                                        uint32_t* sizes_dev, uint8_t* reseed_dev, void* stream)
{
    NVB_REQUIRE( index && reverse_index && p, "NULL argument" );
    if (n_reads == 0) return NVBIO_OK;
    NVB_REQUIRE( reads_dev && deques_dev && sizes_dev, "NULL device pointer" );
    NVB_REQUIRE( read_bits == 2 || read_bits == 4 || read_bits == 8, "read_bits must be 2, 4 or 8" );
    NVB_REQUIRE( p->max_hits > 0 && p->seeds_per_read > 0 && p->seed_len > 0, "max_hits, seeds_per_read and seed_len must be positive" );
    NVB_REQUIRE( (uint64_t)p->first_offset + (uint64_t)(p->seeds_per_read - 1u) * p->seed_interval + p->seed_len <= p->read_len, "seeds do not fit the read" );
    NVB_REQUIRE( p->read_len < 1024u, "SeedHit keeps the seed position in 10 bits (seed_hit.h:217)" );
    FMIndexImpl *fi = (FMIndexImpl*)index, *ri = (FMIndexImpl*)reverse_index;
    NVB_REQUIRE( fi->device == ri->device, "both indices must live on one device" );
    const uint64_t worst = 4ull * p->seeds_per_read * (3ull * ((p->seed_len + 1u) / 2u) + 1ull);
    const uint32_t cap = (uint32_t)((worst < p->max_hits ? worst : p->max_hits) + 1u);
    DeviceGuard g( fi->device ); if (!g.ok) return NVBIO_ERR_NO_DEVICE;
    DevIndex f = fi->dev(), rf = ri->dev();
    const dim3 grid( grid_for( n_reads, 128 ) ), block( 128 );
    return with_value( SymbolBits(), read_bits, [&](auto BITS)
    {
        return NVB_LAUNCH( (fm_map_approx_kernel<BITS>), grid, block, (hipStream_t)stream, f, rf, reads_dev, read_queue_dev, n_reads,
                           p->seeds_per_read, p->first_offset, p->seed_interval, p->seed_len, p->read_len, p->max_hits, p->rep_seeds, cap,
                           (uint2*)deques_dev, sizes_dev, reseed_dev );
    }, bad_symbol_bits );
}

nvbio_status nvbio_seed_hits_approx_capacity(uint32_t seeds_per_read, uint32_t seed_len, uint32_t max_hits, uint32_t* capacity)
{
    NVB_REQUIRE( capacity != nullptr, "capacity is NULL" );
    const uint64_t worst = 4ull * seeds_per_read * (3ull * ((seed_len + 1u) / 2u) + 1ull);
    *capacity = (uint32_t)((worst < max_hits ? worst : max_hits) + 1u);
    return NVBIO_OK;
}
// ... 3 lines not shown
```

### nvbio-gpl_amd/pipeline.py

```python
import math

import numpy as np

from . import (ALN_RAGGED_READS, FM_COMPLEMENT, FM_SCAN_FORWARD, LOCAL, READ_COMPLEMENT, READ_REVERSE, SCORE_MIN, SEMI_GLOBAL, AlignmentBatch,
               BatchedBandedAlignmentScore, FMIndexFilter, GotohAligner, GotohScheme, HitQueues, PackedStringSet, RaggedSeedLayout, SeedHitsParams,
               best_approx_init_ragged, read_queue_begin_ragged, score_reduce_effort, score_reduce_effort_ragged, score_stream_flatten, score_stream_output,
               seed_hits_loc, seed_hits_map, seed_hits_map_ragged, seed_hits_select)


class SeedExtendParams:
    def __init__(self, seed_len=22, seed_interval=None, band=31, aln_type=LOCAL, scheme=None, min_score=None,
                 max_seed_hits=None):
        self.seed_len = seed_len
        self.seed_interval = seed_interval
        self.band = band
        self.aln_type = aln_type
        self.scheme = scheme or GotohScheme(2, 2, 6, -8, -3, -8, -3)
        self.min_score = min_score
        self.max_seed_hits = max_seed_hits
        self.direct = True
        self.fused_seed_pass = True
        self.mapq = False
        self.mapq_version = 2
        self.merge_strands = True
        self.algo_flags = 0
        self.defer_heavy = True
        self.fused_finish = True

    @classmethod
    def end_to_end(cls, constant_quality=True, **kw):
        scheme = GotohScheme(0, 6, 6, -8, -3, -8, -3) if constant_quality else GotohScheme(0, 2, 6, -8, -3, -8, -3)
        p = cls(aln_type=SEMI_GLOBAL, scheme=scheme, **kw)
        p.e2e = True
        return p

    def interval_for(self, read_len):
        return self.seed_interval or int(1 + 1.15 * math.sqrt(read_len))

    def min_score_for(self, read_len):
        if self.min_score is not None:
            return self.min_score
        if getattr(self, "e2e", False):
            return int(np.float32(-0.6) + np.float32(-0.6) * np.float32(read_len))
        return int(np.float32(0.0) + np.float32(10.0) * np.float32(math.log(np.float32(read_len))))

    def interval_table(self, max_len):
        if self.seed_interval:
            return np.full(max_len + 1, self.seed_interval, dtype=np.int32)
        x = np.arange(max_len + 1, dtype=np.float32)
        return np.maximum((np.float32(1.0) + np.float32(1.15) * np.sqrt(x)).astype(np.int32), 1)

    def min_score_table(self, max_len):
        return np.array([self.min_score_for(max(l, 1)) for l in range(max_len + 1)], dtype=np.int32)


class ReadBatch:

    def __init__(self, reads4, n_reads, read_len, quals=None, offsets=None):
        self.reads4, self.n, self.read_len, self.quals = reads4, int(n_reads), int(read_len), quals
        self.offsets = offsets


def _batch_geometry(torch, fmi, reads, params):
    dev = fmi.device
    R, M, L = reads.n, reads.read_len, params.seed_len
    S_int = params.interval_for(M)
    spr = (M - L) // S_int + 1
    ragged = reads.offsets is not None
    intervals = min_scores = None
    if ragged:
        cache = getattr(reads, "_ragged", None)
        if cache is None or cache[0] is not params:
            lens = (reads.offsets[1:] - reads.offsets[:-1]).to(torch.int64)
            itab = params.interval_table(M)
            it = torch.from_numpy(itab).to(dev)
            mt = torch.from_numpy(params.min_score_table(M)).to(dev)
            spr_max = max(((l - L) // int(itab[l]) + 1) if l >= L else 0 for l in range(M + 1))
            cache = reads._ragged = (params, it[lens].contiguous(), mt[lens].contiguous(), int(spr_max))
        _, intervals, min_scores, spr = cache
        qs = PackedStringSet(reads.reads4, 4, R * spr, offsets=reads.offsets, fixed_len=L, stride=0, device=dev, seeds_per_string=spr,
                             seed_intervals=intervals)
        read_off = reads.offsets
    else:
        qs = PackedStringSet(reads.reads4, 4, R * spr, fixed_len=L, stride=M, device=dev, seeds_per_string=spr,
                             seed_interval=S_int)
        read_off = getattr(reads, "_read_off", None)
        if read_off is None:
            read_off = reads._read_off = torch.arange(R + 1, device=dev, dtype=torch.int32) * M
    return dict(S_int=S_int, spr=spr, ragged=ragged, intervals=intervals, min_scores=min_scores, qs=qs, read_off=read_off)


def seed_pass_begin(fmi, reads, params, slot=0, timers=None, stream=None, after=None):
    import torch
    if stream is not None:
        if after is not None:
            stream.wait_event(after)
        with torch.cuda.stream(stream):
            return seed_pass_begin(fmi, reads, params, slot, timers)
    geo = _batch_geometry(torch, fmi, reads, params)
    bufs = getattr(fmi, "_seed_bufs2", None)
    if bufs is None:
        bufs = fmi._seed_bufs2 = {}
    b = bufs.setdefault(slot, {})
    ev_t = None
    if timers is not None:
        a, ev_t = torch.cuda.Event(enable_timing=True), torch.cuda.Event(enable_timing=True)
        timers.setdefault("match_both", []).append((a, ev_t))
        a.record()
    fmi.match_seed_diagonals_both(geo["qs"], reads.read_len, b, inline_hits=min(4, params.max_seed_hits or 4), defer_heavy=params.defer_heavy,
                                  grid_blocks=int(getattr(params, "seed_grid_blocks", 0) or 0))
    if ev_t is not None:
        ev_t.record()
    if "host" not in b:
        b["host"] = torch.empty(4, dtype=torch.int32, pin_memory=True)
    b["host"].copy_(b["counts"][:4], non_blocking=True)
    ev = torch.cuda.Event()
    ev.record()
    return dict(b=b, ev=ev, reads=reads)


SCORE_BIAS = 1 << 20


def pack_best_key(torch, scores, rc, pos):
    s = torch.clamp(scores.to(torch.int64) + SCORE_BIAS, min=0)
    return (s << 34) | (rc.to(torch.int64) << 33) | pos.to(torch.int64)


def seed_and_extend(fmi, genome2, genome_len, reads, params, timers=None, return_windows=False, extras=None, pre=None):
    import torch
    from . import (FinishStatus, best_candidate_reduce, best_candidate_unpack, best_candidate_windows, diagonals_to_windows, finish_reads, mapq,
                   second_candidate_reduce)
    dev = fmi.device
    R, M, L = reads.n, reads.read_len, params.seed_len
    geo = _batch_geometry(torch, fmi, reads, params)
    S_int, spr, ragged, intervals, min_scores, qs, read_off = (geo[k] for k in ("S_int", "spr", "ragged", "intervals", "min_scores", "qs", "read_off"))

    def tick(name):
        if timers is None:
            return None
        a, b = torch.cuda.Event(enable_timing=True), torch.cuda.Event(enable_timing=True)
        timers.setdefault(name, []).append((a, b))
        a.record()
        return b

    def tock(b):
        if b is not None:
            b.record()

    ext_flags = (params.algo_flags or 0) | (ALN_RAGGED_READS if ragged else 0)
    text_planes = fmi.text_planes_of(genome2, genome_len)
    aligner = GotohAligner(params.aln_type, params.scheme)
    top = None
    finish = None

    def extend(keys, tag):
        nonlocal top
        if finish is None and top is None:
            top = torch.zeros((R,), dtype=torch.int64, device=dev)
        e = tick("windows" + tag)
        rid, flags, wb, we = diagonals_to_windows(keys, params.band, M, genome_len, read_offsets=read_off if ragged else None)
        tock(e)
        e = tick("extend" + tag)
        batch = AlignmentBatch(reads.reads4, 4, read_off, genome2, 2, wb, we, quals=reads.quals, read_id=rid,
                               flags=flags, device=dev, max_read_len=M, algo_flags=ext_flags or None, text_planes=text_planes)
        scores, sinks = BatchedBandedAlignmentScore(params.band, aligner).enact(batch)
        tock(e)
        if finish is not None:
            scored.append((keys, scores, sinks, wb))
            return None
        e = tick("reduce")
        best_candidate_reduce(keys, scores, sinks, wb, top)
        tock(e)
        if params.mapq or return_windows:
            scored.append((keys, scores, sinks, wb))
        return None

    use_direct = params.direct and fmi.supports_direct()
    results, n_cand, scored = [], 0, []
    fused = use_direct and params.fused_seed_pass

    def residual_keys(ranges, ids, strand):
        if params.max_seed_hits is not None and params.max_seed_hits <= 64 and use_direct and ids.numel() * params.max_seed_hits < 2 ** 31 \
                and getattr(params, "one_call_residuals", True):
            if strand:
                ids = ids ^ -2 ** 31
            rk, nk = fmi.residual_diagonals(ranges.contiguous(), ids.contiguous(), params.max_seed_hits, spr, S_int, L, M,
                                            read_offsets=read_off if ragged else None, seed_intervals=intervals)
            return rk[:int(nk.item())]
        if params.max_seed_hits is not None:
            x = ranges[:, 0].to(torch.int64) & 0xFFFFFFFF
            y = ranges[:, 1].to(torch.int64) & 0xFFFFFFFF
            ycap = torch.minimum(y, x + (params.max_seed_hits - 1))
            ranges = torch.stack([ranges[:, 0], torch.where(ycap >= 2 ** 31, ycap - 2 ** 32, ycap).to(torch.int32)], dim=1).contiguous()
        flt = FMIndexFilter()
        n_hits = flt.rank_ranges(fmi, ranges.contiguous(), None)
        rkeys = flt.locate_diagonals(0, n_hits, spr, S_int, L, M, strand, query_ids=ids.contiguous(),
                                     read_offsets=read_off if ragged else None, seed_intervals=intervals)
        rkeys = torch.unique_consecutive(rkeys)
        if rkeys.numel() > 2 * R:
            rkeys = torch.unique(rkeys)
        return rkeys

    ck = fmi.canonical_kmer if fused else 0
    both = fused and ck and ck <= L <= ck + 7 and spr <= 64 and getattr(params, "two_strand_pass", True)
    if ragged and fused and not both:
        fused = False
    if both:
        if pre is None:
            pre = seed_pass_begin(fmi, reads, params, 0, timers)
        assert pre["reads"] is reads
        b = pre["b"]
        pre["ev"].synchronize()
        FinishStatus.of(dev).check()
        n_keys, n_rf, n_rr = int(b["host"][0]), int(b["host"][1]), int(b["host"][2])
        if params.mapq and getattr(params, "fused_finish", True) and n_keys and n_rf == 0 and n_rr == 0 and int(b["host"][3]) == n_keys:
            finish = (b["tile_offsets"], b["reads_per_tile"])
        parts = [b["keys"][:n_keys]]
        if n_rf or n_rr:
            e = tick("locate")
            parts.append(residual_keys(torch.cat([b["ranges"][:n_rf], b["ranges"][qs.n:qs.n + n_rr]]),
                                       torch.cat([b["ids"][:n_rf], b["ids"][qs.n:qs.n + n_rr] | -2 ** 31]), 0))
            tock(e)
        keys = parts[0] if len(parts) == 1 else torch.cat(parts)
        n_cand += keys.numel()
        if keys.numel():
            results.append(extend(keys, ""))
    elif fused:
        bufs = getattr(fmi, "_seed_bufs", None)
        if bufs is None:
            bufs = fmi._seed_bufs = ({}, {})
        pending = []
        for strand, flags in ((0, 0), (1, FM_SCAN_FORWARD | FM_COMPLEMENT)):
            b = bufs[strand]
            e = tick("match_fw" if strand == 0 else "match_rc")
            fmi.match_seed_diagonals(qs, flags, M, strand, b)
            tock(e)
            if "host" not in b:
                b["host"] = torch.empty(2, dtype=torch.int32, pin_memory=True)
            b["host"].copy_(b["counts"][:2], non_blocking=True)
            ev = torch.cuda.Event()
            ev.record()
            pending.append((strand, b, ev))
        merged = []
        for strand, b, ev in pending:
            ev.synchronize()
            n_keys, n_res = int(b["host"][0]), int(b["host"][1])
            keys = b["keys"][:n_keys]
            if n_res:
                e = tick("locate")
                keys = torch.cat([keys, residual_keys(b["ranges"][:n_res], b["ids"][:n_res], strand)])
                tock(e)
            if keys.numel() == 0:
                continue
            n_cand += keys.numel()
            if params.merge_strands:
                merged.append(keys)
            else:
                results.append(extend(keys, "_rc" if strand else "_fw"))
        if merged:
            results.append(extend(merged[0] if len(merged) == 1 else torch.cat(merged), ""))
    for strand, flags in (() if fused else ((0, 0), (1, FM_SCAN_FORWARD | FM_COMPLEMENT))):
        flt = FMIndexFilter()
# ... 653 lines not shown
```

Measured before the change: 2.028 billion.

## Add seed-locus line table to settle non-anchor seeds by direct text comparison

Builds a per-index table of 128-byte lines. Each line holds bit-planes of the reference text plus a bitmap marking positions whose seed occurs exactly once on both strands. In the seed-matching kernel, the anchor seed of each read is looked up in the canonical table as before. When its hit is unique, the other seeds of that read are checked against the reference at the implied position with a single line load, instead of each doing its own canonical-table and group lookups. This adds a pipelined locus stage to the seed loop, extra device memory for the table, and a build step at index creation, and it is enabled by default when the seed length matches.

```diff
diff --git a/include/nvbio_amd.h b/include/nvbio_amd.h
--- a/include/nvbio_amd.h
+++ b/include/nvbio_amd.h
@@ -65,6 +65,7 @@
     NVBIO_FM_TABLE_NO_GROUPS  = 4,
     NVBIO_FM_TABLE_CANONICAL_WIDE = 16,
     NVBIO_FM_TABLE_NO_TEXT_PLANES = 32,
+    NVBIO_FM_TABLE_NO_SEED_LOCUS = 64,
     NVBIO_FM_TABLE_CANONICAL  = 8
 };
 
@@ -84,6 +85,11 @@
 nvbio_status nvbio_text_planes_bytes(uint32_t length, uint64_t* bytes);
 nvbio_status nvbio_text_planes_build(int device, const uint32_t* text2_dev, uint32_t length, void* planes_dev, void* stream);
 nvbio_status nvbio_fm_index_text_planes(nvbio_fm_index_t index, const void** planes_dev, uint32_t* length);
+
+nvbio_status nvbio_seed_locus_bytes(uint32_t length, uint64_t* bytes);
+nvbio_status nvbio_seed_locus_build(nvbio_fm_index_t index, uint32_t seed_len, void* lines_dev, void* stream);
+nvbio_status nvbio_fm_index_seed_locus(nvbio_fm_index_t index, const void** lines_dev, uint32_t* seed_len);
+nvbio_status nvbio_fm_index_build_seed_locus(nvbio_fm_index_t index, uint32_t seed_len, void* stream);
 
 typedef struct
 {
@@ -160,6 +166,8 @@
 
 #define NVBIO_FM_INLINE_HITS(h) (((uint32_t)(h) & 15u) << 8)
 #define NVBIO_FM_DEFER_HEAVY 64u
+#define NVBIO_FM_NO_SEED_LOCUS 128u
+#define NVBIO_FM_COUNT_LOCUS 4096u
 nvbio_status nvbio_fm_match_seed_diagonals_both_temp_bytes(const nvbio_string_set* seeds, uint64_t* bytes);
 nvbio_status nvbio_fm_match_seed_diagonals_both_keys_capacity(const nvbio_string_set* seeds, uint64_t* n_keys);
 nvbio_status nvbio_fm_match_seed_diagonals_both(nvbio_fm_index_t index, const nvbio_string_set* seeds, uint32_t flags, uint32_t read_len,
diff --git a/nvbio-gpl_amd/__init__.py b/nvbio-gpl_amd/__init__.py
--- a/nvbio-gpl_amd/__init__.py
+++ b/nvbio-gpl_amd/__init__.py
@@ -12,6 +12,8 @@
 FM_SCAN_FORWARD, FM_COMPLEMENT, FM_NO_KMER_TABLE, FM_NO_VERIFY, FM_COUNT_SECTORS, FM_NO_PIPELINE, FM_DEFER_HEAVY = 1, 2, 4, 8, 16, 32, 64
 FM_TABLE_NO_DIRECT, FM_TABLE_NO_CONTEXT, FM_TABLE_NO_GROUPS, FM_TABLE_CANONICAL, FM_TABLE_CANONICAL_WIDE = 1, 2, 4, 8, 16
 FM_TABLE_NO_TEXT_PLANES = 32
+FM_TABLE_NO_SEED_LOCUS = 64
+FM_NO_SEED_LOCUS, FM_COUNT_LOCUS = 128, 4096
 READ_REVERSE, READ_COMPLEMENT = 1, 2
 TRACEBACK_SINKS_GIVEN = 1
 ALN_NO_UNGAPPED_SCORE, ALN_NO_THIRD_CHANCE, ALN_NO_PACKED_DP, ALN_FORCE_PACKED_DP, ALN_NO_UNGAPPED_TRACEBACK, ALN_PK_THREE_WAVES = 1, 2, 4, 8, 16, 32
@@ -20,6 +22,7 @@
 ALN_SPLIT_CHANCES, ALN_NO_PAIRED_GAP_CHANCE = 131072, 262144
 ALN_NO_NARROW_DP = 524288
 ALN_NO_TEXT_PLANES = 1048576
+SEED_NO_LOCUS = 2097152
 ROUTE_SETTLED, ROUTE_FULL_BAND, ROUTE_CLASS_A, ROUTE_CLASS_B, ROUTE_REDONE = 0, 1, 2, 3, 8
 DEFAULT_ALGO_FLAGS = 0
 BACKTRACK_REFERENCE_QUIRKS = 1
@@ -305,6 +308,18 @@
         p, n = ctypes.c_void_p(), ctypes.c_uint32()
         _check(lib().nvbio_fm_index_text_planes(self._h, ctypes.byref(p), ctypes.byref(n)))
         return (p.value, n.value) if p.value else None
+
+    def seed_locus(self):
+        p, n = ctypes.c_void_p(), ctypes.c_uint32()
+        _check(lib().nvbio_fm_index_seed_locus(self._h, ctypes.byref(p), ctypes.byref(n)))
+        return (p.value, n.value) if p.value else None
+
+    def build_seed_locus(self, seed_len, out=None):
+        if out is None:
+            _check(lib().nvbio_fm_index_build_seed_locus(self._h, ctypes.c_uint32(seed_len), _stream_ptr(self.device)))
+            return None
+        _check(lib().nvbio_seed_locus_build(self._h, ctypes.c_uint32(seed_len), _ptr(out), _stream_ptr(self.device)))
+        return out
 
     def text_planes_of(self, text2, length):
         tp = self._text_planes if self._h is not None else None
@@ -391,7 +406,7 @@
             buffers["keys"] = torch.empty(max(int(cap.value), 1), dtype=torch.int64, device=self.device)
             buffers["ranges"] = torch.empty((2 * n, 2), dtype=torch.int32, device=self.device)
             buffers["ids"] = torch.empty(2 * n, dtype=torch.int32, device=self.device)
-            buffers["counts"] = torch.empty(6, dtype=torch.int32, device=self.device)
+            buffers["counts"] = torch.zeros(10, dtype=torch.int32, device=self.device)
             nb = ctypes.c_uint64(0)
             _check(lib().nvbio_fm_match_seed_diagonals_both_temp_bytes(ctypes.byref(qs), ctypes.byref(nb)))
             buffers["temp"] = torch.empty(nb.value, dtype=torch.uint8, device=self.device)
@@ -1031,6 +1046,12 @@
                       ctypes.c_void_p(self.text_planes.data_ptr() if hasattr(self.text_planes, "data_ptr") else self.text_planes))
 
 
+def seed_locus_bytes(length):
+    b = ctypes.c_uint64()
+    _check(lib().nvbio_seed_locus_bytes(ctypes.c_uint32(length), ctypes.byref(b)))
+    return b.value
+
+
 def text_planes_bytes(length):
     b = ctypes.c_uint64()
     _check(lib().nvbio_text_planes_bytes(ctypes.c_uint32(length), ctypes.byref(b)))
diff --git a/nvbio-gpl_amd/csrc/bitplanes.h b/nvbio-gpl_amd/csrc/bitplanes.h
--- a/nvbio-gpl_amd/csrc/bitplanes.h
+++ b/nvbio-gpl_amd/csrc/bitplanes.h
@@ -166,6 +166,38 @@
     }
 }
 
+constexpr uint32_t SEED_LOCUS_LINE_BYTES = 128u;
+constexpr uint32_t SEED_LOCUS_UNITS      = 5u;
+constexpr uint32_t SEED_LOCUS_MAX_READ   = 193u;
+inline __host__ __device__ uint64_t seed_locus_lines(const uint32_t n) { return ((uint64_t)n >> 7) + 1u; }
+
+struct LocusUnits { uint64_t lo0, hi0, u0, lo1, hi1; };
+
+__device__ __forceinline__ void load_locus_units(const void* __restrict__ lines, const uint32_t base, const uint32_t x, LocusUnits& out)
+{
+    static_assert( 127u + SEED_LOCUS_MAX_READ - 1u <= 64u * SEED_LOCUS_UNITS - 1u, "the last symbol of a read lies in the line its first symbol lies in" );
+    static_assert( 24u * SEED_LOCUS_UNITS <= SEED_LOCUS_LINE_BYTES, "a line holds its units" );
+    const uint32_t line = base >> 7, unit = (x - (line << 7)) >> 6;
+    const uint64_t* __restrict__ p = (const uint64_t*)lines + (size_t)line * 16u;
+    const uint32_t next = unit + 1u < SEED_LOCUS_UNITS ? unit + 1u : unit;
+    out.lo0 = p[3u * unit]; out.hi0 = p[3u * unit + 1u]; out.u0 = p[3u * unit + 2u];
+    out.lo1 = p[3u * next]; out.hi1 = p[3u * next + 1u];
+}
+
+__device__ __forceinline__ uint64_t squeeze2_64(const uint64_t v)
+{
+    return (uint64_t)squeeze2( (uint32_t)v ) | ((uint64_t)squeeze2( (uint32_t)(v >> 32) ) << 16);
+}
+
+__device__ __forceinline__ bool locus_answers(const LocusUnits& lu, const uint32_t x, const uint32_t len, const uint64_t T)
+{
+    const uint32_t s = x & 63u;
+    const uint64_t lo = s ? (lu.lo0 >> s) | (lu.lo1 << (64u - s)) : lu.lo0;
+    const uint64_t hi = s ? (lu.hi0 >> s) | (lu.hi1 << (64u - s)) : lu.hi0;
+    const uint64_t mask = (1ull << len) - 1ull;
+    return ((((lo ^ squeeze2_64( T )) | (hi ^ squeeze2_64( T >> 1 ))) & mask) == 0ull) && ((lu.u0 >> s) & 1ull);
+}
+
 template <typename W>
 __device__ __forceinline__ void text_planes224(const W& tw, const uint32_t tb, uint64_t (&tlo)[4], uint64_t (&thi)[4])
 {
diff --git a/nvbio-gpl_amd/csrc/fm_canon_inl.h b/nvbio-gpl_amd/csrc/fm_canon_inl.h
--- a/nvbio-gpl_amd/csrc/fm_canon_inl.h
+++ b/nvbio-gpl_amd/csrc/fm_canon_inl.h
@@ -182,12 +182,188 @@
     return NVBIO_OK;
 }
 
-template <int BITS, bool COUNT, bool WIDE, bool DEFER>
+__device__ __forceinline__ bool canon_row_hit(const uint32_t P, const uint32_t C, const uint32_t qo, const uint32_t want, const uint32_t fshift,
+                                              const uint32_t r, const uint32_t len, const uint32_t length, bool& rev, uint32_t& v)
+{
+    const uint32_t pay = C - DTAB_MARK;
+    const uint32_t o = (pay >> 28) & 1u;
+    const uint32_t flank = qo ? (pay & 0x3FFFu) : ((pay >> 14) & 0x3FFFu);
+    if ((flank >> fshift) != want) return false;
+    rev = (o ^ qo) != 0u;
+    if (rev ? ((uint64_t)P + len > length) : (P < r)) return false;
+    v = rev ? P : P - r;
+    return true;
+}
+
+__device__ __forceinline__ uint4 canon_entry(const DevIndex& f, const uint64_t V, const uint32_t len, const bool wide, uint32_t& qo)
+{
+    const uint32_t k = f.ckmer;
+    const uint64_t key = V >> (2u * (len - k));
+    qo = (uint32_t)(key >> k) & 1u;
+    const uint64_t idx = canon_index( qo ? canon_revcomp( key, k ) : key, k );
+    if (wide) return ((const uint4*)f.ctab)[idx];
+    const uint2 e = f.ctab[idx];
+    return make_uint4( e.x, e.y, 0u, 0u );
+}
+
+struct CanonHits { uint32_t nf, nr, vf, vr; };
+__device__ __forceinline__ bool canon_lookup(const DevIndex& f, const uint64_t V, const uint32_t len, const uint32_t qo, const uint4 e, CanonHits& h)
+{
+    const uint32_t r = len - f.ckmer, rmask = (1u << (2u * r)) - 1u, fshift = 2u * (CTAB_FLANK - r);
+    h.nf = h.nr = h.vf = h.vr = 0u;
+    if (e.y < DTAB_MARK) return e.x > e.y;
+    const uint32_t rest = (uint32_t)V & rmask, want = qo ? (~rest & rmask) : rest;
+    auto row = [&](const uint32_t P, const uint32_t C) {
+        bool rev; uint32_t v;
+        if (!canon_row_hit( P, C, qo, want, fshift, r, len, f.length, rev, v )) return;
+        h.nr += rev ? 1u : 0u; h.vr = rev ? v : h.vr;
+        h.nf += rev ? 0u : 1u; h.vf = rev ? h.vf : v;
+    };
+    if (e.x < DTAB_MARK) { row( e.x, e.y ); if (e.w >= DTAB_MARK) row( e.z, e.w ); }
+    else
+    {
+        const uint32_t m = e.y - DTAB_MARK;
+        const uint4* g4 = (const uint4*)(f.cside + 4ull * (e.x - DTAB_MARK));
+        #pragma unroll
+        for (uint32_t t = 0; t < CTAB_ROWS_MAX; t += 2u)
+            if (t < m) { const uint4 g = g4[t >> 1]; row( g.x, g.y ); if (t + 1u < m) row( g.z, g.w ); }
+    }
+    return true;
+}
+
+__global__ void __launch_bounds__(256)
+seed_locus_kernel(const DevIndex f, const uint32_t len, const uint32_t wide, const uint64_t n_units, const uint64_t n_lines, uint64_t* __restrict__ lines)
+{
+    const uint32_t lane = threadIdx.x & 63u, n = f.length;
+    for (uint64_t unit = (uint64_t)blockIdx.x * 4u + (threadIdx.x >> 6); unit < n_units; unit += (uint64_t)gridDim.x * 4u)
+    {
+        const uint64_t x64 = unit * 64u + lane;
+        const uint32_t sym = x64 < n ? text_symbol( f.text, (uint32_t)x64 ) : 0u;
+        bool uq = false;
+        if (x64 + len <= n)
+        {
+            const uint32_t x = (uint32_t)x64;
+            uint64_t V; uint32_t qo; CanonHits h;
+            (void)seed_bits_from_words<2>( load_seed_words<2>( f.text, x, len ), x, len, false, false, V );
+            uint4 e = canon_entry( f, V, len, wide != 0u, qo );
+            uq = canon_lookup( f, V, len, qo, e, h ) && h.nf == 1u && h.nr == 0u && h.vf == x;
+            if (uq)
+            {
+                const uint64_t R = canon_revcomp( V, len );
+                e  = canon_entry( f, R, len, wide != 0u, qo );
+                uq = canon_lookup( f, R, len, qo, e, h ) && h.nf == 0u && h.nr == 1u && h.vr == x;
+            }
+        }
+        const uint64_t ub = __ballot( uq ), lo = __ballot( (sym & 1u) != 0u ), hi = __ballot( (sym & 2u) != 0u );
+        if (lane < 3u && (unit >> 1) >= lane)
+        {
+            const uint64_t L = (unit >> 1) - lane, slot = unit - 2u * L;
+            if (L < n_lines && slot < SEED_LOCUS_UNITS) { uint64_t* p = lines + L * 16u + 3u * slot; p[0] = lo; p[1] = hi; p[2] = ub; }
+        }
+    }
+}
+
+template <int BITS, bool COUNT, bool WIDE, typename Geom, typename Entry, typename Resolve>
+__device__ __forceinline__ void fm_seed_locus_loop(const DevIndex& f, const StringSetDev& q, const SeedTiles& tl, const void* __restrict__ locus,
+                                                   unsigned long long* __restrict__ sectors_out, unsigned int* __restrict__ routes, const uint32_t tile0,
+                                                   const uint32_t lane, const uint32_t lr, const uint32_t j, const bool lane_ok,
+                                                   const Geom& seed_geom, const Entry& entry_of, const Resolve& resolve_tile)
+{
+    const uint32_t n_waves = gridDim.x * 4u;
+    const uint32_t k = f.ckmer, len = q.fixed_len, n = f.length;
+    const uint32_t anchor = lane - j;
+    const uint4 none = make_uint4( 1u, 0u, 0u, 0u );
+    auto qo_of = [&](const uint64_t V) -> uint32_t { return (uint32_t)(V >> (2u * (len - k) + k)) & 1u; };
+    auto add = [&](unsigned int* word, const bool on) {
+        const uint32_t c = (uint32_t)__popcll( __ballot( on ) );
+        if (lane == 0 && c) atomicAdd( word, c );
+    };
+    SeedWords W = { 0, 0, 0, 0, 0 }; uint32_t w_begin = 0, w_pfw = 0, w_rlen = 0; bool w_seed = false;
+    uint64_t aV = 0; uint4 ae = none; bool a_seed = false, a_ok = false; uint32_t a_pfw = 0, a_rlen = 0;
+    uint64_t lV = 0; uint4 le = none; bool l_seed = false, l_ok = false; uint32_t l_pfw = 0, l_rlen = 0;
+    bool l_asked = false, l_usable = false; uint32_t l_x = 0, l_strand = 0; LocusUnits LU = { 0, 0, 0, 0, 0 };
+    uint64_t cV = 0; uint4 ce = none; bool c_seed = false, c_ok = false; uint32_t c_pfw = 0, c_rlen = 0;
+    uint32_t c_settled = 0, c_x = 0;
+    for (uint32_t step = 0; ; ++step)
+    {
+        const uint64_t t4 = (uint64_t)tile0 + (uint64_t)step * n_waves;
+        if (step >= 4u && t4 - 4ull * n_waves >= tl.n_tiles) break;
+        uint32_t settled = 0;
+        if (l_asked && locus_answers( LU, l_x, len, l_strand ? canon_revcomp( lV, len ) : lV )) settled = 1u + l_strand;
+        if (COUNT && routes)
+        {
+            add( routes + 1, settled != 0u );
+            add( routes + 2, l_seed && j != 0u && l_usable && !settled );
+            add( routes + 3, l_seed && j != 0u && !l_usable );
+        }
+        uint32_t a_hit = 0xFFFFFFFFu, a_strand = 0;
+        if (j == 0u && a_ok)
+        {
+            CanonHits h;
+            if (canon_lookup( f, aV, len, qo_of( aV ), ae, h ) && h.nf + h.nr == 1u) { a_strand = h.nr; a_hit = h.nr ? h.vr : h.vf; }
+        }
+        const uint32_t r_hit = (uint32_t)__shfl( (int)a_hit, (int)anchor ), r_strand = (uint32_t)__shfl( (int)a_strand, (int)anchor );
+        const bool usable = r_hit != 0xFFFFFFFFu;
+        bool ask = false; uint32_t x = 0, base = 0;
+        if (usable && j != 0u && a_ok && a_rlen <= SEED_LOCUS_MAX_READ)
+        {
+            if (r_strand == 0u) { base = r_hit; x = r_hit + a_pfw; ask = (uint64_t)r_hit + a_pfw + len <= n; }
+            else
+            {
+                const uint32_t span = a_rlen - len;
+                base = r_hit >= span ? r_hit - span : 0u; x = r_hit - a_pfw; ask = r_hit >= a_pfw;
+            }
+        }
+        if (COUNT)
+        {
+            if (routes) add( routes, j == 0u && usable );
+            const uint64_t asked = __ballot( ask );
+            const uint64_t mine = (q.spr >= 64u ? ~0ull : ((1ull << q.spr) - 1ull)) << anchor;
+            const uint32_t c = (uint32_t)__popcll( __ballot( j == 0u && (asked & mine) != 0ull ) );
+            if (lane == 0 && c) atomicAdd( sectors_out, (unsigned long long)c );
+        }
+        uint64_t nV = 0; bool n_ok = false;
+        const bool n_seed = w_seed; const uint32_t n_pfw = w_pfw, n_rlen = w_rlen;
+        if (w_seed) n_ok = seed_bits_from_words<BITS>( W, w_begin, len, false, false, nV );
+        const bool is_one   = c_ok && ce.y >= DTAB_MARK && ce.x < DTAB_MARK;
+        const bool is_group = c_ok && ce.y >= DTAB_MARK && ce.x >= DTAB_MARK;
+        const bool is_heavy = c_ok && ce.y < DTAB_MARK && ce.x <= ce.y;
+        uint4 q0 = make_uint4( 0, 0, 0, 0 ), q1 = q0, q2 = q0, q3 = q0;
+        if (is_group)
+        {
+            const uint4* g4 = (const uint4*)(f.cside + 4ull * (ce.x - DTAB_MARK));
+            q0 = g4[0]; q1 = g4[1];
+            if (ce.y - DTAB_MARK > 4u) { q2 = g4[2]; q3 = g4[3]; }
+        }
+        uint4 fe = (j == 0u) ? le : none;
+        if (l_ok && j != 0u && !settled) { uint32_t qo; fe = entry_of( lV, qo ); }
+        LocusUnits nLU = { 0, 0, 0, 0, 0 };
+        if (ask) load_locus_units( locus, base, x, nLU );
+        uint4 ne = none;
+        if (j == 0u && n_ok) { uint32_t qo; ne = entry_of( nV, qo ); }
+        {
+            const uint64_t rid4 = t4 * tl.rpt + lr;
+            w_seed = t4 < tl.n_tiles && lane_ok && rid4 < tl.reads;
+            if (w_seed) w_seed = seed_geom( (uint32_t)rid4, w_begin, w_pfw, w_rlen );
+            if (w_seed) W = load_seed_words<BITS>( q.symbols, w_begin, len );
+        }
+        if (step >= 4u)
+        {
+            const uint32_t tile = (uint32_t)(t4 - 4ull * n_waves), rid = tile * tl.rpt + lr;
+            resolve_tile( tile, rid, c_seed, cV, ce, c_ok, qo_of( cV ), c_pfw, c_rlen, is_one, is_group, is_heavy, q0, q1, q2, q3, c_settled, c_x );
+        }
+        cV = lV; ce = fe; c_seed = l_seed; c_ok = l_ok; c_pfw = l_pfw; c_rlen = l_rlen; c_settled = settled; c_x = l_x;
+        lV = aV; le = ae; l_seed = a_seed; l_ok = a_ok; l_pfw = a_pfw; l_rlen = a_rlen; l_asked = ask; l_usable = usable; l_x = x; l_strand = r_strand; LU = nLU;
+        aV = nV; ae = ne; a_seed = n_seed; a_ok = n_ok; a_pfw = n_pfw; a_rlen = n_rlen;
+    }
+}
+
+template <int BITS, bool COUNT, bool WIDE, bool DEFER, bool LOCUS>
 __global__ void __launch_bounds__(256)
 fm_seed_both_kernel(const DevIndex f, const StringSetDev q, const SeedTiles tl, const uint32_t read_len, const uint32_t inline_max,
                     uint64_t* __restrict__ tile_keys, uint32_t* __restrict__ tile_counts, uint2* __restrict__ res_ranges,
                     uint32_t* __restrict__ res_ids, const uint32_t res_cap, unsigned int* __restrict__ counts, unsigned long long* __restrict__ sectors_out,
-                    uint32_t* __restrict__ tile_defer, uint32_t* __restrict__ defer_counts)
+                    uint32_t* __restrict__ tile_defer, uint32_t* __restrict__ defer_counts, const void* __restrict__ locus, unsigned int* __restrict__ routes)
 {
     const uint32_t lane = threadIdx.x & 63u;
     const uint32_t n_waves = gridDim.x * 4u;
@@ -220,69 +396,17 @@
         return make_uint4( e.x, e.y, 0u, 0u );
     };
 
-    uint32_t tile = blockIdx.x * 4u + (threadIdx.x >> 6);
-    if (tile >= tl.n_tiles) return;
-    SeedWords W = { 0, 0, 0, 0, 0 }; uint32_t w_begin = 0, w_pfw = 0, w_rlen = 0; bool w_valid = false;
-    uint64_t V = 0; uint4 e = make_uint4( 1u, 0u, 0u, 0u ); bool e_valid = false; uint32_t qo = 0, c_pfw = 0, c_rlen = 0; bool c_seed = false;
-    {
-        const uint32_t rid = tile * tl.rpt + lr;
-        if (lane_ok && rid < tl.reads)
-        {
-            uint32_t b0;
-            c_seed = seed_geom( rid, b0, c_pfw, c_rlen );
-            if (c_seed)
-            {
-                const SeedWords W0 = load_seed_words<BITS>( q.symbols, b0, len );
-                e_valid = seed_bits_from_words<BITS>( W0, b0, len, false, false, V );
-                if (e_valid) e = entry_of( V, qo );
-            }
-        }
-        const uint32_t t1 = tile + n_waves, rid1 = t1 * tl.rpt + lr;
-        if (t1 < tl.n_tiles && lane_ok && rid1 < tl.reads)
-        {
-            w_valid = seed_geom( rid1, w_begin, w_pfw, w_rlen );
-            if (w_valid) W = load_seed_words<BITS>( q.symbols, w_begin, len );
-        }
-    }
-    for (; tile < tl.n_tiles; tile += n_waves)
-    {
-        const uint32_t rid = tile * tl.rpt + lr;
-        const bool valid = lane_ok && rid < tl.reads && c_seed;
-        const bool is_one   = e_valid && e.y >= DTAB_MARK && e.x < DTAB_MARK;
-        const bool is_group = e_valid && e.y >= DTAB_MARK && e.x >= DTAB_MARK;
-        const bool is_heavy = e_valid && e.y < DTAB_MARK && e.x <= e.y;
-        uint4 q0 = make_uint4( 0, 0, 0, 0 ), q1 = q0, q2 = q0, q3 = q0;
+    auto resolve_tile = [&](const uint32_t tile, const uint32_t rid, const bool valid, const uint64_t V, const uint4 e, const bool e_valid, const uint32_t qo,
+                            const uint32_t c_pfw, const uint32_t c_rlen, const bool is_one, const bool is_group, const bool is_heavy,
+                            const uint4 q0, const uint4 q1, const uint4 q2, const uint4 q3, const uint32_t settled, const uint32_t settled_x)
+    {
         const uint32_t m = e.y - DTAB_MARK;
-        if (is_group)
-        {
-            const uint4* g4 = (const uint4*)(f.cside + 4ull * (e.x - DTAB_MARK));
-            q0 = g4[0]; q1 = g4[1];
-            if (m > 4u) { q2 = g4[2]; q3 = g4[3]; }
-        }
-        uint64_t Vn = 0; uint4 en = make_uint4( 1u, 0u, 0u, 0u ); bool en_valid = false; uint32_t qon = 0;
-        const uint32_t n_pfw = w_pfw, n_rlen = w_rlen; const bool n_seed = w_valid;
-        if (w_valid)
-        {
-            en_valid = seed_bits_from_words<BITS>( W, w_begin, len, false, false, Vn );
-            if (en_valid) en = entry_of( Vn, qon );
-        }
-        {
-            const uint32_t t2 = tile + 2u * n_waves, rid2 = t2 * tl.rpt + lr;
-            w_valid = t2 < tl.n_tiles && lane_ok && rid2 < tl.reads;
-            if (w_valid) w_valid = seed_geom( rid2, w_begin, w_pfw, w_rlen );
-            if (w_valid) W = load_seed_words<BITS>( q.symbols, w_begin, len );
-        }
         const uint32_t rest = (uint32_t)V & rmask;
         const uint32_t want = qo ? (~rest & rmask) : rest;
         uint32_t hits[2] = { 0, 0 }, pos[2][CTAB_INLINE] = { { 0, 0, 0, 0 }, { 0, 0, 0, 0 } };
         auto row = [&](const uint32_t P, const uint32_t C) {
-            const uint32_t pay = C - DTAB_MARK;
-            const uint32_t o = (pay >> 28) & 1u;
-            const uint32_t flank = qo ? (pay & 0x3FFFu) : ((pay >> 14) & 0x3FFFu);
-            if ((flank >> fshift) != want) return;
-            const bool rev = (o ^ qo) != 0u;
-            if (rev ? ((uint64_t)P + len > f.length) : (P < r)) return;
-            const uint32_t v = rev ? P : P - r;
+            bool rev; uint32_t v;
+            if (!canon_row_hit( P, C, qo, want, fshift, r, len, f.length, rev, v )) return;
             #pragma unroll
             for (int s = 0; s < 2; ++s)
                 if ((s == 1) == rev)
@@ -300,7 +424,12 @@
             NVB_CROW( 4u, q2.x, q2.y ) NVB_CROW( 5u, q2.z, q2.w ) NVB_CROW( 6u, q3.x, q3.y ) NVB_CROW( 7u, q3.z, q3.w )
 #undef NVB_CROW
         }
-        uint32_t sectors = e_valid ? (is_group ? 2u : 1u) : 0u;
+        if (LOCUS && settled)
+        {
+            hits[0] = settled == 1u; hits[1] = settled == 2u;
+            pos[0][0] = pos[1][0] = settled_x;
+        }
+        uint32_t sectors = (e_valid && !(LOCUS && settled)) ? (is_group ? 2u : 1u) : 0u;
         const uint32_t i = rid * q.spr + j;
         uint32_t tile_fill = 0;
         uint32_t defer_fill = 0;
@@ -378,6 +507,66 @@
             for (int d = 32; d > 0; d >>= 1) tot += (uint32_t)__shfl_xor( (int)tot, d );
             if (lane == 0 && tot) atomicAdd( sectors_out, (unsigned long long)tot );
         }
+    };
+
+    uint32_t tile = blockIdx.x * 4u + (threadIdx.x >> 6);
+    if (tile >= tl.n_tiles) return;
+    if constexpr (LOCUS)
+    {
+        fm_seed_locus_loop<BITS,COUNT,WIDE>( f, q, tl, locus, sectors_out, routes, tile, lane, lr, j, lane_ok, seed_geom, entry_of, resolve_tile );
+        return;
+    }
+    SeedWords W = { 0, 0, 0, 0, 0 }; uint32_t w_begin = 0, w_pfw = 0, w_rlen = 0; bool w_valid = false;
+    uint64_t V = 0; uint4 e = make_uint4( 1u, 0u, 0u, 0u ); bool e_valid = false; uint32_t qo = 0, c_pfw = 0, c_rlen = 0; bool c_seed = false;
+    {
+        const uint32_t rid = tile * tl.rpt + lr;
+        if (lane_ok && rid < tl.reads)
+        {
+            uint32_t b0;
+            c_seed = seed_geom( rid, b0, c_pfw, c_rlen );
+            if (c_seed)
+            {
+                const SeedWords W0 = load_seed_words<BITS>( q.symbols, b0, len );
+                e_valid = seed_bits_from_words<BITS>( W0, b0, len, false, false, V );
+                if (e_valid) e = entry_of( V, qo );
+            }
+        }
+        const uint32_t t1 = tile + n_waves, rid1 = t1 * tl.rpt + lr;
+        if (t1 < tl.n_tiles && lane_ok && rid1 < tl.reads)
+        {
+            w_valid = seed_geom( rid1, w_begin, w_pfw, w_rlen );
+            if (w_valid) W = load_seed_words<BITS>( q.symbols, w_begin, len );
+        }
+    }
+    for (; tile < tl.n_tiles; tile += n_waves)
+    {
+        const uint32_t rid = tile * tl.rpt + lr;
+        const bool valid = lane_ok && rid < tl.reads && c_seed;
+        const bool is_one   = e_valid && e.y >= DTAB_MARK && e.x < DTAB_MARK;
+        const bool is_group = e_valid && e.y >= DTAB_MARK && e.x >= DTAB_MARK;
+        const bool is_heavy = e_valid && e.y < DTAB_MARK && e.x <= e.y;
+        uint4 q0 = make_uint4( 0, 0, 0, 0 ), q1 = q0, q2 = q0, q3 = q0;
+        const uint32_t m = e.y - DTAB_MARK;
+        if (is_group)
+        {
+            const uint4* g4 = (const uint4*)(f.cside + 4ull * (e.x - DTAB_MARK));
+            q0 = g4[0]; q1 = g4[1];
+            if (m > 4u) { q2 = g4[2]; q3 = g4[3]; }
+        }
+        uint64_t Vn = 0; uint4 en = make_uint4( 1u, 0u, 0u, 0u ); bool en_valid = false; uint32_t qon = 0;
+        const uint32_t n_pfw = w_pfw, n_rlen = w_rlen; const bool n_seed = w_valid;
+        if (w_valid)
+        {
+            en_valid = seed_bits_from_words<BITS>( W, w_begin, len, false, false, Vn );
+            if (en_valid) en = entry_of( Vn, qon );
+        }
+        {
+            const uint32_t t2 = tile + 2u * n_waves, rid2 = t2 * tl.rpt + lr;
+            w_valid = t2 < tl.n_tiles && lane_ok && rid2 < tl.reads;
+            if (w_valid) w_valid = seed_geom( rid2, w_begin, w_pfw, w_rlen );
+            if (w_valid) W = load_seed_words<BITS>( q.symbols, w_begin, len );
+        }
+        resolve_tile( tile, rid, valid, V, e, e_valid, qo, c_pfw, c_rlen, is_one, is_group, is_heavy, q0, q1, q2, q3, 0u, 0u );
         V = Vn; e = en; e_valid = en_valid; qo = qon; c_pfw = n_pfw; c_rlen = n_rlen; c_seed = n_seed;
     }
 }
diff --git a/nvbio-gpl_amd/csrc/fm_index.hip b/nvbio-gpl_amd/csrc/fm_index.hip
--- a/nvbio-gpl_amd/csrc/fm_index.hip
+++ b/nvbio-gpl_amd/csrc/fm_index.hip
@@ -1,6 +1,7 @@
 #include "fm_device.h"
 #include "fm_seed_device.h"
 #include "seed_hits_device.h"
+#include "bitplanes.h"
 #include <hipcub/hipcub.hpp>
 #include <new>
 #include <stdlib.h>
@@ -27,6 +28,8 @@
     uint32_t*            isa;
     uint32_t*            text;
     void*                planes;
+    void*                locus;
+    uint32_t             locus_len;
 
     DevIndex dev() const
     {
@@ -1095,6 +1098,52 @@
     return NVBIO_OK;
 }
 
+constexpr uint32_t SEED_LOCUS_DEFAULT_LEN = 22u;
+
+static nvbio_status seed_locus_served(const FMIndexImpl* idx, const uint32_t seed_len)
+{
+    if (!(idx->ctab && idx->text))
+    {
+        set_error( "the seed locus lines need the canonical table and the text: build the index with NVBIO_FM_TABLE_CANONICAL and sa_int = 1" );
+        return NVBIO_ERR_UNSUPPORTED;
+    }
+    NVB_REQUIRE( seed_len >= idx->ckmer && seed_len - idx->ckmer <= CTAB_FLANK, "seed length outside [kmer_len, kmer_len + 7]" );
+    return NVBIO_OK;
+}
+
+static nvbio_status seed_locus_fill(const FMIndexImpl* idx, const uint32_t seed_len, void* lines_dev, hipStream_t stream)
+{
+    NVB_CHECK( seed_locus_served( idx, seed_len ) );
+    NVB_REQUIRE( ((uintptr_t)lines_dev & (SEED_LOCUS_LINE_BYTES - 1u)) == 0, "lines_dev must be 128-byte aligned" );
+    const uint32_t n = idx->view.length;
+    const uint64_t n_lines = seed_locus_lines( n ), n_units = ((uint64_t)n + 63u) >> 6;
+    NVB_HIP( hipMemsetAsync( lines_dev, 0, n_lines * SEED_LOCUS_LINE_BYTES, stream ) );
+    const uint64_t blocks = (n_units + 3u) / 4u;
+    return NVB_LAUNCH( seed_locus_kernel, dim3( (unsigned)(blocks < 256u * 256u ? blocks : 256u * 256u) ), dim3(256), stream, idx->dev(), seed_len, idx->cwide,
+                       n_units, n_lines, (uint64_t*)lines_dev );
+}
+
+static nvbio_status handle_seed_locus(FMIndexImpl* idx, const uint32_t seed_len, hipStream_t stream)
+{
+    NVB_CHECK( seed_locus_served( idx, seed_len ) );
+    const uint64_t bytes = seed_locus_lines( idx->view.length ) * SEED_LOCUS_LINE_BYTES;
+    if (!idx->locus)
+    {
+        if (hipMalloc( &idx->locus, bytes ) != hipSuccess)
+        {
+            (void)hipGetLastError(); idx->locus = nullptr;
+            set_error( "out of device memory (seed locus lines, %llu bytes)", (unsigned long long)bytes );
+            return NVBIO_ERR_NOMEM;
+        }
+        idx->owned_bytes += bytes;
+    }
+    idx->locus_len = 0;
+    NVB_CHECK( seed_locus_fill( idx, seed_len, idx->locus, stream ) );
+    if (hipStreamSynchronize( stream ) != hipSuccess) { set_error( "seed locus build failed" ); return NVBIO_ERR_HIP; }
+    idx->locus_len = seed_len;
+    return NVBIO_OK;
+}
+
 nvbio_status fm_index_adopt(const nvbio_fm_index_view* view, int device, uint32_t kmer_len, bool owns, hipStream_t stream, nvbio_fm_index_t* out,
                             uint32_t* isa, uint32_t* text, uint32_t table_flags)
 {
@@ -1108,7 +1157,7 @@
     idx->isa = isa; idx->text = text;
     if (isa)  idx->owned_bytes += ((uint64_t)view->length + 1u) * 4ull;
     if (text) idx->owned_bytes += (((uint64_t)view->length + 15u) / 16u) * 4ull;
-    idx->planes = nullptr;
+    idx->planes = nullptr; idx->locus = nullptr; idx->locus_len = 0;
     nvbio_status st = build_kmer_table( idx, kmer_len, stream );
     const bool tables = st == NVBIO_OK;
     if (st == NVBIO_OK && text && !(table_flags & NVBIO_FM_TABLE_NO_TEXT_PLANES))
@@ -1120,9 +1169,13 @@
         if (st == NVBIO_OK && hipStreamSynchronize( stream ) != hipSuccess) { set_error( "text planes build failed" ); st = NVBIO_ERR_HIP; }
         if (st == NVBIO_OK) idx->owned_bytes += bytes;
     }
+    if (st == NVBIO_OK && idx->ctab && text && !(table_flags & NVBIO_FM_TABLE_NO_SEED_LOCUS) &&
+        idx->ckmer <= SEED_LOCUS_DEFAULT_LEN && SEED_LOCUS_DEFAULT_LEN <= idx->ckmer + CTAB_FLANK)
+        st = handle_seed_locus( idx, SEED_LOCUS_DEFAULT_LEN, stream );
     if (st != NVBIO_OK)
     {
         if (idx->planes) (void)hipFree( idx->planes );
+        if (idx->locus)  (void)hipFree( idx->locus );
         if (tables)
         {
             if (idx->ktab)  (void)hipFree( idx->ktab );
@@ -1185,6 +1238,7 @@
     if (idx->isa)  (void)hipFree( idx->isa );
     if (idx->text) (void)hipFree( idx->text );
     if (idx->planes) (void)hipFree( idx->planes );
+    if (idx->locus)  (void)hipFree( idx->locus );
     if (idx->owns_arrays) { (void)hipFree( (void*)idx->view.bwt_occ_dev ); (void)hipFree( (void*)idx->view.ssa_dev ); }
     delete idx;
     return NVBIO_OK;
@@ -1223,6 +1277,39 @@
     *planes_dev = idx->planes;
     *length     = idx->planes ? idx->view.length : 0u;
     return NVBIO_OK;
+}
+
+nvbio_status nvbio_seed_locus_bytes(uint32_t length, uint64_t* bytes)
+{
+    NVB_REQUIRE( bytes != nullptr, "bytes is NULL" );
+    *bytes = seed_locus_lines( length ) * SEED_LOCUS_LINE_BYTES;
+    return NVBIO_OK;
+}
+
+nvbio_status nvbio_seed_locus_build(nvbio_fm_index_t index, uint32_t seed_len, void* lines_dev, void* stream)
+{
+    NVB_REQUIRE( index && lines_dev, "index/lines_dev is NULL" );
+    const FMIndexImpl* idx = (const FMIndexImpl*)index;
+    DeviceGuard g( idx->device ); if (!g.ok) return NVBIO_ERR_NO_DEVICE;
+    return seed_locus_fill( idx, seed_len, lines_dev, (hipStream_t)stream );
+}
+
+nvbio_status nvbio_fm_index_seed_locus(nvbio_fm_index_t index, const void** lines_dev, uint32_t* seed_len)
+{
+    NVB_REQUIRE( index && lines_dev && seed_len, "index/lines_dev/seed_len is NULL" );
+    const FMIndexImpl* idx = (const FMIndexImpl*)index;
+    const bool have = idx->locus && idx->locus_len;
+    *lines_dev = have ? idx->locus : nullptr;
+    *seed_len  = have ? idx->locus_len : 0u;
+    return NVBIO_OK;
+}
+
+nvbio_status nvbio_fm_index_build_seed_locus(nvbio_fm_index_t index, uint32_t seed_len, void* stream)
+{
+    NVB_REQUIRE( index != nullptr, "index is NULL" );
+    FMIndexImpl* idx = (FMIndexImpl*)index;
+    DeviceGuard g( idx->device ); if (!g.ok) return NVBIO_ERR_NO_DEVICE;
+    return handle_seed_locus( idx, seed_len, (hipStream_t)stream );
 }
 
 nvbio_status nvbio_fm_match(nvbio_fm_index_t index, const nvbio_string_set* queries, uint32_t flags,
@@ -1584,8 +1671,12 @@
     hipStream_t s = (hipStream_t)stream;
     const bool count = (flags & NVBIO_FM_COUNT_SECTORS) != 0;
     const bool defer = (flags & NVBIO_FM_DEFER_HEAVY) != 0 && !count;
+    const bool routes = (flags & NVBIO_FM_COUNT_LOCUS) != 0;
+    NVB_REQUIRE( !routes || count, "NVBIO_FM_COUNT_LOCUS goes with NVBIO_FM_COUNT_SECTORS" );
     NVB_REQUIRE( !count || ((uintptr_t)counts_dev & 7u) == 0, "counts_dev must be 8-byte aligned with NVBIO_FM_COUNT_SECTORS" );
-    NVB_HIP( hipMemsetAsync( counts_dev, 0, (count ? 6 : 4) * sizeof(uint32_t), s ) );
+    NVB_HIP( hipMemsetAsync( counts_dev, 0, (routes ? 10 : (count ? 6 : 4)) * sizeof(uint32_t), s ) );
+    const bool use_locus = idx->locus && idx->locus_len == q.fixed_len && !(flags & NVBIO_FM_NO_SEED_LOCUS) &&
+                           (q.intervals != nullptr || read_len <= SEED_LOCUS_MAX_READ);
     if (q.n == 0) return NVBIO_OK;
     NVB_REQUIRE( keys_dev && residual_ranges_dev && residual_ids_dev, "NULL device pointer" );
     SeedScratch L; NVB_CHECK( seed_scratch_layout( seeds, true, &L ) );
@@ -1603,18 +1694,20 @@
     inline_max = inline_max < 1u ? 1u : (inline_max > CTAB_INLINE ? CTAB_INLINE : inline_max);
     NVB_CHECK( with_value( Values<2, 4>(), seeds->symbol_bits, [&](auto BITS)
     {
-        const auto launch = [&](auto CNT, auto W, auto D)
-        {
-            return NVB_LAUNCH( (fm_seed_both_kernel<BITS,CNT,W,D>), grid, block, s, f, q, L.tl, read_len, inline_max, tile_keys, tile_counts,
+        const auto launch = [&](auto CNT, auto W, auto D, auto LC)
+        {
+            return NVB_LAUNCH( (fm_seed_both_kernel<BITS,CNT,W,D,LC>), grid, block, s, f, q, L.tl, read_len, inline_max, tile_keys, tile_counts,
                                (uint2*)residual_ranges_dev, residual_ids_dev, residual_capacity, (unsigned int*)counts_dev,
-                               CNT ? (unsigned long long*)(counts_dev + 4) : (unsigned long long*)nullptr, tile_defer, defer_counts );
+                               CNT ? (unsigned long long*)(counts_dev + 4) : (unsigned long long*)nullptr, tile_defer, defer_counts,
+                               (const void*)(LC ? idx->locus : nullptr), routes ? (unsigned int*)counts_dev + 6 : (unsigned int*)nullptr );
         };
-        const auto wide = [&](auto W)
-        {
-            if (count) return launch( std::true_type(),  W, std::false_type() );
-            if (defer) return launch( std::false_type(), W, std::true_type() );
-            return            launch( std::false_type(), W, std::false_type() );
+        const auto kind = [&](auto W, auto LC)
+        {
+            if (count) return launch( std::true_type(),  W, std::false_type(), LC );
+            if (defer) return launch( std::false_type(), W, std::true_type(),  LC );
+            return            launch( std::false_type(), W, std::false_type(), LC );
         };
+        const auto wide = [&](auto W) { return use_locus ? kind( W, std::true_type() ) : kind( W, std::false_type() ); };
         return idx->cwide ? wide( std::true_type() ) : wide( std::false_type() );
     }, bad_symbol_bits ) );
     size_t scan_bytes = L.scan_bytes;
diff --git a/nvbio-gpl_amd/pipeline.py b/nvbio-gpl_amd/pipeline.py
--- a/nvbio-gpl_amd/pipeline.py
+++ b/nvbio-gpl_amd/pipeline.py
@@ -2,10 +2,10 @@
 
 import numpy as np
 
-from . import (ALN_RAGGED_READS, FM_COMPLEMENT, FM_SCAN_FORWARD, LOCAL, READ_COMPLEMENT, READ_REVERSE, SCORE_MIN, SEMI_GLOBAL, AlignmentBatch,
+from . import (ALN_RAGGED_READS, FM_COMPLEMENT, FM_NO_SEED_LOCUS, FM_SCAN_FORWARD, LOCAL, READ_COMPLEMENT, READ_REVERSE, SCORE_MIN, SEMI_GLOBAL, AlignmentBatch,
                BatchedBandedAlignmentScore, FMIndexFilter, GotohAligner, GotohScheme, HitQueues, PackedStringSet, RaggedSeedLayout, SeedHitsParams,
                best_approx_init_ragged, read_queue_begin_ragged, score_reduce_effort, score_reduce_effort_ragged, score_stream_flatten, score_stream_output,
-               seed_hits_loc, seed_hits_map, seed_hits_map_ragged, seed_hits_select)
+               seed_hits_loc, seed_hits_map, seed_hits_map_ragged, seed_hits_select, SEED_NO_LOCUS)
 
 
 class SeedExtendParams:
@@ -108,7 +108,8 @@
         timers.setdefault("match_both", []).append((a, ev_t))
         a.record()
     fmi.match_seed_diagonals_both(geo["qs"], reads.read_len, b, inline_hits=min(4, params.max_seed_hits or 4), defer_heavy=params.defer_heavy,
-                                  grid_blocks=int(getattr(params, "seed_grid_blocks", 0) or 0))
+                                  grid_blocks=int(getattr(params, "seed_grid_blocks", 0) or 0),
+                                  flags=FM_NO_SEED_LOCUS if (params.algo_flags or 0) & SEED_NO_LOCUS else 0)
     if ev_t is not None:
         ev_t.record()
     if "host" not in b:
```

Result: faster. 2.230 billion, median of 6 (+10.0%).
